# a1q123456/image_stitching

Measured on AMD Instinct MI355X. Metric: 4K frames stitched/sec, higher is better.
Workload: dtype u8

## Files before the change

host/job.cpp:

```cpp
#include "job.hpp"
#include <cstring>

namespace mis {

StitchJob::StitchJob(int device, int width, int height, const std::vector<CameraParams>& cameras, const StitchConfig& cfg)
    : JobCore("mis::StitchJob", "", device, nullptr, width, height, cameras, cfg) {}

StitchJob::~StitchJob() {
    mis_image_free(cctx_, &pano_);
    mis_image_free(cctx_, &mask_);
}

void StitchJob::finalize() {
    if (pano_.data && (pano_.width != key_.pano.width || pano_.height != key_.pano.height)) { mis_image_free(cctx_, &pano_); mis_image_free(cctx_, &mask_); pano_ = MisImage{}; mask_ = MisImage{}; }
    if (!pano_.data) { pano_ = MisImage{}; mask_ = MisImage{}; pano_.mem = mask_.mem = MIS_MEM_DEVICE; }
    check(cctx_, mis_blender_blend(blender_, &pano_, &mask_), "mis_blender_blend");
}

JobOutput StitchJob::run(const std::vector<MisImage>& frames) {
    if ((int)frames.size() != n_) throw std::runtime_error("StitchJob::run: one frame per camera");
    JobOutput out;
    check(cctx_, mis_context_wait(cctx_, ctx_), "mis_context_wait");
    const MisImage* work = work_frames(frames);
    prep_.arm([this] { if (spec_ok_) prepare(everyone_); });
    check(ctx_, mis_orb_on_enqueued(orb_, &Hook::fire, &prep_), "mis_orb_on_enqueued");
    std::vector<MisFeatures> feats(n_);
    std::memset(feats.data(), 0, sizeof(MisFeatures) * n_);
    const int rc_f = mis_orb_detect_batch(orb_, work, n_, feats.data());
    mis_orb_on_enqueued(orb_, nullptr, nullptr);
    check(ctx_, rc_f, "mis_orb_detect_batch");
    prep_.finish();
    for (int i = 0; i < n_; i++) { feats[i].img_idx = i; out.num_features.push_back(feats[i].n); }
    const MisMatchParams mp = reset_matches();
    match_.arm([this, &frames] {
        if (!spec_ok_) return;
        fence_knn();
        compose(frames, everyone_, everyone_);
        finalize();
    });
    check(ctx_, mis_match_on_enqueued(ctx_, &Hook::fire, &match_), "mis_match_on_enqueued");
    const int rc = mis_match_pairs_model(ctx_, feats.data(), n_, &mp, model_, nullptr, cfg_.range_width, 0, 1, pairwise_.data());
    mis_match_on_enqueued(ctx_, nullptr, nullptr);
    for (auto& f : feats) mis_features_free(ctx_, &f);
    check(ctx_, rc, "mis_match_pairs_model");
    match_.finish();
    out.confidence.resize((size_t)n_ * n_);
    for (int k = 0; k < n_ * n_; k++) out.confidence[k] = pairwise_[k].confidence;
    std::vector<int> idx(n_);
    int kept = 0;
    check(ctx_, mis_leave_biggest_component(pairwise_.data(), n_, cfg_.conf_thresh, idx.data(), &kept), "mis_leave_biggest_component");
    idx.resize(kept);
    if (kept < 2) throw std::runtime_error("Need more images");
    out.indices = idx;
    out.speculation_kept = spec_ok_ && kept == n_;
    if (!out.speculation_kept) {
        prepare(idx);
        compose(frames, everyone_, idx);
        finalize();
    }
    check(cctx_, mis_context_synchronize(cctx_), "mis_context_synchronize (compose)");
    out.pano = pano_; out.mask = mask_;
    out.num_bands = key_.bands; out.pano_width = key_.pano.width; out.pano_height = key_.pano.height;
    out.matches = pairwise_;
    return out;
}

}
```

host/job_core.cpp:

```cpp
#include "job_core.hpp"
#include <algorithm>
#include <numeric>

namespace mis {

static float median_focal(const std::vector<CameraParams>& cams, const std::vector<int>& idx) {
    std::vector<double> f;
    for (int i : idx) f.push_back(cams[i].focal);
    std::sort(f.begin(), f.end());
    return f.size() % 2 == 1 ? static_cast<float>(f[f.size() / 2]) : static_cast<float>(f[f.size() / 2 - 1] + f[f.size() / 2]) * 0.5f;
}

void JobCore::Hook::fire(void* self_) {
    Hook* self = static_cast<Hook*>(self_);
    self->ran_ = true;
    try { self->body_(); } catch (const std::exception& e) { self->error_ = e.what(); }
}

void JobCore::Hook::arm(std::function<void()> body) {
    body_ = std::move(body);
    ran_ = false;
    error_.clear();
}

void JobCore::Hook::finish() {
    if (!ran_) fire(this);
    if (!error_.empty()) throw std::runtime_error(error_);
}

void JobCore::check(MisContext* c, int rc, const char* what) const {
    if (rc != MIS_OK) throw std::runtime_error(std::string(what) + " failed" + where_ + ": " + mis_last_error(c));
}

JobCore::JobCore(const char* who, std::string where, int device, void* main_stream, int width, int height, const std::vector<CameraParams>& cameras,
                 const StitchConfig& cfg)
    : w_(width), h_(height), n_((int)cameras.size()), wg_(work_geometry(cfg, width, height)), cams_(cameras), cfg_(cfg), everyone_(n_), mstream_(main_stream),
      where_(std::move(where)) {
    std::iota(everyone_.begin(), everyone_.end(), 0);
    if (wg_.scale != 1.0) {
        for (auto& c : cams_) { c.focal *= wg_.scale; c.ppx *= wg_.scale; c.ppy *= wg_.scale; }
        compose_work_aspect_ = 1.0 / wg_.scale;
    }
    try {
        if (cfg_.features_type != "orb" || cfg_.ba_cost_func != "no" || cfg_.expos_comp_type != "no" || cfg_.seam_find_type != "no")
            throw std::runtime_error(std::string(who) + " runs the hot path (ORB, supplied cameras, no seam-scale step); use mis::Stitcher for the other options");
        kind_ = warp_kind(cfg_.warp_type);
        check_range_width(cfg_.range_width);
        model_ = matcher_model(cfg_.matcher_type, cfg_.range_width);
        if (mis_context_create(device, mstream_, &ctx_) != MIS_OK) throw std::runtime_error("mis_context_create failed: no HIP device (there is no CPU fallback)");
        check(ctx_, mis_stream_create(device, 0, &cstream_), "mis_stream_create");
        if (mis_context_create(device, cstream_, &cctx_) != MIS_OK) throw std::runtime_error("mis_context_create (compose stream) failed");
        MisOrbParams op;
        mis_orb_default_params(&op);
        check(ctx_, mis_orb_create(ctx_, &op, wg_.width, wg_.height, &orb_), "mis_orb_create");
    } catch (...) {
        release();
        throw;
    }
    Ks_.resize((size_t)n_ * 9); Rs_.resize((size_t)n_ * 9);
    for (int i = 0; i < n_; i++) {
        CameraParams cc = cams_[i];
        if (compose_work_aspect_ != 1.0) { cc.focal *= compose_work_aspect_; cc.ppx *= compose_work_aspect_; cc.ppy *= compose_work_aspect_; }
        const Mat3<float> K = cc.K().cast<float>(), R = cams_[i].R.cast<float>();
        std::copy(K.m.begin(), K.m.end(), Ks_.begin() + 9 * i);
        std::copy(R.m.begin(), R.m.end(), Rs_.begin() + 9 * i);
    }
    if (kind_ != MIS_WARP_SPHERICAL) {
        const float scale = warp_scale(everyone_);
        MisRect r;
        if (MIS_WARP_ROI_IS_FULL_SCAN(kind_)) {
            std::vector<MisRect> rr((size_t)n_);
            spec_ok_ = n_ == 0 || mis_warper_roi_batch(cctx_, kind_, scale, w_, h_, n_, Ks_.data(), Rs_.data(), rr.data()) == MIS_OK;
        } else
            for (int i = 0; i < n_ && spec_ok_; i++) spec_ok_ = mis_warper_roi(kind_, scale, w_, h_, &Ks_[9 * i], &Rs_[9 * i], &r) == MIS_OK;
    }
}

JobCore::~JobCore() { release(); }

float JobCore::warp_scale(const std::vector<int>& idx) const {
    const float scale = median_focal(cams_, idx);
    return compose_work_aspect_ != 1.0 ? scale * static_cast<float>(compose_work_aspect_) : scale;
}

const MisImage* JobCore::work_frames(const std::vector<MisImage>& frames) {
    if (wg_.scale == 1.0 || frames.empty()) return frames.data();
    if (work_.size() < frames.size()) work_.resize(frames.size(), MisImage{});
    check(ctx_, mis_resize_linear_exact_batch(ctx_, frames.data(), (int)frames.size(), 0, 0, wg_.scale, wg_.scale, work_.data()), "mis_resize_linear_exact_batch");
    return work_.data();
}

void JobCore::release() {
    if (cctx_) mis_context_synchronize(cctx_);
    if (ctx_) mis_context_synchronize(ctx_);
    if (!pairwise_.empty()) mis_matches_free(pairwise_.data(), (int)pairwise_.size());
    if (ctx_) for (auto& im : work_) mis_image_free(ctx_, &im);
    if (blender_) mis_blender_destroy(blender_);
    if (orb_) mis_orb_destroy(orb_);
    if (cctx_) mis_context_destroy(cctx_);
    if (ctx_) mis_context_destroy(ctx_);
    if (cstream_) mis_stream_destroy(cstream_);
    if (mstream_) mis_stream_destroy(mstream_);
}

void JobCore::synchronize() {
    check(ctx_, mis_context_synchronize(ctx_), "mis_context_synchronize");
    check(cctx_, mis_context_synchronize(cctx_), "mis_context_synchronize (compose)");
}

JobCore::Compose JobCore::prepare(const std::vector<int>& idx) {
    const int m = (int)idx.size();
    const float scale = warp_scale(idx);
    std::vector<float> Ks((size_t)m * 9), Rs((size_t)m * 9);
    for (int k = 0; k < m; k++) {
        std::copy(Ks_.begin() + 9 * idx[k], Ks_.begin() + 9 * idx[k] + 9, Ks.begin() + 9 * k);
        std::copy(Rs_.begin() + 9 * idx[k], Rs_.begin() + 9 * idx[k] + 9, Rs.begin() + 9 * k);
    }
    rois_.assign(m, MisRect{});
    check(cctx_, mis_warper_roi_batch(cctx_, kind_, scale, w_, h_, m, Ks.data(), Rs.data(), rois_.data()), "mis_warper_roi_batch");
    std::vector<MisPoint> corners(m);
    std::vector<MisSize> sizes(m);
    for (int k = 0; k < m; k++) { corners[k] = {rois_[k].x, rois_[k].y}; sizes[k] = {rois_[k].width, rois_[k].height}; }
    Compose c;
    check(cctx_, mis_result_roi(corners.data(), sizes.data(), m, &c.pano), "mis_result_roi");
    check(cctx_, mis_blend_config(cfg_.blend_type, cfg_.blend_strength, c.pano.width, c.pano.height, &c.type, &c.bands, &c.sharp), "mis_blend_config");
    if (!blender_ || c.type != key_.type || c.bands != key_.bands || c.sharp != key_.sharp) {
        if (blender_) { mis_blender_destroy(blender_); blender_ = nullptr; }
        check(cctx_, mis_blender_create(cctx_, c.type, c.bands, c.sharp, &blender_), "mis_blender_create");
    }
    key_ = c;
    check(cctx_, mis_blender_prepare(blender_, corners.data(), sizes.data(), m), "mis_blender_prepare");
    return c;
}

void JobCore::fence_knn() {
    const int rc = mis_match_knn_fence(ctx_, cstream_, mis_match_sequence(ctx_), 0);
    if (rc < 0) check(ctx_, rc, "mis_match_knn_fence");
}

void JobCore::compose(const std::vector<MisImage>& frames, const std::vector<int>& frame_ids, const std::vector<int>& idx) {
    std::vector<MisImage> fr;
    std::vector<float> Ks, Rs;
    std::vector<MisRect> rois;
    for (size_t q = 0; q < frame_ids.size(); q++) {
        const auto it = std::find(idx.begin(), idx.end(), frame_ids[q]);
        if (it == idx.end()) continue;
        fr.push_back(frames[q]);
        Ks.insert(Ks.end(), Ks_.begin() + 9 * frame_ids[q], Ks_.begin() + 9 * frame_ids[q] + 9);
        Rs.insert(Rs.end(), Rs_.begin() + 9 * frame_ids[q], Rs_.begin() + 9 * frame_ids[q] + 9);
        rois.push_back(rois_[it - idx.begin()]);
    }
    if (fr.empty()) return;
    check(cctx_, mis_compose_frames_kind(blender_, kind_, fr.data(), (int)fr.size(), warp_scale(idx), Ks.data(), Rs.data(), rois.data()),
          "mis_compose_frames_kind");
}

MisMatchParams JobCore::reset_matches() {
    if (!pairwise_.empty()) { mis_matches_free(pairwise_.data(), (int)pairwise_.size()); pairwise_.clear(); }
    pairwise_.assign((size_t)n_ * n_, MisMatchesInfo{});
    return match_params(model_, cfg_.match_conf);
}

}
```

host/job_core.hpp:

```cpp
#pragma once
#include <functional>
#include <string>
#include <vector>
#include "stitcher.hpp"

namespace mis {

struct JobOutput {
    std::vector<int> indices;
    std::vector<double> confidence;
    std::vector<int> num_features;
    MisImage pano{}, mask{};
    int num_bands = 0, pano_width = 0, pano_height = 0;
    bool speculation_kept = false;
    std::vector<MisMatchesInfo> matches;
};

class JobCore {
protected:
    struct Compose { int type = 0, bands = 0; float sharp = 0; MisRect pano{}; };

    class Hook {
    public:
        static void fire(void* self);
        void arm(std::function<void()> body);
        void finish();
    private:
        std::function<void()> body_;
        bool ran_ = false;
        std::string error_;
    };

    JobCore(const char* who, std::string where, int device, void* main_stream, int width, int height, const std::vector<CameraParams>& cameras,
            const StitchConfig& cfg);
    ~JobCore();
    JobCore(const JobCore&) = delete;
    JobCore& operator=(const JobCore&) = delete;

    void check(MisContext* c, int rc, const char* what) const;
    void synchronize();
    Compose prepare(const std::vector<int>& idx);
    void fence_knn();
    const MisImage* work_frames(const std::vector<MisImage>& frames);
    float warp_scale(const std::vector<int>& idx) const;
    void compose(const std::vector<MisImage>& frames, const std::vector<int>& frame_ids, const std::vector<int>& idx);
    MisMatchParams reset_matches();

    int w_, h_, n_;
    WorkGeometry wg_;
    double compose_work_aspect_ = 1;
    std::vector<CameraParams> cams_;
    std::vector<MisImage> work_;
    StitchConfig cfg_;
    std::vector<int> everyone_;
    int kind_ = MIS_WARP_SPHERICAL;
    int model_ = MIS_MATCH_HOMOGRAPHY;
    bool spec_ok_ = true;
    void* mstream_ = nullptr;
    void* cstream_ = nullptr;
    MisContext* ctx_ = nullptr;
    MisContext* cctx_ = nullptr;
    MisOrb* orb_ = nullptr;
    MisBlender* blender_ = nullptr;
    Compose key_{};
    std::vector<float> Ks_, Rs_;
    std::vector<MisRect> rois_;
    std::vector<MisMatchesInfo> pairwise_;

private:
    void release();
    std::string where_;
};

}
```

image_stitching_amd/_capi.py:

```python
import ctypes as C
import os
import re

_HERE = os.path.dirname(os.path.abspath(__file__))
LIB_PATH = os.path.join(_HERE, "libmistitch.so")
HEADER_PATH = os.path.join(os.path.dirname(_HERE), "include", "mistitch.h")

MIS_OK = 0
MIS_FENCE_TIMEOUT = 1
MEM_HOST, MEM_DEVICE = 0, 1
U8, S16, F32 = 0, 1, 2
INTER_NEAREST, INTER_LINEAR = 0, 1
BORDER_CONSTANT, BORDER_REFLECT = 0, 2
BLEND_NO, BLEND_FEATHER, BLEND_MULTI_BAND = 0, 1, 2
WARP_SPHERICAL, WARP_CYLINDRICAL, WARP_PLANE, WARP_MERCATOR, WARP_FISHEYE, WARP_STEREOGRAPHIC = 0, 1, 2, 3, 4, 5


def roi_is_full_scan(kind):
    return WARP_MERCATOR <= kind <= WARP_STEREOGRAPHIC


MATH_LOG, MATH_TAN, MATH_SINH, MATH_ASIN, MATH_ATAN, MATH_EXP = 0, 1, 2, 3, 4, 5
MATCH_HOMOGRAPHY, MATCH_AFFINE_PARTIAL = 0, 1
EXPOS_NO, EXPOS_GAIN, EXPOS_GAIN_BLOCKS, EXPOS_CHANNELS, EXPOS_CHANNELS_BLOCKS = 0, 1, 2, 3, 4


class MisPoint(C.Structure):
    _fields_ = [("x", C.c_int), ("y", C.c_int)]


class MisSize(C.Structure):
    _fields_ = [("width", C.c_int), ("height", C.c_int)]


class MisRect(C.Structure):
    _fields_ = [("x", C.c_int), ("y", C.c_int), ("width", C.c_int), ("height", C.c_int)]


class MisLevelRect(C.Structure):
    _fields_ = [("level", C.c_int), ("x0", C.c_int), ("y0", C.c_int), ("x1", C.c_int), ("y1", C.c_int), ("offset", C.c_ulonglong)]


class MisImage(C.Structure):
    _fields_ = [("data", C.c_void_p), ("width", C.c_int), ("height", C.c_int), ("channels", C.c_int),
                ("stride", C.c_size_t), ("dtype", C.c_int), ("mem", C.c_int)]


class MisKeyPoint(C.Structure):
    _fields_ = [("x", C.c_float), ("y", C.c_float), ("size", C.c_float), ("angle", C.c_float),
                ("response", C.c_float), ("octave", C.c_int)]


class MisOrbParams(C.Structure):
    _fields_ = [("nfeatures", C.c_int), ("scale_factor", C.c_float), ("nlevels", C.c_int),
                ("edge_threshold", C.c_int), ("first_level", C.c_int), ("wta_k", C.c_int),
                ("score_type", C.c_int), ("patch_size", C.c_int), ("fast_threshold", C.c_int)]


class MisSiftParams(C.Structure):
    _fields_ = [("nfeatures", C.c_int), ("n_octave_layers", C.c_int), ("contrast_threshold", C.c_double),
                ("edge_threshold", C.c_double), ("sigma", C.c_double)]


class MisCameraParams(C.Structure):
    _fields_ = [("focal", C.c_double), ("aspect", C.c_double), ("ppx", C.c_double), ("ppy", C.c_double), ("R", C.c_double * 9),
                ("t", C.c_double * 3)]


class MisFeatures(C.Structure):
    _fields_ = [("img_idx", C.c_int), ("img_w", C.c_int), ("img_h", C.c_int), ("n", C.c_int),
                ("keypoints", C.c_void_p), ("descriptors", C.c_void_p), ("desc_cols", C.c_int),
                ("desc_dtype", C.c_int), ("owner_", C.c_void_p)]


class MisMatchParams(C.Structure):
    _fields_ = [("match_conf", C.c_float), ("num_matches_thresh1", C.c_int), ("num_matches_thresh2", C.c_int),
                ("ransac_thresh", C.c_double), ("max_iters", C.c_int), ("confidence", C.c_double)]


class MisCompensatorParams(C.Structure):
    _fields_ = [("type", C.c_int), ("nr_feeds", C.c_int), ("block_width", C.c_int), ("block_height", C.c_int),
                ("nr_gain_filtering_iterations", C.c_int)]


class MisDMatch(C.Structure):
    _fields_ = [("query_idx", C.c_int), ("train_idx", C.c_int), ("img_idx", C.c_int), ("distance", C.c_float)]


class MisMatchesInfo(C.Structure):
    _fields_ = [("src_img_idx", C.c_int), ("dst_img_idx", C.c_int), ("n_matches", C.c_int),
                ("matches", C.POINTER(MisDMatch)), ("inliers_mask", C.POINTER(C.c_uint8)), ("num_inliers", C.c_int),
                ("has_H", C.c_int), ("H", C.c_double * 9), ("confidence", C.c_double)]


_vp, _i, _f, _d = C.c_void_p, C.c_int, C.c_float, C.c_double
_P = C.POINTER

PROTOTYPES = {
    "mis_context_create": (_i, [_i, _vp, _P(_vp)]),
    "mis_stream_create": (_i, [_i, _i, _P(_vp)]),
    "mis_stream_destroy": (_i, [_vp]),
    "mis_context_destroy": (_i, [_vp]),
    "mis_context_synchronize": (_i, [_vp]),
    "mis_context_wait": (_i, [_vp, _vp]),
    "mis_last_error": (C.c_char_p, [_vp]),
    "mis_version": (C.c_char_p, []),
    "mis_image_free": (_i, [_vp, _P(MisImage)]),
    "mis_orb_default_params": (None, [_P(MisOrbParams)]),
    "mis_orb_create": (_i, [_vp, _P(MisOrbParams), _i, _i, _P(_vp)]),
    "mis_orb_destroy": (_i, [_vp]),
    "mis_orb_detect": (_i, [_vp, _P(MisImage), _P(MisFeatures)]),
    "mis_orb_detect_batch": (_i, [_vp, _P(MisImage), _i, _P(MisFeatures)]),
    "mis_orb_on_enqueued": (_i, [_vp, _vp, _vp]),
    "mis_features_download": (_i, [_vp, _P(MisFeatures), _vp, _vp]),
    "mis_features_upload": (_i, [_vp, _i, _i, _i, _vp, _vp, _i, _i, _P(MisFeatures)]),
    "mis_features_free": (_i, [_vp, _P(MisFeatures)]),
    "mis_orb_debug_level": (_i, [_vp, _i, _i, _vp, _P(_i), _P(_i)]),
    "mis_sift_default_params": (None, [_P(MisSiftParams)]),
    "mis_sift_create": (_i, [_vp, _P(MisSiftParams), _i, _i, _P(_vp)]),
    "mis_sift_destroy": (_i, [_vp]),
    "mis_sift_detect": (_i, [_vp, _P(MisImage), _P(MisFeatures)]),
    "mis_sift_detect_batch": (_i, [_vp, _P(MisImage), _i, _P(MisFeatures)]),
    "mis_sift_debug_level": (_i, [_vp, _P(MisImage), _i, _i, _i, _vp, _P(_i), _P(_i)]),
    "mis_sift_debug_counts": (_i, [_vp, _P(C.c_uint)]),
    "mis_match_default_params": (None, [_P(MisMatchParams)]),
    "mis_match_all_pairs": (_i, [_vp, _P(MisFeatures), _i, _P(MisMatchParams), _P(MisMatchesInfo)]),
    "mis_match_pairs_sharded": (_i, [_vp, _P(MisFeatures), _i, _P(MisMatchParams), _i, _i, _P(MisMatchesInfo)]),
    "mis_match_pairs_select": (_i, [_vp, _P(MisFeatures), _i, _P(MisMatchParams), _vp, _i, _i, _i, _P(MisMatchesInfo)]),
    "mis_match_affine_default_params": (None, [_P(MisMatchParams)]),
    "mis_match_pairs_model": (_i, [_vp, _P(MisFeatures), _i, _P(MisMatchParams), _i, _vp, _i, _i, _i, _P(MisMatchesInfo)]),
    "mis_estimate_affine_partial": (_i, [_vp, _vp, _vp, _i, _d, _i, _d, _i, _vp, _vp, _P(_i)]),
    "mis_matches_free": (_i, [_P(MisMatchesInfo), _i]),
    "mis_match_sequence": (C.c_longlong, [_vp]),
    "mis_match_knn_fence": (_i, [_vp, _vp, C.c_longlong, _i]),
    "mis_match_on_enqueued": (_i, [_vp, _vp, _vp]),
    "mis_knn2": (_i, [_vp, _P(MisFeatures), _P(MisFeatures), _vp, _vp]),
    "mis_find_homography": (_i, [_vp, _vp, _vp, _i, _d, _i, _d, _vp, _vp, _P(_i)]),
    "mis_leave_biggest_component": (_i, [_P(MisMatchesInfo), _i, _f, _vp, _P(_i)]),
    "mis_leave_biggest_component_conf": (_i, [_vp, _i, _f, _vp, _P(_i)]),
    "mis_bundle_adjust_reproj": (_i, [_vp, _P(MisFeatures), _P(MisMatchesInfo), _i, _f, C.c_char_p, _P(MisCameraParams)]),
    "mis_wave_correct": (_i, [_vp, _i, _i]),
    "mis_warp_roi": (_i, [_f, _i, _i, _vp, _vp, _P(MisRect)]),
    "mis_warp_spherical": (_i, [_vp, _P(MisImage), _f, _vp, _vp, _i, _i, _P(MisImage), _P(MisPoint)]),
    "mis_warp_roi_batch": (_i, [_vp, _f, _i, _i, _i, _vp, _vp, _P(MisRect)]),
    "mis_warp_spherical_fused_roi": (_i, [_vp, _P(MisImage), _f, _vp, _vp, _P(MisRect), _P(MisImage), _P(MisImage), _P(MisPoint)]),
    "mis_warp_spherical_fused_batch": (_i, [_vp, _P(MisImage), _i, C.c_float, _P(C.c_float), _P(C.c_float), _P(MisRect), _P(MisImage), _P(MisImage), _P(MisPoint)]),
    "mis_warp_spherical_fused_batch_timed": (_i, [_vp, _P(MisImage), _i, C.c_float, _P(C.c_float), _P(C.c_float), _P(MisRect), _P(MisImage), _P(MisImage), _P(MisPoint), _i,
                                               _P(C.c_float)]),
    "mis_debug_math_f32": (_i, [_vp, _i, _vp, _vp, _i]),
    "mis_warper_roi": (_i, [_i, _f, _i, _i, _vp, _vp, _P(MisRect)]),
    "mis_warper_roi_batch": (_i, [_vp, _i, _f, _i, _i, _i, _vp, _vp, _P(MisRect)]),
    "mis_warper_warp": (_i, [_vp, _i, _P(MisImage), _f, _vp, _vp, _i, _i, _P(MisImage), _P(MisPoint)]),
    "mis_warper_warp_roi": (_i, [_vp, _i, _P(MisImage), _f, _vp, _vp, _P(MisRect), _i, _i, _P(MisImage), _P(MisPoint)]),
    "mis_warper_warp_fused": (_i, [_vp, _i, _P(MisImage), _f, _vp, _vp, _P(MisImage), _P(MisImage), _P(MisPoint)]),
    "mis_warper_warp_fused_roi": (_i, [_vp, _i, _P(MisImage), _f, _vp, _vp, _P(MisRect), _P(MisImage), _P(MisImage), _P(MisPoint)]),
    "mis_warper_warp_fused_batch": (_i, [_vp, _i, _P(MisImage), _i, C.c_float, _P(C.c_float), _P(C.c_float), _P(MisRect), _P(MisImage), _P(MisImage), _P(MisPoint)]),
    "mis_warp_spherical_fused": (_i, [_vp, _P(MisImage), _f, _vp, _vp, _P(MisImage), _P(MisImage), _P(MisPoint)]),
    "mis_resize_linear_exact": (_i, [_vp, _P(MisImage), _i, _i, C.c_double, C.c_double, _P(MisImage)]),
    "mis_resize_linear_exact_batch": (_i, [_vp, _P(MisImage), _i, _i, _i, C.c_double, C.c_double, _P(MisImage)]),
    "mis_rotate": (_i, [_vp, _P(MisImage), _i, _P(MisImage)]),
    "mis_seam_mask_apply": (_i, [_vp, _P(MisImage), _P(MisImage)]),
    "mis_compensator_create": (_i, [_vp, _i, _i, _i, _P(_vp)]),
    "mis_compensator_default_params": (None, [_P(MisCompensatorParams)]),
    "mis_compensator_create_ex": (_i, [_vp, _P(MisCompensatorParams), _P(_vp)]),
    "mis_compensator_destroy": (_i, [_vp]),
    "mis_compensator_gains": (_i, [_vp, _i, _P(_d)]),
    "mis_compensator_gain_map_channels": (_i, [_vp, _i, _P(C.c_float), _i, _P(_i), _P(_i), _P(_i)]),
    "mis_compensator_debug_stats": (_i, [_vp, _i, _i, _i, _P(_i), _P(_d), _P(_d)]),
    "mis_compensator_feed": (_i, [_vp, _P(MisPoint), _P(MisImage), _P(MisImage), _i]),
    "mis_compensator_gain_map": (_i, [_vp, _i, _P(C.c_float), _i, _P(_i), _P(_i)]),
    "mis_compensator_apply": (_i, [_vp, _i, _P(MisImage)]),
    "mis_seam_voronoi": (_i, [_vp, _P(MisPoint), _P(MisImage), _i]),
    "mis_seam_dp": (_i, [_vp, _P(MisPoint), _P(MisImage), _P(MisImage), _i, _i]),
    "mis_warp_spherical_fused_timed": (_i, [_vp, _P(MisImage), _f, _vp, _vp, _P(MisImage), _P(MisImage), _P(MisPoint), _i, _P(C.c_float)]),
    "mis_blend_config": (_i, [_i, _f, _i, _i, _P(_i), _P(_i), _P(_f)]),
    "mis_result_roi": (_i, [_P(MisPoint), _P(MisSize), _i, _P(MisRect)]),
    "mis_blender_create": (_i, [_vp, _i, _i, _f, _P(_vp)]),
    "mis_blender_destroy": (_i, [_vp]),
    "mis_blender_prepare": (_i, [_vp, _P(MisPoint), _P(MisSize), _i]),
    "mis_blender_num_bands": (_i, [_vp]),
    "mis_blender_feed": (_i, [_vp, _P(MisImage), _P(MisImage), MisPoint]),
    "mis_blender_feed_batch": (_i, [_vp, _P(MisImage), _P(MisImage), _P(MisPoint), _i]),
    "mis_blender_blend": (_i, [_vp, _P(MisImage), _P(MisImage)]),
    "mis_compose_frames": (_i, [_vp, _P(MisImage), _i, _f, _vp, _vp, _P(MisRect)]),
    "mis_compose_frames_kind": (_i, [_vp, _i, _P(MisImage), _i, _f, _vp, _vp, _P(MisRect)]),
    "mis_blender_blend_columns": (_i, [_vp, _i, _i, _P(MisImage), _P(MisImage)]),
    "mis_blender_pack_rects": (_i, [_vp, _P(MisLevelRect), _i, _vp, C.c_size_t]),
    "mis_blender_add_rects": (_i, [_vp, _P(MisLevelRect), _i, _vp, C.c_size_t]),
    "mis_blender_zero_rects": (_i, [_vp, _P(MisLevelRect), _i]),
    "mis_features_pack": (_i, [_vp, _P(MisFeatures), _i, _i, _i, _vp, _vp]),
    "mis_copy_2d": (_i, [_vp, _vp, C.c_size_t, _vp, C.c_size_t, C.c_size_t, C.c_size_t]),
    "mis_blender_feed_rect": (_i, [_vp, _i, _i, MisPoint, _P(MisRect)]),
    "mis_blender_level_info": (_i, [_vp, _i, _P(_i), _P(_i), _P(_vp), _P(_vp)]),
}


def header_functions():
    txt = open(HEADER_PATH).read()
    txt = re.sub(r"/\*.*?\*/", "", txt, flags=re.S)
    return sorted(set(re.findall(r"\b(mis_[a-z0-9_]+)\s*\(", txt)))


_lib = None


def load():
    global _lib
    if _lib is not None:
        return _lib
    if not os.path.exists(LIB_PATH):
        raise ImportError("libmistitch.so is not built (%s missing): run `python -c 'import __graft_entry__ as g; g.build()'` "
                          "or `make -C image_stitching_amd/csrc`; there is no CPU fallback" % LIB_PATH)
    lib = C.CDLL(LIB_PATH)
    for name, (res, args) in PROTOTYPES.items():
        fn = getattr(lib, name)
        fn.restype = res
        fn.argtypes = args
    _lib = lib
    return lib
```

image_stitching_amd/csrc/common.h:

```cpp
#pragma once
#include <hip/hip_runtime.h>
#include <stdint.h>
#include <stdio.h>
#include <string.h>
#include <string>
#include <vector>
#include "../../include/mistitch.h"

struct MisWorkspace {
    virtual ~MisWorkspace() {}
};

struct MisContext {
    int device = 0;
    int num_cu = 256;
    MisWorkspace* match_ws = nullptr;
    MisWorkspace* resize_ws = nullptr;
    std::vector<std::pair<size_t, void*>> pool;
    hipStream_t stream = nullptr;
    bool own_stream = false;
    std::string err;
    void* stage = nullptr;
    size_t stage_bytes = 0;
    hipStream_t aux[2] = {nullptr, nullptr};
    void* roi_pinned = nullptr;
    size_t roi_pinned_bytes = 0;
    void* host_stage = nullptr;
    size_t host_stage_bytes = 0;
};

int mis_set_error(MisContext* ctx, int code, const char* fmt, ...);
int mis_host_stage(MisContext* ctx, size_t bytes, void** out);
int mis_dev_stage(MisContext* ctx, size_t bytes, void** out);
int mis_pool_alloc(MisContext* ctx, size_t bytes, void** out, size_t* got, MisContext* errs = nullptr);
int mis_aux_stream(MisContext* ctx, int k, hipStream_t* out);
void mis_pool_free(MisContext* ctx, void* p, size_t bytes);
int mis_feat_block_alloc(MisContext* ctx, size_t bytes, void** out, MisContext* errs = nullptr);
struct MisFeatLayout { size_t desc_off, count_off, bytes; };
MisFeatLayout mis_feat_layout(int cap, int desc_cols, int desc_dtype);
int mis_feat_alloc(MisContext* ctx, int cap, int desc_cols, int desc_dtype, MisFeatures* f);
int* mis_feat_count(const MisFeatures* f, int cap);

#define MIS_HIP(ctx, call)                                                                             \
    do {                                                                                               \
        hipError_t e_ = (call);                                                                        \
        if (e_ != hipSuccess)                                                                          \
            return mis_set_error((ctx), MIS_E_HIP, "%s failed: %s (%s:%d)", #call, hipGetErrorString(e_), \
                                 __FILE__, __LINE__);                                                  \
    } while (0)

#define MIS_CHECK(ctx, cond, code, ...)                              \
    do {                                                             \
        if (!(cond)) return mis_set_error((ctx), (code), __VA_ARGS__); \
    } while (0)

static inline size_t mis_dtype_size(int dtype) { return dtype == MIS_U8 ? 1 : (dtype == MIS_S16 ? 2 : 4); }
static inline size_t mis_align_up(size_t v, size_t a) { return (v + a - 1) / a * a; }

struct DevView {
    void* data = nullptr;
    size_t stride = 0;
    DevView() = default;
    DevView(const DevView&) = delete;
    DevView& operator=(const DevView&) = delete;
    ~DevView();
    int read(MisContext* ctx, const MisImage* img);
    int write(MisContext* ctx, MisImage* img, int width, int height, int channels, int dtype);
    int read_write(MisContext* ctx, MisImage* img);
    int commit();
private:
    MisContext* ctx_ = nullptr;
    MisImage* out_ = nullptr;
    MisImage entry_{};
    bool staged_ = false, fresh_ = false;
};

struct OwnedEvent {
    hipEvent_t ev = nullptr;
    OwnedEvent() = default; OwnedEvent(const OwnedEvent&) = delete;
    ~OwnedEvent() { if (ev) hipEventDestroy(ev); }
    hipError_t ready(unsigned flags = hipEventDisableTiming) { return ev ? hipSuccess : hipEventCreateWithFlags(&ev, flags); }
};
```

image_stitching_amd/csrc/features.hip:

```cpp
#include "common.h"
#include <algorithm>
#include <mutex>
#include <unordered_map>

namespace {

std::mutex g_feat_mutex;
std::unordered_map<void*, size_t> g_feat_sizes;

}

MisFeatLayout mis_feat_layout(int cap, int desc_cols, int desc_dtype) {
    MisFeatLayout l;
    l.desc_off = mis_align_up(sizeof(MisKeyPoint) * (size_t)cap, 256);
    l.count_off = l.desc_off + mis_align_up((size_t)cap * desc_cols * mis_dtype_size(desc_dtype), 256);
    l.bytes = l.count_off + 256;
    return l;
}

int mis_feat_block_alloc(MisContext* ctx, size_t bytes, void** out, MisContext* errs) {
    size_t got = 0;
    const int rc = mis_pool_alloc(ctx, bytes, out, &got, errs);
    if (rc != MIS_OK) return rc;
    std::lock_guard<std::mutex> lock(g_feat_mutex);
    g_feat_sizes[*out] = got;
    return MIS_OK;
}

int mis_feat_alloc(MisContext* ctx, int cap, int desc_cols, int desc_dtype, MisFeatures* f) {
    const MisFeatLayout l = mis_feat_layout(cap, desc_cols, desc_dtype);
    void* mem = nullptr;
    const int rc = mis_feat_block_alloc(ctx, l.bytes, &mem);
    if (rc != MIS_OK) return rc;
    f->keypoints = (MisKeyPoint*)mem;
    f->descriptors = (uint8_t*)mem + l.desc_off;
    f->desc_cols = desc_cols; f->desc_dtype = desc_dtype;
    f->owner_ = mem;
    f->n = 0;
    return MIS_OK;
}

int* mis_feat_count(const MisFeatures* f, int cap) {
    return (int*)((uint8_t*)f->owner_ + mis_feat_layout(cap, f->desc_cols, f->desc_dtype).count_off);
}

extern "C" int mis_features_download(MisContext* ctx, const MisFeatures* f, MisKeyPoint* kps, void* desc) {
    if (!ctx || !f) return MIS_E_INVALID;
    MIS_HIP(ctx, hipSetDevice(ctx->device));
    if (f->n > 0) {
        if (kps) MIS_HIP(ctx, hipMemcpyAsync(kps, f->keypoints, sizeof(MisKeyPoint) * (size_t)f->n, hipMemcpyDeviceToHost, ctx->stream));
        if (desc) MIS_HIP(ctx, hipMemcpyAsync(desc, f->descriptors, (size_t)f->n * f->desc_cols * mis_dtype_size(f->desc_dtype), hipMemcpyDeviceToHost, ctx->stream));
    }
    MIS_HIP(ctx, hipStreamSynchronize(ctx->stream));
    return MIS_OK;
}

extern "C" int mis_features_upload(MisContext* ctx, int img_w, int img_h, int n, const MisKeyPoint* kps, const void* desc, int desc_cols,
                                   int desc_dtype, MisFeatures* out) {
    if (!ctx || !out) return MIS_E_INVALID;
    MIS_CHECK(ctx, n >= 0 && (n == 0 || (kps && desc)) && desc_cols > 0 && (desc_dtype == MIS_U8 || desc_dtype == MIS_F32), MIS_E_INVALID,
              "bad feature arrays");
    MIS_HIP(ctx, hipSetDevice(ctx->device));
    memset(out, 0, sizeof(*out));
    out->img_w = img_w; out->img_h = img_h;
    int rc = mis_feat_alloc(ctx, std::max(n, 1), desc_cols, desc_dtype, out);
    if (rc != MIS_OK) return rc;
    if (n) {
        MIS_HIP(ctx, hipMemcpyAsync(out->keypoints, kps, sizeof(MisKeyPoint) * (size_t)n, hipMemcpyHostToDevice, ctx->stream));
        MIS_HIP(ctx, hipMemcpyAsync(out->descriptors, desc, (size_t)n * desc_cols * mis_dtype_size(desc_dtype), hipMemcpyHostToDevice, ctx->stream));
        MIS_HIP(ctx, hipStreamSynchronize(ctx->stream));
    }
    out->n = n;
    return MIS_OK;
}

extern "C" int mis_features_free(MisContext* ctx, MisFeatures* f) {
    if (!ctx || !f) return MIS_E_INVALID;
    if (f->owner_) {
        size_t bytes = 0;
        {
            std::lock_guard<std::mutex> lock(g_feat_mutex);
            auto it = g_feat_sizes.find(f->owner_);
            if (it != g_feat_sizes.end()) { bytes = it->second; g_feat_sizes.erase(it); }
        }
        if (bytes) mis_pool_free(ctx, f->owner_, bytes);
        else {
            MIS_HIP(ctx, hipSetDevice(ctx->device));
            MIS_HIP(ctx, hipStreamSynchronize(ctx->stream));
            MIS_HIP(ctx, hipFree(f->owner_));
        }
    }
    f->owner_ = nullptr; f->keypoints = nullptr; f->descriptors = nullptr; f->n = 0;
    return MIS_OK;
}
```

image_stitching_amd/csrc/match.hip:

```cpp
#include "common.h"
#include <thread>
#include <chrono>
#include <atomic>
#include "dev_math.h"
#include "homography.h"
#include <algorithm>
#include <vector>

namespace {

struct FeatDev {
    const uint8_t* desc;
    const MisKeyPoint* kps;
    int n, w, h;
};

struct PairDesc {
    int i, j;
    size_t knn_off12, knn_off21;
    size_t m_off;
    int cap;
};

constexpr int KNN_TILE = 256;
__global__ __launch_bounds__(256) void knn2_hamming_kernel(const FeatDev* feats, const PairDesc* pairs, int* idx2, float* dist2) {
    __shared__ uint4 tr[KNN_TILE * 2];
    const PairDesc pd = pairs[blockIdx.y >> 1];
    const bool fwd = (blockIdx.y & 1) == 0;
    const FeatDev Q = feats[fwd ? pd.i : pd.j], T = feats[fwd ? pd.j : pd.i];
    const size_t off = fwd ? pd.knn_off12 : pd.knn_off21;
    const int q0 = blockIdx.x * 256;
    if (q0 >= Q.n) return;
    const int q = q0 + threadIdx.x;
    const bool active = q < Q.n;
    uint4 a0 = make_uint4(0, 0, 0, 0), a1 = a0;
    if (active) {
        const uint4* p = reinterpret_cast<const uint4*>(Q.desc + (size_t)q * 32);
        a0 = p[0]; a1 = p[1];
    }
    int k0 = 0x7fffffff, k1 = 0x7fffffff;
    for (int t0 = 0; t0 < T.n; t0 += KNN_TILE) {
        const int nt = min(KNN_TILE, T.n - t0);
        __syncthreads();
        const uint4* src = reinterpret_cast<const uint4*>(T.desc + (size_t)t0 * 32);
        for (int k = threadIdx.x; k < nt * 2; k += 256) tr[k] = src[k];
        __syncthreads();
        if (active) {
            auto one = [&](int j) {
                const uint4 b0 = tr[2 * j], b1 = tr[2 * j + 1];
                unsigned d = 0;
                auto acc = [&](unsigned x) { asm("v_bcnt_u32_b32 %0, %1, %0" : "+v"(d) : "v"(x)); };
                acc(a0.x ^ b0.x); acc(a0.y ^ b0.y); acc(a0.z ^ b0.z); acc(a0.w ^ b0.w);
                acc(a1.x ^ b1.x); acc(a1.y ^ b1.y); acc(a1.z ^ b1.z); acc(a1.w ^ b1.w);
                const int key = (int)((d << 22) | (unsigned)(t0 + j));
                asm("v_med3_i32 %0, %1, %2, %3" : "=v"(k1) : "v"(k0), "v"(k1), "v"(key));
                k0 = min(k0, key);
            };
            int j = 0;
            for (; j + 8 <= nt; j += 8) {
#pragma unroll
                for (int u = 0; u < 8; u++) one(j + u);
            }
            for (; j < nt; j++) one(j);
        }
    }
    if (active) {
        const int d0 = k0 == 0x7fffffff ? 1 << 30 : k0 >> 22, d1 = k1 == 0x7fffffff ? 1 << 30 : k1 >> 22;
        idx2[(off + q) * 2] = k0 == 0x7fffffff ? -1 : (k0 & 0x3fffff); idx2[(off + q) * 2 + 1] = k1 == 0x7fffffff ? -1 : (k1 & 0x3fffff);
        dist2[(off + q) * 2] = (float)d0; dist2[(off + q) * 2 + 1] = (float)d1;
    }
}

typedef int v4i __attribute__((ext_vector_type(4)));
typedef int v16i __attribute__((ext_vector_type(16)));
constexpr int HM_ROWPAD = 256;
constexpr int HM_MAX_TRAINS = 8192;
constexpr int HM_NONE = 0x7f000000;

struct HmFrame { size_t train_off, query_off; };

struct HmKeys { int k0[2], k1[2]; };
struct HmJob { int pair, dir, q0, pad; };
constexpr int HM_FBIAS = 0x3F800000;
__device__ __forceinline__ void hm_update(HmKeys& K, int set, int key) {
    asm volatile("v_med3_f32 %0, %1, %2, %3" : "=v"(K.k1[set]) : "v"(K.k0[set]), "v"(K.k1[set]), "v"(key));
    asm volatile("v_min_f32 %0, %1, %2" : "=v"(K.k0[set]) : "v"(K.k0[set]), "v"(key));
}
__device__ __forceinline__ void hm_dma(const int8_t* base, unsigned voff, uint32_t lds_off) {
    asm volatile("s_mov_b32 m0, %2\n\ts_nop 0\n\tglobal_load_lds_dwordx4 %0, %1" ::"v"(voff), "s"(base), "s"(lds_off) : "memory", "m0");
}
__global__ __launch_bounds__(256) void hamming_expand4_kernel(const FeatDev* feats, const HmFrame* fr, int8_t* out) {
    const FeatDev F = feats[blockIdx.y];
    const int npad = (F.n + HM_ROWPAD - 1) / HM_ROWPAD * HM_ROWPAD;
    const int item = blockIdx.x * 256 + threadIdx.x, d = item >> 3, w = item & 7;
    if (d >= npad) return;
    const bool live = d < F.n;
    const unsigned x = live ? reinterpret_cast<const unsigned*>(F.desc)[(size_t)d * 8 + w] : 0u;
    unsigned tq[4], qq[4];
#pragma unroll
    for (int k = 0; k < 4; k++) {
        unsigned t = (x >> (8 * k)) & 255u;
        t = (t | (t << 12)) & 0x000F000Fu;
        t = (t | (t << 6)) & 0x03030303u;
        t = (t | (t << 3)) & 0x11111111u;
        tq[k] = live ? (0xEEEEEEEEu ^ (t << 3)) : 0u;
        qq[k] = live ? (0x66666666u ^ (t << 3)) : 0u;
    }
    *reinterpret_cast<uint4*>(out + fr[blockIdx.y].train_off + (size_t)d * 128 + 16 * w) = make_uint4(tq[0], tq[1], tq[2], tq[3]);
    *reinterpret_cast<uint4*>(out + fr[blockIdx.y].query_off + (size_t)d * 128 + 16 * w) = make_uint4(qq[0], qq[1], qq[2], qq[3]);
}
#define HM4_MFMA_FIRST(D, A, B, C, SA, SB) \
    asm volatile("v_mfma_scale_f32_32x32x64_f8f6f4 %0, %1, %2, %3, %4, %5 op_sel_hi:[0,0,0] cbsz:4 blgp:4" : "=&v"(D) : "v"(A), "v"(B), "v"(C), "v"(SA), "v"(SB))
#define HM4_MFMA_ACC(D, A, B, SA, SB) \
    asm volatile("v_mfma_scale_f32_32x32x64_f8f6f4 %0, %1, %2, %0, %3, %4 op_sel_hi:[0,0,0] cbsz:4 blgp:4" : "+v"(D) : "v"(A), "v"(B), "v"(SA), "v"(SB))
typedef float v16f __attribute__((ext_vector_type(16)));
__device__ __forceinline__ void hm_update_triples(HmKeys& K, int x0, int x1, int x2, int y0, int y1, int y2) {
    int t0, t1, u0, u1;
    asm volatile(
        "v_min3_f32 %4, %8, %9, %10\n\tv_med3_f32 %5, %8, %9, %10\n\tv_min3_f32 %6, %11, %12, %13\n\tv_med3_f32 %7, %11, %12, %13\n\t"
        "v_min_f32 %5, %1, %5\n\tv_min_f32 %7, %3, %7\n\t"
        "v_med3_f32 %1, %0, %4, %5\n\tv_med3_f32 %3, %2, %6, %7\n\t"
        "v_min_f32 %0, %0, %4\n\tv_min_f32 %2, %2, %6"
        : "+v"(K.k0[0]), "+v"(K.k1[0]), "+v"(K.k0[1]), "+v"(K.k1[1]), "=&v"(t0), "=&v"(t1), "=&v"(u0), "=&v"(u1)
        : "v"(x0), "v"(x1), "v"(x2), "v"(y0), "v"(y1), "v"(y2));
}
__device__ __forceinline__ void hm_update_both(HmKeys& K, int a, int b) {
    asm volatile("v_med3_f32 %1, %0, %1, %4\n\tv_min_f32 %0, %0, %4\n\tv_med3_f32 %3, %2, %3, %5\n\tv_min_f32 %2, %2, %5"
                 : "+v"(K.k0[0]), "+v"(K.k1[0]), "+v"(K.k0[1]), "+v"(K.k1[1]) : "v"(a), "v"(b));
}
template <bool UPD>
__device__ __forceinline__ void hm_tile_fp4(v16i& accA, v16i& accB, const v16i& prevA, const v16i& prevB, v16f& cb, v4i* a, const v4i (&bq)[2][4], HmKeys& K,
                                            const int8_t* lds_next, uint32_t lds_store, const int8_t* gnext, unsigned voff, const unsigned (&aoff)[4], int sa, int sb) {
    hm_dma(gnext, voff, lds_store);
#pragma unroll
    for (int s4 = 0; s4 < 4; s4++) {
#pragma unroll
        for (int half = 0; half < 2; half++) {
            const int slot = 2 * s4 + half;
            if (half == 0) { if (s4 == 0) HM4_MFMA_FIRST(accA, a[0], bq[0][0], cb, sa, sb); else HM4_MFMA_ACC(accA, a[s4], bq[0][s4], sa, sb); }
            else {
                if (s4 == 0) HM4_MFMA_FIRST(accB, a[0], bq[1][0], cb, sa, sb); else HM4_MFMA_ACC(accB, a[s4], bq[1][s4], sa, sb);
                a[s4] = *reinterpret_cast<const v4i*>(lds_next + aoff[s4]);
            }
            if (slot >= 2) {
                if (UPD) {
                    const int j = slot - 2;
                    if (j < 5) hm_update_triples(K, prevA[3 * j], prevA[3 * j + 1], prevA[3 * j + 2], prevB[3 * j], prevB[3 * j + 1], prevB[3 * j + 2]);
                    else hm_update_both(K, prevA[15], prevB[15]);
                }
                if (slot >= 4) {
#pragma unroll
                    for (int g = (slot - 4) * 4; g < (slot - 3) * 4; g++) cb[g] += 32.f;
                }
            }
            __builtin_amdgcn_sched_barrier(0);
        }
    }
    asm volatile("s_waitcnt vmcnt(0)" ::: "memory");
    __syncthreads();
}

__global__ __launch_bounds__(256) void knn2_hamming_fp4_kernel(const FeatDev* feats, const PairDesc* pairs, const HmFrame* fr, const int8_t* __restrict__ xp, int* idx2,
                                                               float* dist2, const HmJob* jobs) {
    __shared__ __attribute__((aligned(1024))) int8_t tr[2][32 * 128];
    const HmJob job = jobs[blockIdx.x];
    if (job.pair < 0) return;
    const PairDesc pd = pairs[job.pair];
    const bool fwd = job.dir == 0;
    const int qi = fwd ? pd.i : pd.j, ti = fwd ? pd.j : pd.i;
    const int nq = feats[qi].n, nt = feats[ti].n;
    const size_t off = fwd ? pd.knn_off12 : pd.knn_off21;
    const int q0 = job.q0;
    if (q0 >= nq) return;
    const int lane = threadIdx.x & 63, wave = __builtin_amdgcn_readfirstlane(threadIdx.x >> 6), r = lane & 31, h = lane >> 5;
    const int8_t* qx = xp + fr[qi].query_off;
    const int8_t* tx = xp + fr[ti].train_off;
    HmKeys K;
    K.k0[0] = K.k0[1] = K.k1[0] = K.k1[1] = HM_NONE;
    const int ntiles = (nt + 31) / 32;
    if (ntiles > 0) {
        v4i bq[2][4];
#pragma unroll
        for (int set = 0; set < 2; set++)
#pragma unroll
            for (int s4 = 0; s4 < 4; s4++)
                bq[set][s4] = *reinterpret_cast<const v4i*>(qx + (size_t)(q0 + wave * 64 + set * 32 + r) * 128 + 32 * s4 + 16 * h);
        v16f cb;
#pragma unroll
        for (int g = 0; g < 16; g++) cb[g] = (float)((1 << 20) + (g & 3) + 8 * (g >> 2) + 4 * h);
        const int sa = 127 + 4, sb = 127 + 4;
        const int R = 8 * wave + (lane >> 3);
        const unsigned voff = (unsigned)(R * 128 + 16 * ((lane & 7) ^ ((R >> 1) & 7)));
        unsigned aoff[4];
#pragma unroll
        for (int s4 = 0; s4 < 4; s4++) aoff[s4] = (unsigned)(r * 128 + 16 * ((2 * s4 + h) ^ ((r >> 1) & 7)));
        const uint32_t lds0 = (uint32_t)(uintptr_t)&tr[0][0] + (uint32_t)wave * 1024, lds1 = (uint32_t)(uintptr_t)&tr[1][0] + (uint32_t)wave * 1024;
        auto gtile = [&](int t) { return tx + (size_t)min(t, ntiles - 1) * 32 * 128; };
        hm_dma(gtile(0), voff, lds0);
        hm_dma(gtile(1), voff, lds1);
        asm volatile("s_waitcnt vmcnt(0)" ::: "memory");
        __syncthreads();
        v4i a[4];
#pragma unroll
        for (int s4 = 0; s4 < 4; s4++) a[s4] = *reinterpret_cast<const v4i*>(&tr[0][aoff[s4]]);
        __syncthreads();
        v16i A0, B0, A1, B1;
        hm_tile_fp4<false>(A0, B0, A1, B1, cb, a, bq, K, tr[1], lds0, gtile(2), voff, aoff, sa, sb);
        int t = 1;
        for (; t + 1 < ntiles; t += 2) {
            hm_tile_fp4<true>(A1, B1, A0, B0, cb, a, bq, K, tr[0], lds1, gtile(t + 2), voff, aoff, sa, sb);
            hm_tile_fp4<true>(A0, B0, A1, B1, cb, a, bq, K, tr[1], lds0, gtile(t + 3), voff, aoff, sa, sb);
        }
        const bool odd_last = t < ntiles;
        if (odd_last) hm_tile_fp4<true>(A1, B1, A0, B0, cb, a, bq, K, tr[0], lds1, gtile(t + 2), voff, aoff, sa, sb);
        asm volatile("s_nop 15\n\ts_nop 15\n\ts_nop 15\n\ts_nop 15\n\ts_nop 15" ::: "memory");
#pragma unroll
        for (int g = 0; g < 16; g++) {
            const int ka = odd_last ? A1[g] : A0[g], kb = odd_last ? B1[g] : B0[g];
            hm_update(K, 0, ((int)__int_as_float(ka) & (HM_MAX_TRAINS - 1)) < nt ? ka : HM_NONE);
            hm_update(K, 1, ((int)__int_as_float(kb) & (HM_MAX_TRAINS - 1)) < nt ? kb : HM_NONE);
        }
    }
#pragma unroll
    for (int set = 0; set < 2; set++) {
        const int o0 = __shfl_xor(K.k0[set], 32), o1 = __shfl_xor(K.k1[set], 32);
        const int b0 = min(K.k0[set], o0), b1 = min(max(K.k0[set], o0), min(K.k1[set], o1));
        const int q = q0 + wave * 64 + set * 32 + r;
        if (h == 0 && q < nq) {
            const bool v0 = b0 < HM_NONE, v1 = b1 < HM_NONE;
            const int i0 = v0 ? (int)__int_as_float(b0) : 0, i1 = v1 ? (int)__int_as_float(b1) : 0;
            idx2[(off + q) * 2] = v0 ? (i0 & (HM_MAX_TRAINS - 1)) : -1; idx2[(off + q) * 2 + 1] = v1 ? (i1 & (HM_MAX_TRAINS - 1)) : -1;
            dist2[(off + q) * 2] = (float)(v0 ? i0 >> 13 : 1 << 30); dist2[(off + q) * 2 + 1] = (float)(v1 ? i1 >> 13 : 1 << 30);
        }
    }
}

struct L2Set {
    const _Float16* h;
    const float* nrm;
    int n;
};
__global__ __launch_bounds__(256) void l2_prep_kernel(const float* desc, int n, int dim, _Float16* h, float* nrm, int* bad) {
    const int i = blockIdx.x * 4 + (threadIdx.x >> 6), lane = threadIdx.x & 63;
    if (i >= n) return;
    float s = 0;
    for (int k = lane; k < 128; k += 64) {
        float v = k < dim ? desc[(size_t)i * dim + k] : 0.f;
        if (!(v >= 0.f && v <= 255.f && v == floorf(v))) atomicOr(bad, 1);
        h[(size_t)i * 128 + k] = (_Float16)v;
        s += v * v;
    }
    for (int o = 32; o > 0; o >>= 1) s += __shfl_xor(s, o);
    if (lane == 0) nrm[i] = s;
}

typedef _Float16 half8 __attribute__((ext_vector_type(8)));
typedef float float16v __attribute__((ext_vector_type(16)));

__device__ __forceinline__ void top2_insert(float d, int i, float& d0, int& i0, float& d1, int& i1) {
    if (d < d0 || (d == d0 && i < i0)) { d1 = d0; i1 = i0; d0 = d; i0 = i; }
    else if (d < d1 || (d == d1 && i < i1)) { d1 = d; i1 = i; }
}
// ... 193 lines not shown
    const int* i21 = idx2 + pd.knn_off21 * 2;
    const float* d21 = dist2 + pd.knn_off21 * 2;
    const float hw1 = centre ? (float)F1.w * 0.5f : 0.f, hh1 = centre ? (float)F1.h * 0.5f : 0.f, hw2 = centre ? (float)F2.w * 0.5f : 0.f, hh2 = centre ? (float)F2.h * 0.5f : 0.f;
    int base = 0;
    if (F2.n >= 2)
        for (int q0 = 0; q0 < F1.n; q0 += 1024) {
            int q = q0 + threadIdx.x, ok = 0;
            if (q < F1.n) ok = d12[2 * q] < ratio * d12[2 * q + 1];
            int tot, off = block_scan_flag(ok, &tot);
            if (ok) {
                int t = i12[2 * q];
                MisDMatch mm = {q, t, 0, d12[2 * q]};
                m[base + off] = mm;
                sp[2 * (base + off)] = F1.kps[q].x - hw1; sp[2 * (base + off) + 1] = F1.kps[q].y - hh1;
                dp[2 * (base + off)] = F2.kps[t].x - hw2; dp[2 * (base + off) + 1] = F2.kps[t].y - hh2;
            }
            base += tot;
        }
    if (F1.n >= 2)
        for (int q0 = 0; q0 < F2.n; q0 += 1024) {
            int q = q0 + threadIdx.x, ok = 0, t1 = 0;
            if (q < F2.n) {
                ok = d21[2 * q] < ratio * d21[2 * q + 1];
                if (ok) {
                    t1 = i21[2 * q];
                    bool acc12 = F2.n >= 2 && d12[2 * t1] < ratio * d12[2 * t1 + 1];
                    if (acc12 && i12[2 * t1] == q) ok = 0;
                }
            }
            int tot, off = block_scan_flag(ok, &tot);
            if (ok) {
                MisDMatch mm = {t1, q, -1, d21[2 * q]};
                m[base + off] = mm;
                sp[2 * (base + off)] = F1.kps[t1].x - hw1; sp[2 * (base + off) + 1] = F1.kps[t1].y - hh1;
                dp[2 * (base + off)] = F2.kps[q].x - hw2; dp[2 * (base + off) + 1] = F2.kps[q].y - hh2;
            }
            base += tot;
        }
    if (threadIdx.x == 0) n_matches[blockIdx.x] = base;
}

struct PairOut {
    int ran_ransac;
    int passed;
    int second;
    int pad;
};

__host__ __device__ __forceinline__ double det3(const double* H) {
    return H[0] * (H[4] * H[8] - H[5] * H[7]) - H[1] * (H[3] * H[8] - H[5] * H[6]) + H[2] * (H[3] * H[7] - H[4] * H[6]);
}

__global__ void first_calls_kernel(const PairDesc* pairs, int np, const int* n_matches, const float* src_xy, const float* dst_xy, uint8_t* masks,
                                   int thresh1, HomoCall* calls, PairOut* outs) {
    int k = blockIdx.x * blockDim.x + threadIdx.x;
    if (k >= np) return;
    const PairDesc pd = pairs[k];
    const int nm = n_matches[k];
    HomoCall c;
    c.src = src_xy + 2 * pd.m_off; c.dst = dst_xy + 2 * pd.m_off; c.mask = masks + pd.m_off; c.pt_off = (long long)pd.m_off;
    c.n = nm; c.active = nm >= thresh1;
    calls[k] = c;
    outs[k].ran_ransac = c.active; outs[k].passed = 0; outs[k].second = 0;
}


__global__ __launch_bounds__(256) void pack_lists_kernel(const PairDesc* pairs, int np, const int* nm, const MisDMatch* matches, MisDMatch* host_m, int* host_nm) {
    __shared__ int red[256];
    const int k = blockIdx.x, t = threadIdx.x;
    int part = 0;
    for (int q = t; q < k; q += 256) part += nm[q];
    red[t] = part;
    __syncthreads();
    for (int o = 128; o > 0; o >>= 1) { if (t < o) red[t] += red[t + o]; __syncthreads(); }
    const int off = red[0], cnt = nm[k];
    if (t == 0) host_nm[k] = cnt;
    const uint4* s = reinterpret_cast<const uint4*>(matches + pairs[k].m_off);
    uint4* d = reinterpret_cast<uint4*>(host_m + off);
    static_assert(sizeof(MisDMatch) == 16, "one 16-byte store per match");
    for (int i = t; i < cnt; i += 256) d[i] = s[i];
}

struct CopySegs { const uint8_t* src[8]; uint8_t* dst[8]; unsigned bytes[8]; int n; };
__global__ __launch_bounds__(256) void copy_segments_kernel(CopySegs c) {
    for (int k = 0; k < c.n; k++) {
        const uint8_t* s = c.src[k];
        uint8_t* d = c.dst[k];
        const unsigned nb = c.bytes[k];
        if ((((uintptr_t)s | (uintptr_t)d) & 3) == 0) {
            const unsigned nw = nb >> 2;
            for (unsigned i = blockIdx.x * 256 + threadIdx.x; i < nw; i += gridDim.x * 256) reinterpret_cast<unsigned*>(d)[i] = reinterpret_cast<const unsigned*>(s)[i];
            for (unsigned i = (nw << 2) + blockIdx.x * 256 + threadIdx.x; i < nb; i += gridDim.x * 256) d[i] = s[i];
        } else {
            for (unsigned i = blockIdx.x * 256 + threadIdx.x; i < nb; i += gridDim.x * 256) d[i] = s[i];
        }
    }
}

__global__ void second_calls_kernel(int np, const HomoCall* calls1, const HomoResult* res1, const float* scr1, const int* fin1, int want, int thresh2,
                                    HomoCall* calls2, PairOut* outs) {
    int k = blockIdx.x * blockDim.x + threadIdx.x;
    if (k >= np) return;
    const HomoCall c1 = calls1[k];
    HomoCall c;
    c.src = nullptr; c.dst = nullptr; c.mask = nullptr; c.pt_off = c1.pt_off; c.n = 0; c.active = 0;
    if (fin1[k] == want && c1.active && res1[k].ok) {
        outs[k].passed = 1;
        const int ninl = res1[k].ninl;
        if (ninl >= thresh2) {
            c.src = scr1 + 4 * c1.pt_off; c.dst = c.src + 2 * (size_t)c1.n; c.n = ninl; c.active = 1;
            outs[k].second = 1;
        }
    }
    calls2[k] = c;
}

void invert3(const double* H, double* I) {
    double d = H[0] * (H[4] * H[8] - H[5] * H[7]) - H[1] * (H[3] * H[8] - H[5] * H[6]) + H[2] * (H[3] * H[7] - H[4] * H[6]);
    if (d != 0.) d = 1. / d;
    I[0] = (H[4] * H[8] - H[5] * H[7]) * d; I[1] = (H[2] * H[7] - H[1] * H[8]) * d; I[2] = (H[1] * H[5] - H[2] * H[4]) * d;
    I[3] = (H[5] * H[6] - H[3] * H[8]) * d; I[4] = (H[0] * H[8] - H[2] * H[6]) * d; I[5] = (H[2] * H[3] - H[0] * H[5]) * d;
    I[6] = (H[3] * H[7] - H[4] * H[6]) * d; I[7] = (H[1] * H[6] - H[0] * H[7]) * d; I[8] = (H[0] * H[4] - H[1] * H[3]) * d;
}

struct Arena {
    void* p = nullptr;
    size_t bytes = 0;
    bool host = false;
    hipError_t reserve(size_t need) {
        if (need <= bytes) return hipSuccess;
        if (p) { hipError_t e = host ? hipHostFree(p) : hipFree(p); p = nullptr; bytes = 0; if (e != hipSuccess) return e; }
        need = need + need / 4 + 4096;
        hipError_t e = host ? hipHostMalloc(&p, need, hipHostMallocDefault) : hipMalloc(&p, need);
        if (e == hipSuccess) bytes = need;
        return e;
    }
    void release() { if (p) { if (host) hipHostFree(p); else hipFree(p); } p = nullptr; bytes = 0; }
};

struct MatchWorkspace : MisWorkspace {
    Arena dev, pinned, l2;
    HomoBatch b1, b2, b3;
    hipStream_t side = nullptr, third = nullptr;
    OwnedEvent ev_phase0, ev_side_done, ev_phase1, ev_third_done, ev_matches;
    OwnedEvent ev_knn;
    OwnedEvent ev_draw1;
    OwnedEvent ev_spec_fork, ev_spec_join;
    OwnedEvent tev[9];
    hipEvent_t ev_gate = nullptr;
    std::atomic<long long> seq{0}, knn_seq{0};
    OwnedEvent ev_lists;
    void (*enqueued_cb)(void*) = nullptr;
    void* enqueued_user = nullptr;
    MatchWorkspace() { pinned.host = true; }
    ~MatchWorkspace() override {
        dev.release(); pinned.release(); l2.release();
        homo_batch_release(&b1); homo_batch_release(&b2); homo_batch_release(&b3);
    }
    hipError_t events_ready() {
        for (OwnedEvent* e : {&ev_knn, &ev_matches, &ev_lists, &ev_phase0, &ev_draw1, &ev_side_done, &ev_phase1, &ev_third_done, &ev_spec_fork, &ev_spec_join})
            if (const hipError_t r = e->ready()) return r;
        return hipSuccess;
    }
};

MatchWorkspace* workspace(MisContext* ctx) {
    if (!ctx->match_ws) ctx->match_ws = new MatchWorkspace();
    return static_cast<MatchWorkspace*>(ctx->match_ws);
}

struct Carver {
    uintptr_t base = 0;
    size_t off = 0;
    size_t take(size_t bytes) { size_t o = off; off += mis_align_up(bytes ? bytes : 1, 256); return o; }
    void* at(size_t bytes) { return (void*)(base + take(bytes)); }
};

void init_info(MisMatchesInfo* m) { memset(m, 0, sizeof(*m)); m->src_img_idx = -1; m->dst_img_idx = -1; }

bool match_trace() { static const bool on = getenv("MIS_MATCH_TRACE") != nullptr; return on; }
void trace_mark(MatchWorkspace* ws, int i, hipStream_t s) {
    if (match_trace() && ws->tev[i].ready(hipEventDefault) == hipSuccess) hipEventRecord(ws->tev[i].ev, s);
}

int l2_knn2_pairs(MisContext* ctx, Arena& arena, const MisFeatures* f, int nsets, const PairDesc* pairs, int np, bool both_ways, int* idx2,
                  float* dist2, int* bad_host) {
    hipStream_t st = ctx->stream;
    std::vector<size_t> off(nsets);
    Carver lc;
    int maxq = 0;
    for (int s = 0; s < nsets; s++) {
        off[s] = lc.take((size_t)std::max(f[s].n, 1) * (256 + 4));
        maxq = std::max(maxq, f[s].n);
    }
    const size_t o_bad = lc.take(4), o_part = lc.take((size_t)16 * L2_MAX_SLICES * std::max(maxq, 1));
    MIS_HIP(ctx, arena.reserve(lc.off));
    uint8_t* L = (uint8_t*)arena.p;
    auto set = [&](int s) { return L2Set{(const _Float16*)(L + off[s]), (const float*)(L + off[s] + (size_t)std::max(f[s].n, 1) * 256), std::max(f[s].n, 0)}; };
    MIS_HIP(ctx, hipMemsetAsync(L + o_bad, 0, 4, st));
    for (int s = 0; s < nsets; s++)
        if (f[s].n > 0)
            hipLaunchKernelGGL(l2_prep_kernel, dim3((f[s].n + 3) / 4), dim3(256), 0, st, (const float*)f[s].descriptors, f[s].n, f[s].desc_cols,
                               (_Float16*)set(s).h, (float*)set(s).nrm, (int*)(L + o_bad));
    for (const PairDesc* pd = pairs; pd < pairs + np; pd++) {
        l2_knn2_launch(st, ctx->num_cu, set(pd->i), set(pd->j), L + o_part, idx2 + 2 * pd->knn_off12, dist2 + 2 * pd->knn_off12);
        if (both_ways) l2_knn2_launch(st, ctx->num_cu, set(pd->j), set(pd->i), L + o_part, idx2 + 2 * pd->knn_off21, dist2 + 2 * pd->knn_off21);
    }
    MIS_HIP(ctx, hipMemcpyAsync(bad_host, L + o_bad, 4, hipMemcpyDeviceToHost, st));
    return MIS_OK;
}

enum DescKind { DESC_NONE, DESC_BINARY, DESC_L2 };
struct MatchPlan {
    std::vector<PairDesc> pairs;
    std::vector<FeatDev> fd;
    size_t knn_total = 0, m_total = 0;
    int maxq = 0;
    DescKind kind = DESC_NONE;
    std::vector<HmJob> hm_jobs;
};
int plan_match(MisContext* ctx, const MisFeatures* feats, int n, const uint8_t* mask, int range_width, int rank, int world, MatchPlan* pl) {
    std::vector<PairDesc>& pairs = pl->pairs;
    pl->fd.resize(n);
    bool use_l2 = false, use_bin = false;
    for (int i = 0; i < n; i++) {
        const bool bin_i = feats[i].desc_dtype == MIS_U8 && feats[i].desc_cols == 32;
        const bool l2_i = feats[i].desc_dtype == MIS_F32 && feats[i].desc_cols >= 1 && feats[i].desc_cols <= 128;
        MIS_CHECK(ctx, feats[i].n == 0 || bin_i || l2_i, MIS_E_UNSUPPORTED,
                  "all-pairs matching supports 32-byte binary descriptors (Hamming) or f32 descriptors of <= 128 columns (L2)");
        MIS_CHECK(ctx, feats[i].n < (1 << 22), MIS_E_UNSUPPORTED, "more than 4 M keypoints in one image");
        if (feats[i].n > 0) { if (l2_i) use_l2 = true; else use_bin = true; }
        pl->fd[i] = FeatDev{(const uint8_t*)feats[i].descriptors, feats[i].keypoints, feats[i].n, feats[i].img_w, feats[i].img_h};
    }
    int pair_index = 0;
    for (int i = 0; i < n; i++)
        for (int j = i + 1; j < n; j++) {
            if (feats[i].n <= 0 || feats[j].n <= 0) continue;
            if (mask && !mask[(size_t)i * n + j]) continue;
            if (range_width != -1 && j >= i + range_width) continue;
            if ((pair_index++ % world) != rank) continue;
            const int cap = feats[i].n + feats[j].n;
            pl->maxq = std::max(pl->maxq, std::max(feats[i].n, feats[j].n));
            pairs.push_back(PairDesc{i, j, pl->knn_total, pl->knn_total + feats[i].n, pl->m_total, cap});
            pl->knn_total += cap; pl->m_total += cap;
        }
    MIS_CHECK(ctx, !(use_l2 && use_bin), MIS_E_INVALID, "binary and float descriptors cannot be mixed in one matcher call");
    for (int i = 0, cols = 0; use_l2 && i < n; i++)
        if (feats[i].n > 0) {
            MIS_CHECK(ctx, cols == 0 || feats[i].desc_cols == cols, MIS_E_INVALID, "float descriptors of different widths in one matcher call");
            cols = feats[i].desc_cols;
        }
    pl->kind = use_l2 ? DESC_L2 : (use_bin ? DESC_BINARY : DESC_NONE);
    const int np = (int)pairs.size();
    if (np == 0) return MIS_OK;
    if (pl->kind == DESC_BINARY && pl->maxq <= HM_MAX_TRAINS) {
        std::vector<HmJob> lists[8];
        for (int t = 0; t < n; t++)
            for (int k = 0; k < np; k++) {
                const int dir = pairs[k].j == t ? 0 : (pairs[k].i == t ? 1 : -1);
                if (dir < 0) continue;
                const int nqf = feats[dir == 0 ? pairs[k].i : pairs[k].j].n;
                for (int q0 = 0; q0 < nqf; q0 += 256) lists[t & 7].push_back(HmJob{k, dir, q0, 0});
            }
        size_t longest = 0;
        for (auto& l : lists) longest = std::max(longest, l.size());
        pl->hm_jobs.assign(longest * 8, HmJob{-1, 0, 0, 0});
        for (int c = 0; c < 8; c++)
            for (size_t sl = 0; sl < lists[c].size(); sl++) pl->hm_jobs[sl * 8 + c] = lists[c][sl];
    }
    return MIS_OK;
}

struct MatchDev { FeatDev* feats; PairDesc* pairs; int* idx; float* dist; MisDMatch* matches; float* src; float* dst; int* nm; uint8_t* mask; PairOut* out; };
int carve_dev(MisContext* ctx, Arena& arena, const MatchPlan& pl, MatchDev* d) {
    const size_t n = pl.fd.size(), np = pl.pairs.size(), kt = pl.knn_total, mt = pl.m_total;
    auto lay = [&](Carver c) {
        d->feats = (FeatDev*)c.at(sizeof(FeatDev) * n); d->pairs = (PairDesc*)c.at(sizeof(PairDesc) * np);
        d->idx = (int*)c.at(sizeof(int) * 2 * kt); d->dist = (float*)c.at(sizeof(float) * 2 * kt);
        d->matches = (MisDMatch*)c.at(sizeof(MisDMatch) * mt); d->src = (float*)c.at(sizeof(float) * 2 * mt); d->dst = (float*)c.at(sizeof(float) * 2 * mt);
        d->nm = (int*)c.at(sizeof(int) * np); d->mask = (uint8_t*)c.at(mt); d->out = (PairOut*)c.at(sizeof(PairOut) * np);
        return c.off;
    };
    MIS_HIP(ctx, arena.reserve(lay(Carver{})));
    lay(Carver{(uintptr_t)arena.p});
    return MIS_OK;
}

struct MatchPinned {
    FeatDev* feats; PairDesc* pairs; HmFrame* frames; HmJob* jobs;
    int* nm; PairOut* out; HomoResult *r1, *r2, *r3; int* fin; MisDMatch* m; uint8_t* mask; volatile int* l2_bad;
};
int carve_pinned(MisContext* ctx, Arena& arena, const MatchPlan& pl, MatchPinned* h) {
    const size_t n = pl.fd.size(), np = pl.pairs.size(), mt = pl.m_total;
    auto lay = [&](Carver c) {
        h->feats = (FeatDev*)c.at(sizeof(FeatDev) * n); h->pairs = (PairDesc*)c.at(sizeof(PairDesc) * np); h->frames = (HmFrame*)c.at(sizeof(HmFrame) * n);
        h->jobs = (HmJob*)c.at(sizeof(HmJob) * pl.hm_jobs.size()); h->nm = (int*)c.at(sizeof(int) * np); h->out = (PairOut*)c.at(sizeof(PairOut) * np);
        h->r1 = (HomoResult*)c.at(sizeof(HomoResult) * np); h->r2 = (HomoResult*)c.at(sizeof(HomoResult) * np); h->r3 = (HomoResult*)c.at(sizeof(HomoResult) * np);
        h->fin = (int*)c.at(sizeof(int) * np); h->m = (MisDMatch*)c.at(sizeof(MisDMatch) * mt); h->mask = (uint8_t*)c.at(mt); h->l2_bad = (volatile int*)c.at(sizeof(int));
        return c.off;
    };
    MIS_HIP(ctx, arena.reserve(lay(Carver{})));
    lay(Carver{(uintptr_t)arena.p});
    return MIS_OK;
}

int enqueue_knn(MisContext* ctx, MatchWorkspace* ws, const MatchPlan& pl, const MisFeatures* feats, const MatchDev& d, const MatchPinned& h) {
    hipStream_t st = ctx->stream;
    const int n = (int)pl.fd.size(), np = (int)pl.pairs.size();
    if (pl.kind == DESC_L2) return l2_knn2_pairs(ctx, ws->l2, feats, n, pl.pairs.data(), np, true, d.idx, d.dist, (int*)h.l2_bad);
    if (pl.maxq > HM_MAX_TRAINS) {
        hipLaunchKernelGGL(knn2_hamming_kernel, dim3((pl.maxq + 255) / 256, 2 * np), dim3(256), 0, st, (const FeatDev*)d.feats, (const PairDesc*)d.pairs, d.idx, d.dist);
        return MIS_OK;
    }
    Carver lc;
    const size_t o_fr = lc.take(sizeof(HmFrame) * n), o_jobs = lc.take(sizeof(HmJob) * pl.hm_jobs.size());
    for (int i = 0; i < n; i++) {
        const size_t rows = (size_t)(std::max(feats[i].n, 1) + HM_ROWPAD - 1) / HM_ROWPAD * HM_ROWPAD;
        h.frames[i].train_off = lc.take(rows * 128); h.frames[i].query_off = lc.take(rows * 128);
    }
    MIS_HIP(ctx, ws->l2.reserve(lc.off));
    uint8_t* L = (uint8_t*)ws->l2.p;
    MIS_HIP(ctx, hipMemcpyAsync(L + o_fr, h.frames, sizeof(HmFrame) * n, hipMemcpyHostToDevice, st));
    const int maxpad = (pl.maxq + HM_ROWPAD - 1) / HM_ROWPAD * HM_ROWPAD;
    hipLaunchKernelGGL(hamming_expand4_kernel, dim3(maxpad * 8 / 256, n), dim3(256), 0, st, (const FeatDev*)d.feats, (const HmFrame*)(L + o_fr), (int8_t*)L);
    memcpy(h.jobs, pl.hm_jobs.data(), sizeof(HmJob) * pl.hm_jobs.size());
    MIS_HIP(ctx, hipMemcpyAsync(L + o_jobs, h.jobs, sizeof(HmJob) * pl.hm_jobs.size(), hipMemcpyHostToDevice, st));
    hipLaunchKernelGGL(knn2_hamming_fp4_kernel, dim3((unsigned)pl.hm_jobs.size()), dim3(256), 0, st, (const FeatDev*)d.feats, (const PairDesc*)d.pairs,
                       (const HmFrame*)(L + o_fr), (const int8_t*)L, d.idx, d.dist, (const HmJob*)(L + o_jobs));
    return MIS_OK;
}

int enqueue_chains(MisContext* ctx, MatchWorkspace* ws, int np, const MisMatchParams* p, int model, const MatchDev& d, const MatchPinned& h) {
    hipStream_t st = ctx->stream;
    int rc;
    if (!ws->side && (rc = mis_aux_stream(ctx, 0, &ws->side)) != MIS_OK) return rc;
    trace_mark(ws, 0, st);
    if (!ws->third && (rc = mis_aux_stream(ctx, 1, &ws->third)) != MIS_OK) return rc;
    MIS_HIP(ctx, hipEventRecord(ws->ev_matches.ev, st));
    MIS_HIP(ctx, hipStreamWaitEvent(ws->third, ws->ev_matches.ev, 0));
    hipLaunchKernelGGL(pack_lists_kernel, dim3(np), dim3(256), 0, ws->third, (const PairDesc*)d.pairs, np, (const int*)d.nm, (const MisDMatch*)d.matches, h.m, h.nm);
    MIS_HIP(ctx, hipEventRecord(ws->ev_lists.ev, ws->third));
    if (model == MIS_MATCH_AFFINE_PARTIAL) {
        const HomoParams aprm{p->ransac_thresh, p->max_iters, p->confidence, MODEL_AFFINE_PARTIAL, 10};
        for (RansacPhase ph : {PHASE_FIRST, PHASE_SECOND})
            if ((rc = homo_phase(ctx, &ws->b1, aprm, ph, st)) != MIS_OK || (rc = homo_tails(ctx, &ws->b1, aprm, ph, TAIL_MASK, st)) != MIS_OK ||
                (rc = homo_tails(ctx, &ws->b1, aprm, ph, TAIL_REFINE, st)) != MIS_OK) return rc;
        MIS_HIP(ctx, hipStreamWaitEvent(st, ws->ev_lists.ev, 0));
        return MIS_OK;
    }
    const HomoParams prm{p->ransac_thresh, p->max_iters, p->confidence};
    HomoHooks chain;
    chain.spec_stream = ws->side; chain.spec_fork = ws->ev_spec_fork.ev; chain.spec_join = ws->ev_spec_join.ev;
    if (match_trace() && ws->tev[8].ready(hipEventDefault) == hipSuccess) chain.spec_mark = ws->tev[8].ev;
    if (match_trace() && ws->tev[7].ready(hipEventDefault) == hipSuccess) chain.after_second_draw = ws->tev[7].ev;
    if ((rc = homo_phase(ctx, &ws->b1, prm, PHASE_FIRST, st, &chain)) != MIS_OK || (rc = homo_tails(ctx, &ws->b1, prm, PHASE_FIRST, TAIL_MASK, st)) != MIS_OK) return rc;
    MIS_HIP(ctx, hipEventRecord(ws->ev_phase0.ev, st));
    trace_mark(ws, 1, st);
    MIS_HIP(ctx, hipStreamWaitEvent(ws->side, ws->ev_phase0.ev, 0));
    hipLaunchKernelGGL(second_calls_kernel, dim3((np + 127) / 128), dim3(128), 0, ws->side, np, (const HomoCall*)ws->b1.calls, (const HomoResult*)ws->b1.results,
                       (const float*)ws->b1.scr, (const int*)ws->b1.fin, PHASE_FIRST, p->num_matches_thresh2, ws->b2.calls, d.out);
    HomoHooks gate;
    gate.after_first_draw = ws->ev_gate = ws->ev_draw1.ev;
    if ((rc = homo_solve(ctx, &ws->b2, prm, ws->side, &gate)) != MIS_OK) return rc;
    MIS_HIP(ctx, hipEventRecord(ws->ev_side_done.ev, ws->side));
    trace_mark(ws, 4, ws->side);
    MIS_HIP(ctx, hipStreamWaitEvent(ws->third, ws->ev_phase0.ev, 0));
    if ((rc = homo_tails(ctx, &ws->b1, prm, PHASE_FIRST, TAIL_REFINE, ws->third)) != MIS_OK) return rc;
    trace_mark(ws, 6, ws->third);
    if ((rc = homo_phase(ctx, &ws->b1, prm, PHASE_SECOND, st, &chain)) != MIS_OK || (rc = homo_tails(ctx, &ws->b1, prm, PHASE_SECOND, TAIL_MASK, st)) != MIS_OK) return rc;
    MIS_HIP(ctx, hipEventRecord(ws->ev_phase1.ev, st));
    trace_mark(ws, 2, st);
    if ((rc = homo_tails(ctx, &ws->b1, prm, PHASE_SECOND, TAIL_REFINE, st)) != MIS_OK) return rc;
    trace_mark(ws, 3, st);
    MIS_HIP(ctx, hipStreamWaitEvent(ws->third, ws->ev_phase1.ev, 0));
    hipLaunchKernelGGL(second_calls_kernel, dim3((np + 127) / 128), dim3(128), 0, ws->third, np, (const HomoCall*)ws->b1.calls, (const HomoResult*)ws->b1.results,
                       (const float*)ws->b1.scr, (const int*)ws->b1.fin, PHASE_SECOND, p->num_matches_thresh2, ws->b3.calls, d.out);
    if ((rc = homo_solve(ctx, &ws->b3, prm, ws->third)) != MIS_OK) return rc;
    MIS_HIP(ctx, hipEventRecord(ws->ev_third_done.ev, ws->third));
    trace_mark(ws, 5, ws->third);
    MIS_HIP(ctx, hipStreamWaitEvent(st, ws->ev_third_done.ev, 0));
    MIS_HIP(ctx, hipStreamWaitEvent(st, ws->ev_side_done.ev, 0));
    return MIS_OK;
}

void enqueue_results(MatchWorkspace* ws, int np, size_t m_total, const MatchDev& d, const MatchPinned& h, hipStream_t st, int model) {
    CopySegs cs{};
    const void* srcs[6] = {d.out, ws->b1.results, ws->b2.results, ws->b3.results, ws->b1.fin, d.mask};
    void* dsts[6] = {h.out, h.r1, h.r2, h.r3, h.fin, h.mask};
    const size_t sizes[6] = {sizeof(PairOut) * np, sizeof(HomoResult) * np, sizeof(HomoResult) * np, sizeof(HomoResult) * np, sizeof(int) * np, m_total};
    cs.n = 6;
    for (int k = 0; k < 6; k++) { cs.src[k] = (const uint8_t*)srcs[k]; cs.dst[k] = (uint8_t*)dsts[k]; cs.bytes[k] = model == MIS_MATCH_AFFINE_PARTIAL && (k == 2 || k == 3) ? 0u : (unsigned)sizes[k]; }
    hipLaunchKernelGGL(copy_segments_kernel, dim3(64), dim3(256), 0, st, cs);
}

int assemble_matches(MisContext* ctx, MatchWorkspace* ws, const MatchPlan& pl, const MatchPinned& h, int n, int model, MisMatchesInfo* out,
                     std::chrono::steady_clock::time_point* ts) {
    const int np = (int)pl.pairs.size();
    auto drop_lists = [&]() {
        for (const PairDesc& pd : pl.pairs)
            for (MisMatchesInfo* m : {&out[pd.i * n + pd.j], &out[pd.j * n + pd.i]}) { free(m->matches); free(m->inliers_mask); init_info(m); }
    };
    MIS_HIP(ctx, hipEventSynchronize(ws->ev_lists.ev));
    size_t packed_off = 0;
    for (int k = 0; k < np; k++) {
        const PairDesc& pd = pl.pairs[k];
        MisMatchesInfo *a = &out[pd.i * n + pd.j], *b = &out[pd.j * n + pd.i];
        const int nm = h.nm[k];
        a->src_img_idx = pd.i; a->dst_img_idx = pd.j;
        a->n_matches = nm;
        a->matches = (MisDMatch*)malloc(sizeof(MisDMatch) * (size_t)(nm + 1));
        memcpy(a->matches, h.m + packed_off, sizeof(MisDMatch) * (size_t)nm);
        packed_off += (size_t)nm;
        b->matches = (MisDMatch*)malloc(sizeof(MisDMatch) * (size_t)(nm + 1));
        for (int q = 0; q < nm; q++) { b->matches[q] = a->matches[q]; std::swap(b->matches[q].query_idx, b->matches[q].train_idx); }
    }
    const hipError_t e = hipStreamSynchronize(ctx->stream);
    *ts = std::chrono::steady_clock::now();
    if (e != hipSuccess || *h.l2_bad) {
        drop_lists();
        if (e != hipSuccess) return mis_set_error(ctx, MIS_E_HIP, "hipStreamSynchronize failed: %s (%s:%d)", hipGetErrorString(e), __FILE__, __LINE__);
        return mis_set_error(ctx, MIS_E_UNSUPPORTED, "L2 matching needs integer-valued descriptors in 0..255 (SIFT style)");
    }
    for (int k = 0; k < np; k++) {
        const PairDesc& pd = pl.pairs[k];
        const PairOut& po = h.out[k];
        const int nm = h.nm[k];
        MisMatchesInfo *a = &out[pd.i * n + pd.j], *b = &out[pd.j * n + pd.i];
        MisDMatch* bm = b->matches;
        if (po.ran_ransac) {
            a->inliers_mask = (uint8_t*)malloc((size_t)nm + 1);
            memcpy(a->inliers_mask, h.mask + pd.m_off, (size_t)nm);
        }
        if (model == MIS_MATCH_AFFINE_PARTIAL) {
            const HomoResult& ar = h.r1[k];
            a->has_H = po.ran_ransac ? ar.ok : 0;
            if (a->has_H) {
                memcpy(a->H, ar.H, sizeof(a->H));
                a->num_inliers = ar.ninl;
                a->confidence = a->num_inliers / (8 + 0.3 * nm);
            }
            *b = *a;
            b->src_img_idx = pd.j; b->dst_img_idx = pd.i;
            b->matches = bm;
            if (a->inliers_mask) {
                b->inliers_mask = (uint8_t*)malloc((size_t)nm + 1);
                memcpy(b->inliers_mask, a->inliers_mask, (size_t)nm);
            }
            if (a->has_H) invert3(a->H, b->H);
            continue;
        }
        const bool det_ok = !(fabs(det3(h.r1[k].H)) < DBL_EPSILON);
        const bool passed = po.passed && det_ok, second = po.second && det_ok;
        const HomoResult& hr = second ? (h.fin[k] == 0 ? h.r2[k] : h.r3[k]) : h.r1[k];
        a->has_H = po.ran_ransac ? hr.ok : 0;
        if (a->has_H) memcpy(a->H, hr.H, sizeof(a->H));
        a->num_inliers = passed ? h.r1[k].ninl : 0;
        if (passed) {
            double c = a->num_inliers / (8 + 0.3 * nm);
            a->confidence = c > 3. ? 0. : c;
        }
        *b = *a;
        b->src_img_idx = pd.j; b->dst_img_idx = pd.i;
        b->matches = bm;
        if (a->inliers_mask) {
            b->inliers_mask = (uint8_t*)malloc((size_t)nm + 1);
            memcpy(b->inliers_mask, a->inliers_mask, (size_t)nm);
        }
        if (a->has_H) invert3(a->H, b->H);
    }
    return MIS_OK;
}

void trace_report(MatchWorkspace* ws, std::chrono::steady_clock::time_point t_begin, std::chrono::steady_clock::time_point tq,
                  std::chrono::steady_clock::time_point ts) {
    const auto te = std::chrono::steady_clock::now();
    auto us = [](auto a, auto b) { return (double)std::chrono::duration_cast<std::chrono::microseconds>(b - a).count(); };
    fprintf(stderr, "match: enqueue %.0f us, device wait %.0f us, host assembly %.0f us\n", us(t_begin, tq), us(tq, ts), us(ts, te));
    const OwnedEvent* t = ws->tev;
    auto ms = [&](int i) { float e = 0; if (t[i].ev) hipEventElapsedTime(&e, t[0].ev, t[i].ev); return e; };
    if (!(t[0].ev && t[1].ev && t[3].ev && t[4].ev && t[5].ev && t[6].ev)) return;
    if (t[7].ev) fprintf(stderr, "match chains: main chain's second draw done %.2f\n", ms(7));
    if (t[8].ev) fprintf(stderr, "match chains: speculative draw done %.2f\n", ms(8));
    fprintf(stderr, "match chains, ms after the 2-NN pass was enqueued-behind (device events): first phase done %.2f | tails of its finishers done %.2f | main chain: second RANSAC phase done %.2f, done %.2f | side chain done %.2f | third chain done %.2f\n",
            ms(1), ms(6), ms(2), ms(3), ms(4), ms(5));
}

int match_impl(MisContext* ctx, const MisFeatures* feats, int n, const MisMatchParams* p, int model, const uint8_t* mask, int range_width, int rank, int world,
               MisMatchesInfo* out) {
    MIS_CHECK(ctx, feats && p && out && n >= 1, MIS_E_INVALID, "null argument");
    MIS_CHECK(ctx, model == MIS_MATCH_HOMOGRAPHY || model == MIS_MATCH_AFFINE_PARTIAL, MIS_E_UNSUPPORTED, "unknown matcher model %d (MIS_MATCH_HOMOGRAPHY, MIS_MATCH_AFFINE_PARTIAL)", model);
    MIS_CHECK(ctx, world >= 1 && rank >= 0 && rank < world, MIS_E_INVALID, "bad rank / world size");
    MIS_CHECK(ctx, range_width == -1 || range_width >= 1, MIS_E_INVALID, "range_width must be -1 (all pairs) or >= 1");
    MIS_HIP(ctx, hipSetDevice(ctx->device));
    const auto t_begin = std::chrono::steady_clock::now();
    struct SeqGuard {
        MatchWorkspace* ws; long long seq;
        ~SeqGuard() { if (ws->knn_seq.load() < seq) ws->knn_seq.store(seq); }
    } seq_guard{workspace(ctx), 0};
    seq_guard.seq = ++seq_guard.ws->seq;
    for (int i = 0; i < n * n; i++) init_info(&out[i]);
    MatchPlan pl;
    int rc;
    if ((rc = plan_match(ctx, feats, n, mask, range_width, rank, world, &pl)) != MIS_OK) return rc;
    const int np = (int)pl.pairs.size();
    if (np == 0) return MIS_OK;
    MatchWorkspace* ws = workspace(ctx);
    hipStream_t st = ctx->stream;
    MIS_HIP(ctx, hipStreamSynchronize(st));
    MatchDev d; MatchPinned h;
    if ((rc = carve_dev(ctx, ws->dev, pl, &d)) != MIS_OK) return rc;
    for (HomoBatch* b : {&ws->b1, &ws->b2, &ws->b3})
        if ((rc = homo_batch_reserve(ctx, b, np, (long long)pl.m_total, p->max_iters)) != MIS_OK) return rc;
    if ((rc = carve_pinned(ctx, ws->pinned, pl, &h)) != MIS_OK) return rc;
    memcpy(h.feats, pl.fd.data(), sizeof(FeatDev) * n);
    memcpy(h.pairs, pl.pairs.data(), sizeof(PairDesc) * np);
    MIS_HIP(ctx, hipMemcpyAsync(d.feats, h.feats, sizeof(FeatDev) * n, hipMemcpyHostToDevice, st));
    MIS_HIP(ctx, hipMemcpyAsync(d.pairs, h.pairs, sizeof(PairDesc) * np, hipMemcpyHostToDevice, st));
    *h.l2_bad = 0;
    if ((rc = enqueue_knn(ctx, ws, pl, feats, d, h)) != MIS_OK) return rc;
    MIS_HIP(ctx, ws->events_ready());
    MIS_HIP(ctx, hipEventRecord(ws->ev_knn.ev, st));
    ws->ev_gate = ws->ev_knn.ev;
    hipLaunchKernelGGL(ratio_union_kernel, dim3(np), dim3(1024), 0, st, (const FeatDev*)d.feats, (const PairDesc*)d.pairs, (const int*)d.idx,
                       (const float*)d.dist, 1.f - p->match_conf, d.matches, d.src, d.dst, d.nm, model == MIS_MATCH_HOMOGRAPHY ? 1 : 0);
    hipLaunchKernelGGL(first_calls_kernel, dim3((np + 127) / 128), dim3(128), 0, st, (const PairDesc*)d.pairs, np, (const int*)d.nm, (const float*)d.src,
                       (const float*)d.dst, d.mask, p->num_matches_thresh1, ws->b1.calls, d.out);
    if ((rc = enqueue_chains(ctx, ws, np, p, model, d, h)) != MIS_OK) {
        if (ws->side) hipStreamSynchronize(ws->side);
        if (ws->third) hipStreamSynchronize(ws->third);
        hipStreamSynchronize(st);
        return rc;
    }
    MIS_HIP(ctx, hipGetLastError());
    enqueue_results(ws, np, pl.m_total, d, h, st, model);
    ws->knn_seq.store(seq_guard.seq);
    if (ws->enqueued_cb) {
        void (*cb)(void*) = ws->enqueued_cb;
        void* user = ws->enqueued_user;
        ws->enqueued_cb = nullptr; ws->enqueued_user = nullptr;
        cb(user);
        MIS_HIP(ctx, hipSetDevice(ctx->device));
    }
    const auto tq = std::chrono::steady_clock::now();
    std::chrono::steady_clock::time_point ts;
    if ((rc = assemble_matches(ctx, ws, pl, h, n, model, out, &ts)) != MIS_OK) return rc;
    if (match_trace() && model == MIS_MATCH_HOMOGRAPHY) trace_report(ws, t_begin, tq, ts);
    return MIS_OK;
}

}

extern "C" int mis_match_on_enqueued(MisContext* ctx, void (*fn)(void*), void* user) {
    if (!ctx) return MIS_E_INVALID;
    MatchWorkspace* ws = workspace(ctx);
    ws->enqueued_cb = fn; ws->enqueued_user = user;
    return MIS_OK;
}

extern "C" long long mis_match_sequence(MisContext* ctx) {
    if (!ctx) return -1;
    return workspace(ctx)->seq.load();
}

extern "C" int mis_match_knn_fence(MisContext* ctx, void* stream, long long target_seq, int timeout_ms) {
    if (!ctx) return MIS_E_INVALID;
    MatchWorkspace* ws = (MatchWorkspace*)ctx->match_ws;
    MIS_CHECK(ctx, ws, MIS_E_STATE, "mis_match_sequence must have been called on this context first");
    const auto t0 = std::chrono::steady_clock::now();
    while (ws->knn_seq.load() < target_seq) {
        if (std::chrono::duration_cast<std::chrono::milliseconds>(std::chrono::steady_clock::now() - t0).count() >= timeout_ms) return MIS_FENCE_TIMEOUT;
        std::this_thread::yield();
    }
    if (stream && ws->ev_gate && hipStreamWaitEvent((hipStream_t)stream, ws->ev_gate, 0) != hipSuccess) return mis_set_error(ctx, MIS_E_HIP, "hipStreamWaitEvent failed");
    return MIS_OK;
}

extern "C" int mis_debug_ransac_states(MisContext* ctx, int which, int* out, int cap) {
    if (!ctx || !ctx->match_ws || !out) return -1;
    MatchWorkspace* ws = (MatchWorkspace*)ctx->match_ws;
    return homo_batch_debug_states(ctx, which ? &ws->b2 : &ws->b1, out, cap);
}

extern "C" void mis_match_default_params(MisMatchParams* p) {
    if (p) *p = MisMatchParams{0.32f, 6, 6, 3.0, 2000, 0.995};
}

extern "C" int mis_match_all_pairs(MisContext* ctx, const MisFeatures* feats, int n, const MisMatchParams* p, MisMatchesInfo* out) {
    if (!ctx) return MIS_E_INVALID;
    return match_impl(ctx, feats, n, p, MIS_MATCH_HOMOGRAPHY, nullptr, -1, 0, 1, out);
}

extern "C" int mis_match_pairs_sharded(MisContext* ctx, const MisFeatures* feats, int n, const MisMatchParams* p, int rank, int world,
                                       MisMatchesInfo* out) {
    if (!ctx) return MIS_E_INVALID;
    return match_impl(ctx, feats, n, p, MIS_MATCH_HOMOGRAPHY, nullptr, -1, rank, world, out);
}

extern "C" int mis_match_pairs_select(MisContext* ctx, const MisFeatures* feats, int n, const MisMatchParams* p, const uint8_t* mask, int range_width,
                                      int rank, int world, MisMatchesInfo* out) {
    if (!ctx) return MIS_E_INVALID;
    return match_impl(ctx, feats, n, p, MIS_MATCH_HOMOGRAPHY, mask, range_width, rank, world, out);
}

extern "C" void mis_match_affine_default_params(MisMatchParams* p) {
    if (p) *p = MisMatchParams{0.32f, 6, 6, 3.0, 2000, 0.99};
}

extern "C" int mis_match_pairs_model(MisContext* ctx, const MisFeatures* feats, int n, const MisMatchParams* p, int model, const uint8_t* mask, int range_width,
                                     int rank, int world, MisMatchesInfo* out) {
    if (!ctx) return MIS_E_INVALID;
    return match_impl(ctx, feats, n, p, model, mask, range_width, rank, world, out);
}

extern "C" int mis_matches_free(MisMatchesInfo* m, int count) {
    if (!m) return MIS_E_INVALID;
    for (int i = 0; i < count; i++) {
        free(m[i].matches); free(m[i].inliers_mask);
        m[i].matches = nullptr; m[i].inliers_mask = nullptr;
    }
    return MIS_OK;
}

extern "C" int mis_knn2(MisContext* ctx, const MisFeatures* q, const MisFeatures* t, int* idx2, float* dist2) {
    if (!ctx) return MIS_E_INVALID;
    MIS_CHECK(ctx, q && t && idx2 && dist2, MIS_E_INVALID, "null argument");
    const bool binary = q->desc_dtype == MIS_U8 && q->desc_cols == 32 && t->desc_dtype == MIS_U8 && t->desc_cols == 32;
    const bool l2 = q->desc_dtype == MIS_F32 && t->desc_dtype == MIS_F32 && q->desc_cols == t->desc_cols && q->desc_cols >= 1 && q->desc_cols <= 128;
    MIS_CHECK(ctx, binary || l2, MIS_E_UNSUPPORTED, "mis_knn2 supports 32-byte binary descriptors (Hamming) and f32 descriptors of <= 128 columns (L2)");
    if (q->n <= 0) return MIS_OK;
    MIS_HIP(ctx, hipSetDevice(ctx->device));
    MatchWorkspace* ws = workspace(ctx);
    hipStream_t st = ctx->stream;
    MIS_HIP(ctx, hipStreamSynchronize(st));
    const size_t nq = (size_t)q->n;
    Carver dc;
    const size_t o_feats = dc.take(2 * sizeof(FeatDev)), o_pairs = dc.take(sizeof(PairDesc)), o_idx = dc.take(sizeof(int) * 2 * nq), o_dist = dc.take(sizeof(float) * 2 * nq);
    MIS_HIP(ctx, ws->dev.reserve(dc.off));
    uint8_t* D = (uint8_t*)ws->dev.p;
    const PairDesc pd{0, 1, 0, nq, 0, q->n + t->n};
    int bad = 0;
    if (binary) {
        FeatDev fd[2] = {{(const uint8_t*)q->descriptors, q->keypoints, q->n, q->img_w, q->img_h},
                         {(const uint8_t*)t->descriptors, t->keypoints, t->n, t->img_w, t->img_h}};
        MIS_HIP(ctx, hipMemcpyAsync(D + o_feats, fd, sizeof(fd), hipMemcpyHostToDevice, st));
        MIS_HIP(ctx, hipMemcpyAsync(D + o_pairs, &pd, sizeof(pd), hipMemcpyHostToDevice, st));
        MIS_HIP(ctx, hipStreamSynchronize(st));
        hipLaunchKernelGGL(knn2_hamming_kernel, dim3((q->n + 255) / 256, 1), dim3(256), 0, st, (const FeatDev*)(D + o_feats), (const PairDesc*)(D + o_pairs),
                           (int*)(D + o_idx), (float*)(D + o_dist));
    } else {
        const MisFeatures qt[2] = {*q, *t};
        if (int rc = l2_knn2_pairs(ctx, ws->l2, qt, 2, &pd, 1, false, (int*)(D + o_idx), (float*)(D + o_dist), &bad); rc != MIS_OK) return rc;
    }
    MIS_HIP(ctx, hipGetLastError());
    MIS_HIP(ctx, hipMemcpyAsync(idx2, D + o_idx, sizeof(int) * 2 * nq, hipMemcpyDeviceToHost, st));
    MIS_HIP(ctx, hipMemcpyAsync(dist2, D + o_dist, sizeof(float) * 2 * nq, hipMemcpyDeviceToHost, st));
    MIS_HIP(ctx, hipStreamSynchronize(st));
    MIS_CHECK(ctx, !bad, MIS_E_UNSUPPORTED, "L2 matching needs integer-valued descriptors in 0..255 (SIFT style): exactness of the fp16 MFMA path");
    return MIS_OK;
}

static int solve_single(MisContext* ctx, const float* src, const float* dst, int n, const HomoParams& prm, double* out, int n_out, uint8_t* mask, int* ok) {
    MIS_HIP(ctx, hipSetDevice(ctx->device));
    MatchWorkspace* ws = workspace(ctx);
    hipStream_t st = ctx->stream;
    MIS_HIP(ctx, hipStreamSynchronize(st));
    const size_t nn = (size_t)std::max(n, 1);
    Carver dc;
    const size_t o_src = dc.take(sizeof(float) * 2 * nn), o_dst = dc.take(sizeof(float) * 2 * nn), o_mask = dc.take(nn);
    MIS_HIP(ctx, ws->dev.reserve(dc.off));
    uint8_t* D = (uint8_t*)ws->dev.p;
    int rc;
    if ((rc = homo_batch_reserve(ctx, &ws->b1, 1, (long long)nn, prm.max_iters)) != MIS_OK) return rc;
    if (n) {
        MIS_HIP(ctx, hipMemcpyAsync(D + o_src, src, sizeof(float) * 2 * n, hipMemcpyHostToDevice, st));
        MIS_HIP(ctx, hipMemcpyAsync(D + o_dst, dst, sizeof(float) * 2 * n, hipMemcpyHostToDevice, st));
    }
    HomoCall c;
    c.src = (const float*)(D + o_src); c.dst = (const float*)(D + o_dst); c.mask = D + o_mask; c.pt_off = 0; c.n = n; c.active = 1;
    MIS_HIP(ctx, hipMemcpyAsync(ws->b1.calls, &c, sizeof(c), hipMemcpyHostToDevice, st));
    MIS_HIP(ctx, hipStreamSynchronize(st));
    if ((rc = homo_solve(ctx, &ws->b1, prm)) != MIS_OK) return rc;
    HomoResult r;
    MIS_HIP(ctx, hipMemcpyAsync(&r, ws->b1.results, sizeof(r), hipMemcpyDeviceToHost, st));
    if (mask && n) MIS_HIP(ctx, hipMemcpyAsync(mask, D + o_mask, n, hipMemcpyDeviceToHost, st));
    MIS_HIP(ctx, hipStreamSynchronize(st));
    *ok = r.ok;
    if (r.ok) memcpy(out, r.H, sizeof(double) * n_out); else memset(out, 0, sizeof(double) * n_out);
    return MIS_OK;
}

extern "C" int mis_find_homography(MisContext* ctx, const float* src, const float* dst, int n, double thresh, int max_iters, double confidence,
                                   double H[9], uint8_t* mask, int* ok) {
    if (!ctx) return MIS_E_INVALID;
    MIS_CHECK(ctx, src && dst && H && ok && n >= 0, MIS_E_INVALID, "null argument");
    return solve_single(ctx, src, dst, n, HomoParams{thresh, max_iters, confidence}, H, 9, mask, ok);
}

extern "C" int mis_estimate_affine_partial(MisContext* ctx, const float* src, const float* dst, int n, double thresh, int max_iters, double confidence,
                                           int refine_iters, double M[6], uint8_t* mask, int* ok) {
    if (!ctx) return MIS_E_INVALID;
    MIS_CHECK(ctx, src && dst && M && ok && n >= 0, MIS_E_INVALID, "null argument");
    return solve_single(ctx, src, dst, n, HomoParams{thresh, max_iters, confidence, MODEL_AFFINE_PARTIAL, refine_iters}, M, 6, mask, ok);
// ... 39 lines not shown
```

image_stitching_amd/csrc/orb.hip:

```cpp
#include "common.h"
#include "dev_math.h"
#include <algorithm>
#include <chrono>
#include <cmath>

#define ORB_MAX_LEVELS 16
#define ORB_BORDER 32

namespace {

struct LevelDesc {
    int w, h;
    int pp;
    int sp;
    size_t pad_off;
    size_t map_off;
    float scale;
    int nfeat;
    int n2;
    int tiles_x, tiles_y, tile_off;
    int cap1, cand_off;
    int cap2, fin_off;
    int tab_off;
};
// ... 655 lines not shown
    }
    __syncthreads();
    const int kq[7] = {18, 34, 48, 56, 48, 34, 18};
    for (int i = t; i < (TR + 6) * 16; i += 256) {
        const int r = i >> 4, cg = i & 15;
        const unsigned* p = reinterpret_cast<const unsigned*>(tile + r * TP + 4 * cg);
        const unsigned w0 = p[0], w1 = p[1], w2 = p[2];
        int b[12];
#pragma unroll
        for (int k = 0; k < 4; k++) { b[k] = (w0 >> (8 * k)) & 255; b[4 + k] = (w1 >> (8 * k)) & 255; b[8 + k] = (w2 >> (8 * k)) & 255; }
        unsigned short o[4];
#pragma unroll
        for (int k = 0; k < 4; k++) {
            int acc = 0;
#pragma unroll
            for (int j = 0; j < 7; j++) acc += kq[j] * b[k + 1 + j];
            o[k] = (unsigned short)acc;
        }
        *reinterpret_cast<uint2*>(hbuf + r * 64 + 4 * cg) = make_uint2(o[0] | ((unsigned)o[1] << 16), o[2] | ((unsigned)o[3] << 16));
    }
    __syncthreads();
    const int c = t & 63, px = tx0 + c;
    if (px >= pw) return;
    const int r0 = (t >> 6) * (TR / 4);
    int hv[TR / 4 + 6];
#pragma unroll
    for (int j = 0; j < TR / 4 + 6; j++) hv[j] = hbuf[(r0 + j) * 64 + c];
#pragma unroll
    for (int k = 0; k < TR / 4; k++) {
        const int r = r0 + k, py = ty0 + r;
        if (py >= ph) break;
        const int x = px - ORB_BORDER, y = py - ORB_BORDER;
        uint8_t o;
        if ((unsigned)x < (unsigned)d.w && (unsigned)y < (unsigned)d.h) {
            int acc = 0;
#pragma unroll
            for (int j = 0; j < 7; j++) acc += kq[j] * hv[k + j];
            o = (uint8_t)((acc + (1 << 15)) >> 16);
        } else o = tile[(r + 3) * TP + c + 4];
        dst[(size_t)py * d.pp + px] = o;
    }
}

constexpr int DD_R = 28, DD_P = DD_R + 3, DD_N = 2 * DD_P + 1, DD_ROW_DW = (DD_N + 3 + 3) / 4, DD_PITCH = 4 * DD_ROW_DW + 4;
constexpr int ORB_MAX_PATCH = 40;
static_assert(8 * (ORB_MAX_PATCH / 2) * (ORB_MAX_PATCH / 2) < (2 * DD_R + 1) * (2 * DD_R + 1), "round(sqrt(2) h) <= DD_R: every sample lies in the staged patch");
static_assert(3 + ORB_BORDER >= DD_P, "the staged patch lies inside the padded level");
struct UMax16 { int v[16]; };
__global__ __launch_bounds__(256) void describe_direct_kernel(Levels L, const uint8_t* pad, OrbIO io, const int8_t* pattern, const int* umax, UMax16 um16, size_t ws) {
    __shared__ __attribute__((aligned(16))) uint8_t patch[4][DD_N * DD_PITCH];
    const int wave = threadIdx.x >> 6, lane = threadIdx.x & 63;
    const int i = blockIdx.x * 4 + wave, fr = blockIdx.y;
    WS_OFF(pad, fr, ws);
    MisKeyPoint* kps = io.kps[fr];
    const int* n_ptr = io.n_dev[fr];
    uint8_t* desc = io.desc[fr];
    if (i >= *n_ptr) return;
    const MisKeyPoint kp = kps[i];
    const LevelDesc& d = L.d[kp.octave];
    const float inv = 1.f / d.scale;
    const int cx = mis_round_f(kp.x * inv), cy = mis_round_f(kp.y * inv);
    const int pp = d.pp;
    const uint8_t* org = pad + d.pad_off + (size_t)(cy + ORB_BORDER - DD_P) * pp + (cx + ORB_BORDER - DD_P);
    const int shift = (int)((uintptr_t)org & 3);
    const uint8_t* abase = org - shift;
    uint8_t* P = patch[wave];
    for (int k = lane; k < DD_N * DD_ROW_DW; k += 64) {
        const int r = k / DD_ROW_DW, c = k - r * DD_ROW_DW;
        reinterpret_cast<unsigned*>(P + r * DD_PITCH)[c] = *reinterpret_cast<const unsigned*>(abase + (size_t)r * pp + 4 * c);
    }
    __builtin_amdgcn_fence(__ATOMIC_ACQ_REL, "wavefront");
    __builtin_amdgcn_wave_barrier();
    const int c0 = DD_P * DD_PITCH + DD_P + shift;
    float kp_angle;
    {
        const int hp = L.half_patch;
        const uint8_t* ctr = P + c0;
        int m01 = 0, m10 = 0;
        const int u = lane - hp;
        if (lane <= 2 * hp) {
            m10 = u * ctr[u];
            if (hp <= 15) {
#pragma unroll 3
                for (int v = 1; v <= hp; ++v) {
                    const int vp = ctr[u + v * DD_PITCH], vm = ctr[u - v * DD_PITCH];
                    const bool in = abs(u) <= um16.v[v];
                    m10 += in ? u * (vp + vm) : 0;
                    m01 += in ? v * (vp - vm) : 0;
                }
            } else {
                for (int v = 1; v <= hp; ++v) {
                    if (abs(u) <= umax[v]) {
                        const int vp = ctr[u + v * DD_PITCH], vm = ctr[u - v * DD_PITCH];
                        m10 += u * (vp + vm);
                        m01 += v * (vp - vm);
                    }
                }
            }
        }
#pragma unroll
        for (int o = 32; o > 0; o >>= 1) { m01 += __shfl_xor(m01, o); m10 += __shfl_xor(m10, o); }
        kp_angle = mis_fast_atan2((float)m01, (float)m10);
        if (lane == 0) kps[i].angle = kp_angle;
    }
    float ang = kp_angle * (float)(3.14159265358979323846 / 180.f);
    float sa, ca;
    mis_sincosf(ang, &sa, &ca);
    const int b = lane & 31, h = lane >> 5;
    const int8_t* pat = pattern + b * 32 + h * 16;
    const unsigned* P32 = reinterpret_cast<const unsigned*>(P);
    auto blurred = [&](int ix, int iy) {
        const int a = c0 + (iy - 3) * DD_PITCH + (ix - 3);
        const bool inside = (unsigned)(cx + ix) < (unsigned)d.w && (unsigned)(cy + iy) < (unsigned)d.h;
        const unsigned* q = P32 + (a >> 2);
        const unsigned sh = (unsigned)(a & 3) << 3;
        const int kq[7] = {18, 34, 48, 56, 48, 34, 18};
        unsigned acc = 0, centre = 0;
#pragma unroll
        for (int j = 0; j < 7; j++) {
            const unsigned d0 = q[j * (DD_PITCH / 4)], d1 = q[j * (DD_PITCH / 4) + 1], d2 = q[j * (DD_PITCH / 4) + 2];
            const unsigned lo = __builtin_amdgcn_alignbit(d1, d0, sh), hi = __builtin_amdgcn_alignbit(d2, d1, sh);
            const unsigned hs = __builtin_amdgcn_udot4(lo, 0x38302212u, __builtin_amdgcn_udot4(hi, 0x00122230u, 0u, false), false);
            acc += (unsigned)kq[j] * hs;
            if (j == 3) centre = lo >> 24;
        }
        return inside ? (int)((acc + (1u << 15)) >> 16) : (int)centre;
    };
    int val = 0;
#pragma unroll 1
    for (int bit = 0; bit < 4; bit++) {
        float x0 = (float)pat[4 * bit], y0 = (float)pat[4 * bit + 1], x1 = (float)pat[4 * bit + 2], y1 = (float)pat[4 * bit + 3];
        int ix0 = mis_round_f(x0 * ca - y0 * sa), iy0 = mis_round_f(x0 * sa + y0 * ca);
        int ix1 = mis_round_f(x1 * ca - y1 * sa), iy1 = mis_round_f(x1 * sa + y1 * ca);
        const int t0 = blurred(ix0, iy0), t1 = blurred(ix1, iy1);
        val |= (t0 < t1) << (bit + 4 * h);
    }
    val |= __shfl_xor(val, 32);
    if (h == 0) desc[(size_t)i * 32 + b] = (uint8_t)val;
}

constexpr int ORB_GATHER_MAX = 96;
struct GatherPtrs { const int* p[ORB_GATHER_MAX]; };
__global__ void gather_ints_kernel(GatherPtrs g, int n, int* __restrict__ out) {
    const int i = blockIdx.x * blockDim.x + threadIdx.x;
    if (i < n) out[i] = *g.p[i];
}

}

struct MisOrb {
    MisContext* ctx = nullptr;
    void (*enqueued_cb)(void*) = nullptr;
    void* enqueued_user = nullptr;
    MisOrbParams p;
    int max_w = 0, max_h = 0;
    int cur_w = 0, cur_h = 0;
    Levels L;
    Work w;
    size_t ws_stride = 0;
    int ws_frames = 0;
    int umax_host[64] = {0};
    int8_t pattern_host[1024] = {0};
    void* mem = nullptr;
    size_t pad_bytes = 0, map_bytes = 0;
    int cand_total = 0, fin_total = 0, tab_total = 0, surv_total = 0, out_cap = 0;
    std::vector<int> tab_host;
    int* host_counts = nullptr;
};

namespace {

void linear_exact_coeffs(int dlen, int slen, int* ofs, int* m1) {
    double inv = (double)dlen / (double)slen, scale = 1.0 / inv;
    for (int i = 0; i < dlen; i++) {
        double v = ((double)i + 0.5) * scale - 0.5;
        int iv = (int)floor(v);
        if (iv < 0) { ofs[i] = 0; m1[i] = 0; }
        else if (iv >= slen - 1) { ofs[i] = slen - 1; m1[i] = 0; }
        else { ofs[i] = iv; m1[i] = (int)lrint((v - (double)iv) * 256.0); }
    }
}

constexpr int ORB_MAX_LEVEL_FEATURES = 2048 - 128;

inline float level_scale(const MisOrbParams& p, int l) { return (float)pow((double)p.scale_factor, (double)l); }
inline int level_dim(int len, float sc) { return (int)lrint((double)((float)len / sc)); }

void level_budgets(const MisOrbParams& p, int* nfeat) {
    float factor = (float)(1.0 / (double)p.scale_factor);
    float nd = (float)p.nfeatures * (1 - factor) / (1 - (float)pow((double)factor, (double)p.nlevels));
    int sum = 0;
    for (int l = 0; l < p.nlevels - 1; l++) { nfeat[l] = (int)lrintf(nd); sum += nfeat[l]; nd *= factor; }
    nfeat[p.nlevels - 1] = std::max(p.nfeatures - sum, 0);
}

int check_level_sizes(MisContext* ctx, const MisOrbParams& p, int w, int h) {
    for (int l = 0; l < p.nlevels; l++) {
        const float sc = level_scale(p, l);
        MIS_CHECK(ctx, level_dim(w, sc) >= 1 && level_dim(h, sc) >= 1, MIS_E_UNSUPPORTED,
                  "ORB level %d of a %dx%d frame is empty (scale_factor %g, nlevels %d)", l, w, h, (double)p.scale_factor, p.nlevels);
    }
    return MIS_OK;
}

void plan_levels(MisOrb* o, int w, int h) {
    Levels& L = o->L;
    const MisOrbParams& p = o->p;
    L.n = p.nlevels; L.fast_t = p.fast_threshold; L.patch = p.patch_size; L.half_patch = p.patch_size / 2; L.edge = p.edge_threshold;
    size_t pad_off = 0, map_off = 0;
    int cand_off = 0, fin_off = 0, tab_off = 0, surv_off = 0;
    int nfeat[ORB_MAX_LEVELS];
    level_budgets(p, nfeat);
    for (int l = 0; l < L.n; l++) {
        LevelDesc& d = L.d[l];
        float sc = level_scale(p, l);
        d.scale = sc;
        d.w = level_dim(w, sc);
        d.h = level_dim(h, sc);
        d.pp = (int)mis_align_up((size_t)d.w + 2 * ORB_BORDER, 64);
        d.sp = (int)mis_align_up((size_t)d.w, 64);
        d.pad_off = pad_off; pad_off += (size_t)d.pp * (d.h + 2 * ORB_BORDER);
        d.map_off = map_off; map_off += (size_t)d.sp * d.h;
        d.nfeat = nfeat[l];
        d.n2 = p.score_type == 0 ? 2 * d.nfeat : d.nfeat;
        d.tiles_x = (d.w + FT_COLS - 1) / FT_COLS; d.tiles_y = (d.h + FT_ROWS - 1) / FT_ROWS;
        d.tile_off = surv_off; surv_off += d.tiles_x * d.tiles_y;
        d.cap1 = 4 * d.n2 + 4096;
        d.cap2 = std::min(d.nfeat + 128, 2048);
        d.cand_off = cand_off; cand_off += d.cap1;
        d.fin_off = fin_off; fin_off += d.cap2;
        d.tab_off = tab_off; tab_off += (2 * ((d.w + 3) & ~3) + 2 * d.h + 3) & ~3;
    }
    o->pad_bytes = pad_off; o->map_bytes = map_off; o->cand_total = cand_off; o->fin_total = fin_off; o->tab_total = tab_off; o->surv_total = surv_off;
    o->tab_host.assign(tab_off, 0);
    for (int l = 1; l < L.n; l++) {
        int* t = o->tab_host.data() + L.d[l].tab_off;
        const int dw4 = (L.d[l].w + 3) & ~3;
        linear_exact_coeffs(L.d[l].w, L.d[l - 1].w, t, t + dw4);
        linear_exact_coeffs(L.d[l].h, L.d[l - 1].h, t + 2 * dw4, t + 2 * dw4 + L.d[l].h);
    }
}

int upload_tables(MisOrb* o) {
    MisContext* ctx = o->ctx;
    if (o->tab_total)
        MIS_HIP(ctx, hipMemcpyAsync(o->w.tab, o->tab_host.data(), sizeof(int) * o->tab_total, hipMemcpyHostToDevice, ctx->stream));
    MIS_HIP(ctx, hipStreamSynchronize(ctx->stream));
    return MIS_OK;
}

int enqueue_detect_group(MisOrb* o, const DevView* img, int w, int h, MisFeatures* out, int ng) {
    MisContext* ctx = o->ctx;
    const Levels& L = o->L;
    const Work& W = o->w;
    hipStream_t st = ctx->stream;
    const LevelDesc& d0 = L.d[0];
    const size_t ws = o->ws_stride;
    const unsigned nf = (unsigned)ng;
    OrbIO io;
    for (int k = 0; k < ORB_BATCH; k++) {
        const int q = k < ng ? k : 0;
        io.src[k] = (const uint8_t*)img[q].data; io.sstride[k] = img[q].stride;
        io.aligned[k] = (img[q].stride % 4 == 0) && ((uintptr_t)img[q].data % 4 == 0);
        io.kps[k] = out[q].keypoints; io.n_dev[k] = mis_feat_count(&out[q], o->out_cap);
        io.desc[k] = (uint8_t*)out[q].descriptors;
    }
    MIS_HIP(ctx, hipMemset2DAsync(W.hist, ws ? ws : sizeof(int) * (256 * HIST_COPIES * ORB_MAX_LEVELS + 4 * ORB_MAX_LEVELS), 0,
                                  sizeof(int) * (256 * HIST_COPIES * ORB_MAX_LEVELS + 4 * ORB_MAX_LEVELS), nf, st));
    hipLaunchKernelGGL(gray_kernel, dim3((w + 1023) / 1024, (h + GRAY_ROWS - 1) / GRAY_ROWS, nf), dim3(256), 0, st, io, w, h, W.pad + d0.pad_off, d0.pp, ws);
    for (int l = 1; l < L.n; l++) {
        const LevelDesc &s = L.d[l - 1], &d = L.d[l];
        hipLaunchKernelGGL(resize_kernel, dim3((d.w + 255) / 256, (d.h + 4 * RS_ROWS - 1) / (4 * RS_ROWS), nf), dim3(256), 0, st, W.pad + s.pad_off, s.w, s.h, s.pp, W.pad + d.pad_off, d.w,
                           d.h, d.pp, W.tab + d.tab_off, ws);
    }
    const int pw0 = d0.w + 2 * ORB_BORDER;
    hipLaunchKernelGGL((border_kernel<true>), dim3((d0.h * 16 + 255) / 256, 1, L.n * nf), dim3(256), 0, st, L, W.pad, ws);
    hipLaunchKernelGGL((border_kernel<false>), dim3((pw0 + 1023) / 1024, 2 * ORB_BORDER / 4, L.n * nf), dim3(256), 0, st, L, W.pad, ws);
    dim3 gmap((d0.w + FT_COLS - 1) / FT_COLS, (d0.h + FT_ROWS - 1) / FT_ROWS, L.n * nf);
    hipLaunchKernelGGL(fast_nms_kernel, gmap, dim3(256), 0, st, L, W.pad, W.hist, W.tile_cnt, W.surv_xy, W.surv_sc, ws);
    hipLaunchKernelGGL(fast_cut_kernel, dim3(L.n, nf), dim3(256), 0, st, L, W.hist, W.thr, W.flags, ws);
    hipLaunchKernelGGL(compact_kernel, dim3((d0.tiles_x * d0.tiles_y + CT_TILES - 1) / CT_TILES, L.n, nf), dim3(256), 0, st, L, W.tile_cnt, W.surv_xy, W.surv_sc, W.thr, W.cnt1,
                       W.cand_xy, W.cand_resp, ws);
    const int use_harris = o->p.score_type == 0;
    if (use_harris)
        hipLaunchKernelGGL(harris_kernel, dim3((L.d[0].cap1 + 255) / 256, L.n, nf), dim3(256), 0, st, L, W.pad, W.cnt1, W.cand_xy, W.cand_resp, ws);
    hipLaunchKernelGGL(select_rank_kernel, dim3(L.n, nf), dim3(1024), 0, st, L, W.cnt1, W.cand_xy, W.cand_resp, W.cnt2, W.fin_xy, W.fin_resp, W.flags,
                       use_harris, ws);
    hipLaunchKernelGGL(assemble_kernel, dim3((o->out_cap + 3) / 4, nf), dim3(256), 0, st, L, W.cnt2, W.fin_xy, W.fin_resp, io, o->out_cap, ws);
    UMax16 um16;
    for (int v = 0; v < 16; v++) um16.v[v] = o->umax_host[v];
    hipLaunchKernelGGL(describe_direct_kernel, dim3((o->out_cap + 3) / 4, nf), dim3(256), 0, st, L, W.pad, io, W.pattern, W.umax, um16, ws);
    MIS_HIP(ctx, hipGetLastError());
    return MIS_OK;
}

int check_image(MisOrb* o, const MisImage* bgr) {
    MisContext* ctx = o->ctx;
    MIS_CHECK(ctx, bgr && bgr->data, MIS_E_INVALID, "null image");
    MIS_CHECK(ctx, bgr->dtype == MIS_U8 && bgr->channels == 3, MIS_E_UNSUPPORTED, "ORB input must be 8UC3 (BGR)");
    MIS_CHECK(ctx, bgr->width <= o->max_w && bgr->height <= o->max_h && bgr->width >= 64 && bgr->height >= 64, MIS_E_INVALID,
              "image %dx%d outside the finder's range (64x64 .. %dx%d)", bgr->width, bgr->height, o->max_w, o->max_h);
    return MIS_OK;
}

int replan_if_needed(MisOrb* o, int w, int h) {
    if (w == o->cur_w && h == o->cur_h) return MIS_OK;
    const int rc = check_level_sizes(o->ctx, o->p, w, h);
    if (rc != MIS_OK) return rc;
    MIS_HIP(o->ctx, hipStreamSynchronize(o->ctx->stream));
    plan_levels(o, w, h);
    o->cur_w = w; o->cur_h = h;
    return upload_tables(o);
}

int orb_alloc_workspace(MisOrb* o, int frames) {
    MisContext* ctx = o->ctx;
    size_t off = 0;
    auto carve = [&](size_t bytes) { size_t o_ = off; off += mis_align_up(bytes, 256); return o_; };
    size_t o_pad = carve(o->pad_bytes);
    size_t o_hist = carve(sizeof(int) * (256 * HIST_COPIES * ORB_MAX_LEVELS + 4 * ORB_MAX_LEVELS)), o_flags = carve(256);
    size_t o_sxy = carve(sizeof(uint32_t) * FT_SLOTS * (size_t)o->surv_total), o_ssc = carve(FT_SLOTS * (size_t)o->surv_total), o_tc = carve(sizeof(int) * (size_t)o->surv_total);
    size_t o_cxy = carve(sizeof(uint32_t) * o->cand_total), o_cr = carve(sizeof(float) * o->cand_total);
    size_t o_fxy = carve(sizeof(uint32_t) * o->fin_total), o_fr = carve(sizeof(float) * o->fin_total);
    size_t o_tab = carve(sizeof(int) * (o->tab_total + 4)), o_umax = carve(sizeof(int) * 64), o_pat = carve(1024);
    const size_t tail = mis_align_up(o->map_bytes, 256) + mis_align_up(o->pad_bytes, 256);
    void* mem = nullptr;
    if (hipMalloc(&mem, off * (size_t)frames + tail) != hipSuccess) return mis_set_error(ctx, MIS_E_NOMEM, "hipMalloc of %zu bytes failed", off * (size_t)frames + tail);
    o->mem = mem; o->ws_stride = off; o->ws_frames = frames;
    uint8_t* m = (uint8_t*)o->mem;
    uint8_t* shared = m + off * (size_t)frames;
    Work& W = o->w;
    W.pad = m + o_pad; W.nms = shared; W.blur = shared + mis_align_up(o->map_bytes, 256);
    W.hist = (int*)(m + o_hist); W.thr = W.hist + 256 * HIST_COPIES * ORB_MAX_LEVELS; W.cnt1 = W.thr + ORB_MAX_LEVELS; W.cnt2 = W.cnt1 + ORB_MAX_LEVELS;
    W.surv_xy = (uint32_t*)(m + o_sxy); W.surv_sc = m + o_ssc; W.tile_cnt = (int*)(m + o_tc);
    W.flags = (int*)(m + o_flags);
    W.cand_xy = (uint32_t*)(m + o_cxy); W.cand_resp = (float*)(m + o_cr); W.fin_xy = (uint32_t*)(m + o_fxy); W.fin_resp = (float*)(m + o_fr);
    W.tab = (int*)(m + o_tab); W.umax = (int*)(m + o_umax); W.pattern = (int8_t*)(m + o_pat);
    return MIS_OK;
}

int orb_init_workspace(MisOrb* o) {
    MisContext* ctx = o->ctx;
    const Work& W = o->w;
    MIS_HIP(ctx, hipMemcpyAsync(W.umax, o->umax_host, sizeof(o->umax_host), hipMemcpyHostToDevice, ctx->stream));
    MIS_HIP(ctx, hipMemcpyAsync(W.pattern, o->pattern_host, sizeof(o->pattern_host), hipMemcpyHostToDevice, ctx->stream));
    MIS_HIP(ctx, hipMemset2DAsync(W.flags, o->ws_stride, 0, 256, (size_t)o->ws_frames, ctx->stream));
    MIS_HIP(ctx, hipStreamSynchronize(ctx->stream));
    return upload_tables(o);
}

int orb_ensure_frames(MisOrb* o, int frames) {
    frames = std::min(frames, ORB_BATCH);
    if (o->ws_frames >= frames) return MIS_OK;
    MisContext* ctx = o->ctx;
    MIS_HIP(ctx, hipStreamSynchronize(ctx->stream));
    void* old = o->mem;
    const Work oldw = o->w;
    const size_t olds = o->ws_stride;
    const int oldf = o->ws_frames;
    int rc = MIS_E_NOMEM;
    for (int f = frames; f > oldf; f = std::max(oldf, f / 2)) {
        if ((rc = orb_alloc_workspace(o, f)) == MIS_OK) break;
    }
    if (rc != MIS_OK) {
        o->mem = old; o->w = oldw; o->ws_stride = olds; o->ws_frames = oldf;
        return oldf >= 1 ? MIS_OK : rc;
    }
    if (old) MIS_HIP(ctx, hipFree(old));
    return orb_init_workspace(o);
}

int gather_counts_and_flags(MisOrb* o, MisFeatures* out, int n, int* flags) {
    MisContext* ctx = o->ctx;
    const int total = n + o->ws_frames;
    std::vector<int> vals(total);
    if (!o->host_counts) MIS_HIP(ctx, hipHostMalloc((void**)&o->host_counts, sizeof(int) * ORB_GATHER_MAX, hipHostMallocMapped));
    int* dev_view = nullptr;
    MIS_HIP(ctx, hipHostGetDevicePointer((void**)&dev_view, o->host_counts, 0));
    for (int i0 = 0; i0 < total; i0 += ORB_GATHER_MAX) {
        const int m = std::min(ORB_GATHER_MAX, total - i0);
        GatherPtrs gp;
        for (int k = 0; k < m; k++)
            gp.p[k] = i0 + k < n ? mis_feat_count(&out[i0 + k], o->out_cap) : (const int*)((const char*)o->w.flags + (size_t)(i0 + k - n) * o->ws_stride);
        hipLaunchKernelGGL(gather_ints_kernel, dim3(1), dim3(ORB_GATHER_MAX), 0, ctx->stream, gp, m, dev_view);
        MIS_HIP(ctx, hipStreamSynchronize(ctx->stream));
        std::copy(o->host_counts, o->host_counts + m, vals.begin() + i0);
    }
    for (int i = 0; i < n; i++) out[i].n = vals[i];
    *flags = 0;
    for (int k = n; k < total; k++) *flags |= vals[k];
    return MIS_OK;
}

}

extern "C" void mis_orb_default_params(MisOrbParams* p) {
    if (p) *p = MisOrbParams{4000, 1.2f, 8, 1, 0, 2, 0, 40, 20};
}

extern "C" int mis_orb_create(MisContext* ctx, const MisOrbParams* p, int max_w, int max_h, MisOrb** out) {
    if (!ctx || !out) return MIS_E_INVALID;
    MIS_CHECK(ctx, p, MIS_E_INVALID, "null params");
    MIS_CHECK(ctx, p->nlevels >= 1 && p->nlevels <= ORB_MAX_LEVELS && p->first_level == 0 && p->wta_k == 2 && p->patch_size >= 2 &&
                       p->patch_size <= ORB_MAX_PATCH && p->nfeatures >= 1 && p->scale_factor > 1.f && (p->score_type == 0 || p->score_type == 1) &&
                       p->edge_threshold >= 0 && p->fast_threshold >= 1 && p->fast_threshold < 255,
              MIS_E_UNSUPPORTED, "unsupported ORB parameters (need first_level 0, wta_k 2, patch <= 40, nlevels <= 16)");
    MIS_CHECK(ctx, p->patch_size != 31, MIS_E_UNSUPPORTED, "ORB patch_size 31 (OpenCV's fixed bit_pattern_31_) is not supported");
    {
        int nfeat[ORB_MAX_LEVELS];
        level_budgets(*p, nfeat);
        for (int l = 0; l < p->nlevels; l++)
            MIS_CHECK(ctx, nfeat[l] <= ORB_MAX_LEVEL_FEATURES, MIS_E_UNSUPPORTED,
                      "ORB nfeatures %d gives level %d a budget of %d keypoints (at most %d per level)", p->nfeatures, l, nfeat[l], ORB_MAX_LEVEL_FEATURES);
    }
    MIS_CHECK(ctx, max_w >= 64 && max_h >= 64 && max_w <= 32767 && max_h <= 32767, MIS_E_INVALID, "bad maximum size");
    if (int rc = check_level_sizes(ctx, *p, max_w, max_h)) return rc;
    MIS_HIP(ctx, hipSetDevice(ctx->device));
    MisOrb* o = new MisOrb();
    o->ctx = ctx; o->p = *p; o->max_w = max_w; o->max_h = max_h;
    plan_levels(o, max_w, max_h);
    o->out_cap = o->fin_total;
    int umax[64] = {0};
    {
        int hp = p->patch_size / 2, v, v0;
        int vmax = (int)floor((double)((float)hp * sqrtf(2.f) / 2 + 1));
        int vmin = (int)ceil((double)((float)hp * sqrtf(2.f) / 2));
        for (v = 0; v <= vmax; ++v) umax[v] = (int)lrint(sqrt((double)hp * hp - (double)v * v));
        for (v = hp, v0 = 0; v >= vmin; --v) {
            while (umax[v0] == umax[v0 + 1]) ++v0;
            umax[v] = v0;
            ++v0;
        }
    }
    int8_t pat[1024];
    {
        uint64_t state = 0x34985739u;
        auto next = [&]() { state = (uint64_t)(uint32_t)state * 4164903690u + (uint32_t)(state >> 32); return (uint32_t)state; };
        int hp = p->patch_size / 2;
        for (int i = 0; i < 1024; i++) pat[i] = (int8_t)(int)(next() % (uint32_t)(2 * hp + 1) + (uint32_t)(-hp));
    }
    int rc0 = orb_alloc_workspace(o, 1);
    if (rc0 != MIS_OK) { delete o; return rc0; }
    memcpy(o->umax_host, umax, sizeof(umax));
    memcpy(o->pattern_host, pat, sizeof(pat));
    o->cur_w = max_w; o->cur_h = max_h;
    int rc = orb_init_workspace(o);
    if (rc != MIS_OK) { hipFree(o->mem); delete o; return rc; }
    *out = o;
    return MIS_OK;
}

extern "C" int mis_orb_destroy(MisOrb* o) {
    if (!o) return MIS_OK;
    hipSetDevice(o->ctx->device);
    hipStreamSynchronize(o->ctx->stream);
    if (o->mem) hipFree(o->mem);
    if (o->host_counts) hipHostFree(o->host_counts);
    delete o;
    return MIS_OK;
}


extern "C" int mis_orb_detect_batch(MisOrb* o, const MisImage* imgs, int n, MisFeatures* out) {
    if (!o) return MIS_E_INVALID;
    MisContext* ctx = o->ctx;
    MIS_CHECK(ctx, imgs && out && n >= 1, MIS_E_INVALID, "null argument");
    MIS_HIP(ctx, hipSetDevice(ctx->device));
    int rc;
    for (int i = 0; i < n; i++) {
        if ((rc = check_image(o, &imgs[i])) != MIS_OK) return rc;
        MIS_CHECK(ctx, imgs[i].width == imgs[0].width && imgs[i].height == imgs[0].height, MIS_E_INVALID, "batch frames must share one size");
    }
    if ((rc = replan_if_needed(o, imgs[0].width, imgs[0].height)) != MIS_OK) return rc;
    if ((rc = orb_ensure_frames(o, n)) != MIS_OK) return rc;
    std::vector<DevView> dimg(n);
    for (int i = 0; i < n; i++) memset(&out[i], 0, sizeof(MisFeatures));
    auto fail = [&](int code) {
        hipStreamSynchronize(ctx->stream);
        for (int i = 0; i < n; i++)
            if (out[i].keypoints || out[i].descriptors) mis_features_free(ctx, &out[i]);
        return code;
    };
    for (int i = 0; i < n; i++) {
        out[i].img_idx = i; out[i].img_w = imgs[i].width; out[i].img_h = imgs[i].height;
        if ((rc = mis_feat_alloc(ctx, o->out_cap, 32, MIS_U8, &out[i])) != MIS_OK) return fail(rc);
        if ((rc = dimg[i].read(ctx, &imgs[i])) != MIS_OK) return fail(rc);
    }
    const bool trace = getenv("MIS_ORB_TRACE") != nullptr;
    const auto t_enq0 = std::chrono::steady_clock::now();
    for (int g0 = 0; g0 < n; g0 += o->ws_frames) {
        const int ng = std::min(o->ws_frames, n - g0);
        if ((rc = enqueue_detect_group(o, &dimg[g0], imgs[0].width, imgs[0].height, &out[g0], ng)) != MIS_OK) return fail(rc);
    }
    if (trace) fprintf(stderr, "orb batch: %d frames enqueued in %.0f us\n", n, (double)std::chrono::duration_cast<std::chrono::microseconds>(std::chrono::steady_clock::now() - t_enq0).count());
    if (o->enqueued_cb) {
        void (*cb)(void*) = o->enqueued_cb;
        void* user = o->enqueued_user;
        o->enqueued_cb = nullptr; o->enqueued_user = nullptr;
        cb(user);
        MIS_HIP(ctx, hipSetDevice(ctx->device));
    }
    int flags = 0;
    if ((rc = gather_counts_and_flags(o, out, n, &flags)) != MIS_OK) return rc;
    if (flags) {
        hipMemset2DAsync(o->w.flags, o->ws_stride, 0, sizeof(int), (size_t)o->ws_frames, ctx->stream);
        return mis_set_error(ctx, MIS_E_OVERFLOW, "ORB candidate buffers overflowed (flags %d): too many tied scores", flags);
    }
    return MIS_OK;
}

extern "C" int mis_orb_detect(MisOrb* o, const MisImage* bgr, MisFeatures* out) { return mis_orb_detect_batch(o, bgr, 1, out); }

extern "C" int mis_orb_on_enqueued(MisOrb* o, void (*fn)(void*), void* user) {
    if (!o) return MIS_E_INVALID;
    o->enqueued_cb = fn; o->enqueued_user = user;
    return MIS_OK;
}

extern "C" int mis_orb_debug_level(MisOrb* o, int level, int which, uint8_t* host_out, int* width, int* height) {
    if (!o) return MIS_E_INVALID;
    MisContext* ctx = o->ctx;
    MIS_CHECK(ctx, level >= 0 && level < o->L.n && which >= 0 && which <= 2, MIS_E_INVALID, "bad level / selector");
    const LevelDesc& d = o->L.d[level];
    int w = which == 2 ? d.w + 2 * ORB_BORDER : d.w, h = which == 2 ? d.h + 2 * ORB_BORDER : d.h;
    if (width) *width = w;
    if (height) *height = h;
    if (!host_out) return MIS_OK;
    MIS_HIP(ctx, hipSetDevice(ctx->device));
    const uint8_t* src;
    size_t pitch;
    if (which == 0) { src = o->w.pad + d.pad_off + (size_t)ORB_BORDER * d.pp + ORB_BORDER; pitch = d.pp; }
    else if (which == 1) {
        MIS_HIP(ctx, hipMemsetAsync(o->w.nms + d.map_off, 0, (size_t)d.sp * d.h, ctx->stream));
        hipLaunchKernelGGL(nms_raster_kernel, dim3(256), dim3(64), 0, ctx->stream, d, o->w.tile_cnt, o->w.surv_xy, o->w.surv_sc, o->w.nms);
        src = o->w.nms + d.map_off; pitch = d.sp;
    }
    else {
        const int pw0 = o->L.d[0].w + 2 * ORB_BORDER, ph0 = o->L.d[0].h + 2 * ORB_BORDER;
        hipLaunchKernelGGL(blur_kernel, dim3((pw0 + 63) / 64, (ph0 + 31) / 32, o->L.n), dim3(256), 0, ctx->stream, o->L, o->w.pad, o->w.blur);
        src = o->w.blur + d.pad_off; pitch = d.pp;
    }
    MIS_HIP(ctx, hipMemcpy2DAsync(host_out, w, src, pitch, w, h, hipMemcpyDeviceToHost, ctx->stream));
    MIS_HIP(ctx, hipStreamSynchronize(ctx->stream));
    return MIS_OK;
}

#ifdef MIS_ORB_STATS
extern "C" int mis_debug_orb_stats(unsigned long long* out, int reset) {
    hipDeviceSynchronize();
    hipMemcpyFromSymbol(out, HIP_SYMBOL(g_orb_stats), sizeof(unsigned long long) * 8);
    if (reset) { unsigned long long z[8] = {0}; hipMemcpyToSymbol(HIP_SYMBOL(g_orb_stats), z, sizeof(z)); }
    return 0;
}
#endif
```

image_stitching_amd/distributed.py:

```python
import ctypes as C
import os
import time

import numpy as np
import torch

from . import _capi as capi
from . import stitching as st


def frame_block(n, rank, world):
    base, rem = divmod(n, world)
    lo = rank * base + min(rank, rem)
    return list(range(lo, lo + base + (1 if rank < rem else 0)))


class Comm:

    def __init__(self, rank=0, world=1, group=None, always_collective=False):
        self.rank, self.world, self.group = rank, world, group
        self._stage = False
        self._solo = world == 1 and not always_collective
        if not self._solo:
            import torch.distributed as dist
# ... 230 lines not shown
                            capi.BLEND_FEATHER: lambda: st.FeatherBlender(self.cctx, sharp), capi.BLEND_NO: lambda: st.Blender(self.cctx)}[btype]()
        self.blender.prepare(corners, sizes)
        self.warper = st.RotationWarper(self.cctx, scale, self.kind)
        self.pano_size = (pw, ph)
        return btype, bands

    def warp_feed(self, frame, cam, roi):
        tl, img_s, mask = self.warper.warp_fused(frame, cam["K"], cam["R"], roi)
        self.blender.feed(img_s, mask, tl)

    def match_fence_target(self):
        return int(self.ctx.lib.mis_match_sequence(self.ctx.h)) + 1

    def on_match_enqueued(self, fn):
        if fn is None:
            self._enqueued_fn = None
            self.ctx.lib.mis_match_on_enqueued(self.ctx.h, None, None)
            return
        self._enqueued_fn = fn
        if getattr(self, "_enqueued_cb", None) is None:
            self._enqueued_cb = C.CFUNCTYPE(None, C.c_void_p)(self._run_enqueued)
        self.ctx.check(self.ctx.lib.mis_match_on_enqueued(self.ctx.h, C.cast(self._enqueued_cb, C.c_void_p), None))

    def _run_enqueued(self, _user):
        fn, self._enqueued_fn = getattr(self, "_enqueued_fn", None), None
        if fn is not None:
            fn()

    def compose_after_knn(self, target_seq):
        rc = self.ctx.lib.mis_match_knn_fence(self.ctx.h, self._compose_stream_handle, target_seq, 50)
        if rc == 1:
            self.fence_timeouts = getattr(self, "fence_timeouts", 0) + 1
        elif rc != 0:
            self.ctx.check(rc)

    def warp_feed_many(self, frames, cams, rois):
        self.blender.compose_frames(frames, self.warper.scale, cams, rois, self.kind)

    def accumulators(self):
        out = []
        dev = self.ctx.device
        nb = self.ctx.lib.mis_blender_num_bands(self.blender.h)
        for l in range(nb + 1):
            w, h, lp, wp = C.c_int(), C.c_int(), C.c_void_p(), C.c_void_p()
            self.cctx.check(self.cctx.lib.mis_blender_level_info(self.blender.h, l, C.byref(w), C.byref(h), C.byref(lp), C.byref(wp)))
            out.append((dev_tensor(lp.value, (h.value, w.value * 3), "<i2", dev), dev_tensor(wp.value, (h.value, w.value), "<f4", dev)))
        return out

    def finalize(self):
        return self.blender.blend()

    def num_bands(self):
        return self.ctx.lib.mis_blender_num_bands(self.blender.h)

    def level_sizes(self):
        out = []
        for l in range(self.num_bands() + 1):
            w, h = C.c_int(), C.c_int()
            self.cctx.check(self.cctx.lib.mis_blender_level_info(self.blender.h, l, C.byref(w), C.byref(h), None, None))
            out.append((w.value, h.value))
        return out

    @staticmethod
    def _rect_array(rects):
        return (capi.MisLevelRect * max(len(rects), 1))(*[capi.MisLevelRect(*r) for r in rects])

    def pack_rects(self, rects, nbytes):
        buf = torch.empty(max(int(nbytes), 16), dtype=torch.uint8, device=self.ctx.device)
        if rects:
            self.cctx.check(self.cctx.lib.mis_blender_pack_rects(self.blender.h, self._rect_array(rects), len(rects), C.c_void_p(buf.data_ptr()), buf.numel()))
        return buf[:int(nbytes)]

    def add_rects(self, rects, buf):
        if rects:
            self.cctx.check(self.cctx.lib.mis_blender_add_rects(self.blender.h, self._rect_array(rects), len(rects), C.c_void_p(buf.data_ptr()), buf.numel()))

    def zero_rects(self, rects):
        if rects:
            self.cctx.check(self.cctx.lib.mis_blender_zero_rects(self.blender.h, self._rect_array(rects), len(rects)))

    def finalize_columns(self, x0, x1):
        w, h = self.blender._size
        x1 = min(x1, w)
        dst = st._empty_image(self.cctx, h, x1 - x0, 3, torch.int16)
        msk = st._empty_image(self.cctx, h, x1 - x0, 1, torch.uint8)
        d, m = st.as_image(dst), st.as_image(msk)
        self.cctx.check(self.cctx.lib.mis_blender_blend_columns(self.blender.h, int(x0), int(x1), C.byref(d), C.byref(m)))
        return dst, msk

    def strip_to_bytes(self, img, msk, cap_w):
        h, w = msk.shape
        out = torch.zeros(h * cap_w * 7, dtype=torch.uint8, device=self.ctx.device)
        lib, cx = self.cctx.lib, self.cctx
        cx.check(lib.mis_copy_2d(cx.h, C.c_void_p(out.data_ptr()), cap_w * 6, C.c_void_p(img.data_ptr()), img.stride(0) * 2, w * 6, h))
        cx.check(lib.mis_copy_2d(cx.h, C.c_void_p(out.data_ptr() + h * cap_w * 6), cap_w, C.c_void_p(msk.data_ptr()), msk.stride(0), w, h))
        return out

    def assemble(self, strips, bounds, cap_w, size):
        w, h = size
        pano = st._empty_image(self.cctx, h, w, 3, torch.int16)
        mask = st._empty_image(self.cctx, h, w, 1, torch.uint8)
        lib, cx = self.cctx.lib, self.cctx
        for k, (x0, x1) in enumerate(bounds):
            x1 = min(x1, w)
            if x1 <= x0:
                continue
            base = strips[k].data_ptr()
            cx.check(lib.mis_copy_2d(cx.h, C.c_void_p(pano.data_ptr() + x0 * 6), pano.stride(0) * 2, C.c_void_p(base), cap_w * 6, (x1 - x0) * 6, h))
            cx.check(lib.mis_copy_2d(cx.h, C.c_void_p(mask.data_ptr() + x0), mask.stride(0), C.c_void_p(base + h * cap_w * 6), cap_w, x1 - x0, h))
        return pano, mask

    def sync(self):
        torch.cuda.synchronize(self.ctx.device)


class StitchJob:

    def __init__(self, ctx, frame_size, cameras, rank=0, world_size=1, group=None, engine=None, config=None, force_collectives=False, always_collective=False):
        self.cfg = config or st.StitchConfig.hot_path()
        st.check_seam_config(self.cfg)
        self.kind = st.check_warp_config(self.cfg)
        st.check_range_config(self.cfg)
        st.check_matcher_config(self.cfg)
        self.engine = engine or HipEngine(ctx, frame_size, self.cfg)
        engine_warp = getattr(self.engine, "warp_type", "spherical")
        if engine_warp != self.cfg.warp_type:
            raise NotImplementedError("warp_type %r: the engine %s warps %r only" % (self.cfg.warp_type, type(self.engine).__name__, engine_warp))
        engine_range = getattr(self.engine, "range_width", -1)
        if engine_range != self.cfg.range_width:
            raise NotImplementedError("range_width %r: the engine %s matches with range_width %r only" % (self.cfg.range_width, type(self.engine).__name__, engine_range))
        engine_matcher = getattr(self.engine, "matcher_type", "homography")
        if engine_matcher != self.cfg.matcher_type:
            raise NotImplementedError("matcher_type %r: the engine %s matches with matcher_type %r only" % (self.cfg.matcher_type, type(self.engine).__name__, engine_matcher))
        self.work_scale, self.work_size = st.work_geometry(self.cfg, frame_size)
        if self.work_scale != 1.0 and getattr(self.engine, "work_scale", 1.0) != self.work_scale:
            raise NotImplementedError("work_megapix %r (work scale %.6f): the engine %s does not resize frames to work scale"
                                      % (self.cfg.work_megapix, self.work_scale, type(self.engine).__name__))
        self.cams0 = cameras
        self.work_cams0 = cameras if self.work_scale == 1.0 else [st.scaled_camera(c, self.work_scale) for c in cameras]
        self.cams = self.work_cams0
        self.n = len(cameras)
        self.rank, self.world = rank, world_size
        self.comm = Comm(rank, world_size, group, always_collective)
        self.my_frames = frame_block(self.n, rank, world_size)
        self.frame_size = frame_size
        self.scale = st.Stitcher.warped_image_scale(self.cams)
        self.force_collectives = force_collectives
        self.seam_needed = self.cfg.expos_comp_type != "no" or self.cfg.seam_find_type != "no"
        counts = {len(frame_block(self.n, r, world_size)) for r in range(world_size)}
        if len(counts) != 1:
            raise ValueError("the frame count must divide evenly over the ranks")

    def stage_features(self, frames):
        return self.engine.detect([frames[i] for i in self.my_frames])

    def stage_gather(self, local_feats):
        if self.world == 1 and not self.force_collectives:
            return local_feats
        counts_all = self.comm.all_gather(self.engine.feature_counts(local_feats)).flatten(0, 1)
        cap = max(int(counts_all.max()), 1)
        kps, desc = self.engine.pack_features(local_feats, cap)
        kps_all = self.comm.all_gather(kps).flatten(0, 1)
        desc_all = self.comm.all_gather(desc).flatten(0, 1)
        return self.engine.unpack_features(kps_all, desc_all, counts_all)

    def stage_match(self, feats):
        pm = self.engine.match(feats, self.rank, self.world)
        if self.world == 1 and not self.force_collectives and isinstance(self.engine, HipEngine):
            return pm, self.engine.confidence_tensor(pm, self.n, on_device=False)
        conf = self.engine.confidence_tensor(pm, self.n)
        conf = self.comm.all_reduce_sum(conf)
        return pm, conf

    def stage_prune(self, conf):
        return [int(i) for i in st.leaveBiggestComponentConf(conf.cpu().numpy().reshape(self.n, self.n), self.cfg.conf_thresh)]

    def stage_compose_prepare(self, indices):
        eng = self.engine
        self.scale = st.Stitcher.warped_image_scale([self.cams[i] for i in indices])
        g = st.compose_geometry(self.cfg, self.frame_size, self.scale, self.work_scale)
        self._geom = g
        ccams = {i: st.scaled_camera(self.cams[i], g.aspect) for i in indices} if g.aspect != 1.0 else {i: self.cams[i] for i in indices}
        if g.size != tuple(self.frame_size) and not hasattr(eng, "resize_frame"):
            raise NotImplementedError("this engine does not resize frames (compose_megapix > 0 needs resize_frame)")
        if hasattr(eng, "warp_rois"):
            rois = dict(zip(indices, eng.warp_rois(g.warp_scale, [ccams[i] for i in indices], g.size)))
        else:
            rois = {i: eng.warp_roi(g.warp_scale, ccams[i], g.size) for i in indices}
        corners = [(rois[i][0], rois[i][1]) for i in indices]
        sizes = [(rois[i][2], rois[i][3]) for i in indices]
        btype, bands = eng.begin_compose(g.warp_scale, corners, sizes)
        self._compose_indices, self._compose_rois, self._compose_cams = indices, rois, ccams
        return btype, bands

    def stage_compose(self, frames, indices, prepared=None):
        eng = self.engine
        btype, bands = prepared if prepared is not None else self.stage_compose_prepare(indices)
        rois, ccams, g = self._compose_rois, self._compose_cams, self._geom
        mine = [i for i in self.my_frames if i in rois]
        cframes = {i: eng.resize_frame(frames[i], g.compose_scale) for i in mine} if g.size != tuple(self.frame_size) else frames
        if self.seam_needed:
            marks = getattr(self, "marks", None)
            if marks is not None:
                marks.append(("compose: sized", time.perf_counter()))
            self.stage_seam(frames, indices)
            if marks is not None:
                marks.append(("compose: seams solved", time.perf_counter()))
            if hasattr(eng, "warp_feed_seam_many"):
                eng.warp_feed_seam_many([cframes[i] for i in mine], [ccams[i] for i in mine], [rois[i] for i in mine], [indices.index(i) for i in mine])
            else:
                for i in mine:
                    eng.warp_feed_seam(cframes[i], ccams[i], rois[i], indices.index(i))
            return btype, bands
        if hasattr(eng, "warp_feed_many"):
            eng.warp_feed_many([cframes[i] for i in mine], [ccams[i] for i in mine], [rois[i] for i in mine])
        else:
            for i in mine:
                eng.warp_feed(cframes[i], ccams[i], rois[i])
        return btype, bands

    def stage_seam(self, frames, indices):
        eng = self.engine
        mine = [i for i in self.my_frames if i in indices]
        local = eng.seam_local([frames[i] for i in mine], [self.cams[i] for i in mine], self.scale)
        if getattr(self, "marks", None) is not None:
            self.marks.append(("compose: seam-scale warps enqueued", time.perf_counter()))
        if self.world == 1 and not self.force_collectives:
            items = local
        else:
            per = len(self.my_frames)
            meta = torch.zeros((per, 5), dtype=torch.int32)
            for k, (i, it) in enumerate(zip(mine, local)):
                meta[k] = torch.tensor([i, it[0][0], it[0][1], it[2].shape[1], it[2].shape[0]], dtype=torch.int32)
            meta[len(mine):, 0] = -1
            dev = torch.device(getattr(eng, "exchange_device", None) or (local[0][1].device if local else "cpu"))
            meta_all = self.comm.all_gather(meta.to(dev)).flatten(0, 1).cpu()
            cap = max(int((meta_all[:, 3] * meta_all[:, 4]).max()), 1)
            bufs = [eng.seam_pack(it, cap) for it in local] + [torch.zeros(cap * 4, dtype=torch.uint8, device=dev) for _ in range(per - len(mine))]
            all_bufs = self.comm.all_gather(torch.stack(bufs)).flatten(0, 1)
            by_index = {}
            for row, buf in zip(meta_all.tolist(), all_bufs):
                if row[0] >= 0:
                    iw, mw = eng.seam_unpack(buf, row[3], row[4], cap)
                    by_index[row[0]] = ((row[1], row[2]), iw, mw)
            items = [by_index[i] for i in indices]
        eng.seam_global([it[0] for it in items], [it[1] for it in items], [it[2] for it in items])

    def rank_region(self, r, indices, rois, bands, w0, h0):
        mine = [i for i in frame_block(self.n, r, self.world) if i in rois]
        if not mine:
            return None
        px = min(rois[i][0] for i in indices)
        py = min(rois[i][1] for i in indices)
        gap, a = 3 << bands, (1 << bands) - 1
        x0 = max(0, min(rois[i][0] for i in mine) - px - gap) & ~a
        y0 = max(0, min(rois[i][1] for i in mine) - py - gap) & ~a
        x1 = min(w0, (max(rois[i][0] + rois[i][2] for i in mine) - px + gap + a) & ~a)
        y1 = min(h0, (max(rois[i][1] + rois[i][3] for i in mine) - py + gap + a) & ~a)
        return x0, y0, x1, y1

    @staticmethod
    def strip_bounds(w0, bands, world):
        q = 1 << bands
        nq = w0 // q
        c = [(k * nq // world) * q for k in range(world)] + [w0]
        return [(c[k], c[k + 1]) for k in range(world)]

    @staticmethod
    def need_ranges(strip, level_sizes):
        lo, hi = strip
        out = [(lo, hi)]
        for l in range(1, len(level_sizes)):
            lo, hi = max(0, (lo >> 1) - 1), min(level_sizes[l][0], ((hi - 1) >> 1) + 2)
            out.append((lo, hi))
        return out

    @staticmethod
    def exchange_rects(region, need, level_sizes):
        rects, off = [], 0
        if region is None:
            return rects, 0
        rx0, ry0, rx1, ry1 = region
        for l, ((lw, lh), (nlo, nhi)) in enumerate(zip(level_sizes, need)):
            x0, x1 = max(min(rx0 >> l, lw), nlo), min(min(-((-rx1) >> l), lw), nhi)
            y0, y1 = min(ry0 >> l, lh), min(-((-ry1) >> l), lh)
            if x1 <= x0 or y1 <= y0:
                continue
            m = (x1 - x0) * (y1 - y0)
            rects.append((l, x0, y0, x1, y1, off))
            off += (m * 6 + 15) // 16 * 16 + (m * 4 + 15) // 16 * 16
        return rects, off

    def stage_reduce_finalize(self):
        eng = self.engine
        sizes = eng.level_sizes()
        bands = len(sizes) - 1
        w0, h0 = sizes[0]
        indices, rois = self._compose_indices, self._compose_rois
        world = self.world
        bounds = self.strip_bounds(w0, bands, world)
        needs = [self.need_ranges(bnd, sizes) for bnd in bounds]
        regions = [self.rank_region(r, indices, rois, bands, w0, h0) for r in range(world)]
        plan = [[self.exchange_rects(regions[r], needs[k], sizes) for k in range(world)] for r in range(world)]
        me = self.rank
        send = [eng.pack_rects(*plan[me][k]) for k in range(world)]
        recv = self.comm.all_to_all_bytes(send, [plan[r][me][1] for r in range(world)])
        full_h = [(l, lo, 0, hi, sizes[l][1], 0) for l, (lo, hi) in enumerate(needs[me]) if hi > lo]
# ... 191 lines not shown
```

image_stitching_amd/stitching.py:

```python
import ctypes as C
import math
from dataclasses import dataclass, field

import numpy as np

from . import _capi as capi

try:
    import torch
except Exception:
    torch = None


class MisError(RuntimeError):
    def __init__(self, code, text):
        super().__init__("libmistitch error %d: %s" % (code, text))
        self.code = code


KP_DTYPE = np.dtype([("x", "f4"), ("y", "f4"), ("size", "f4"), ("angle", "f4"), ("response", "f4"), ("octave", "i4")])
DMATCH_DTYPE = np.dtype([("query_idx", "i4"), ("train_idx", "i4"), ("img_idx", "i4"), ("distance", "f4")])

_TORCH_DT = {}
if torch is not None:
# ... 487 lines not shown
    def feed_batch(self, imgs, masks, tls):
        n = len(imgs)
        im = (capi.MisImage * n)(*[as_image(i) for i in imgs])
        mk = (capi.MisImage * n)(*[as_image(m) for m in masks])
        ts = (capi.MisPoint * n)(*[capi.MisPoint(int(t[0]), int(t[1])) for t in tls])
        self.ctx.check(self.ctx.lib.mis_blender_feed_batch(self.h, im, mk, ts, n))

    def blend(self):
        if self._size is None:
            raise MisError(-5, "blend before prepare")
        w, h = self._size
        dst = _empty_image(self.ctx, h, w, 3, torch.int16)
        msk = _empty_image(self.ctx, h, w, 1, torch.uint8)
        d, m = as_image(dst), as_image(msk)
        self.ctx.check(self.ctx.lib.mis_blender_blend(self.h, C.byref(d), C.byref(m)))
        return dst, msk

    def level(self, i):
        w, h, lp, wp = C.c_int(), C.c_int(), C.c_void_p(), C.c_void_p()
        self.ctx.check(self.ctx.lib.mis_blender_level_info(self.h, i, C.byref(w), C.byref(h), C.byref(lp), C.byref(wp)))
        self.ctx.synchronize()
        n = w.value * h.value
        lap = np.empty((h.value, w.value, 3), np.int16)
        wgt = np.empty((h.value, w.value), np.float32)
        _memcpy_dtoh(lap, lp.value, n * 6)
        _memcpy_dtoh(wgt, wp.value, n * 4)
        return lap, wgt

    def close(self):
        if getattr(self, "h", None) and self.ctx.h:
            self.ctx.lib.mis_blender_destroy(self.h)
        self.h = None

    def __del__(self):
        try:
            self.close()
        except Exception:
            pass


class MultiBandBlender(Blender):

    def __init__(self, ctx, num_bands=5):
        super().__init__(ctx, capi.BLEND_MULTI_BAND, num_bands, 0.0)

    def numBands(self):
        return self.ctx.lib.mis_blender_num_bands(self.h)


class FeatherBlender(Blender):

    def __init__(self, ctx, sharpness=0.02):
        super().__init__(ctx, capi.BLEND_FEATHER, 0, sharpness)


_hip = None


def _memcpy_dtoh(dst_np, dev_ptr, nbytes):
    global _hip
    if _hip is None:
        _hip = C.CDLL("libamdhip64.so")
        _hip.hipMemcpy.argtypes = [C.c_void_p, C.c_void_p, C.c_size_t, C.c_int]
    rc = _hip.hipMemcpy(dst_np.ctypes.data_as(C.c_void_p), C.c_void_p(dev_ptr), nbytes, 2)
    if rc:
        raise RuntimeError("hipMemcpy D2H failed: %d" % rc)


class ImageFeatures:

    def __init__(self, ctx, raw):
        self.ctx, self.raw = ctx, raw

    @property
    def img_idx(self):
        return self.raw.img_idx

    @img_idx.setter
    def img_idx(self, v):
        self.raw.img_idx = int(v)

    @property
    def img_size(self):
        return self.raw.img_w, self.raw.img_h

    def __len__(self):
        return self.raw.n

    def download(self):
        n = self.raw.n
        kps = np.zeros(n, KP_DTYPE)
        dt = np.uint8 if self.raw.desc_dtype == capi.U8 else np.float32
        desc = np.zeros((n, self.raw.desc_cols), dt)
        if n:
            self.ctx.check(self.ctx.lib.mis_features_download(self.ctx.h, C.byref(self.raw), kps.ctypes.data_as(C.c_void_p),
                                                              desc.ctypes.data_as(C.c_void_p)))
        return kps, desc

    @staticmethod
    def upload(ctx, img_size, kps, desc, img_idx=0):
        kps = np.ascontiguousarray(kps, KP_DTYPE)
        desc = np.ascontiguousarray(desc)
        raw = capi.MisFeatures()
        ctx.check(ctx.lib.mis_features_upload(ctx.h, int(img_size[0]), int(img_size[1]), len(kps),
                                              kps.ctypes.data_as(C.c_void_p), desc.ctypes.data_as(C.c_void_p), desc.shape[1],
                                              _NP_DT[desc.dtype], C.byref(raw)))
        raw.img_idx = img_idx
        return ImageFeatures(ctx, raw)

    def close(self):
        if self.raw is not None and self.ctx.h:
            self.ctx.lib.mis_features_free(self.ctx.h, C.byref(self.raw))
        self.raw = None

    def __del__(self):
        try:
            self.close()
        except Exception:
            pass


def orb_params(**kw):
    p = capi.MisOrbParams()
    capi.load().mis_orb_default_params(C.byref(p))
    for k, v in kw.items():
        setattr(p, k, v)
    return p


class OrbFeatureFinder:

    def __init__(self, ctx, max_size, params=None):
        self.ctx = ctx
        self.params = params or orb_params()
        h = C.c_void_p()
        ctx.check(ctx.lib.mis_orb_create(ctx.h, C.byref(self.params), int(max_size[0]), int(max_size[1]), C.byref(h)))
        self.h = h

    def detect(self, img):
        raw = capi.MisFeatures()
        i = as_image(img)
        self.ctx.check(self.ctx.lib.mis_orb_detect(self.h, C.byref(i), C.byref(raw)))
        return ImageFeatures(self.ctx, raw)

    def on_enqueued(self, fn):
        if fn is None:
            self._enqueued_fn = None
            self.ctx.lib.mis_orb_on_enqueued(self.h, None, None)
            return
        self._enqueued_fn = fn
        if getattr(self, "_enqueued_cb", None) is None:
            self._enqueued_cb = C.CFUNCTYPE(None, C.c_void_p)(self._run_enqueued)
        self.ctx.check(self.ctx.lib.mis_orb_on_enqueued(self.h, C.cast(self._enqueued_cb, C.c_void_p), None))

    def _run_enqueued(self, _user):
        fn, self._enqueued_fn = getattr(self, "_enqueued_fn", None), None
        if fn is not None:
            fn()

    def detect_batch(self, imgs):
        n = len(imgs)
        arr = (capi.MisImage * n)(*[as_image(i) for i in imgs])
        raws = (capi.MisFeatures * n)()
        self.ctx.check(self.ctx.lib.mis_orb_detect_batch(self.h, arr, n, raws))
        out = []
        for k in range(n):
            r = capi.MisFeatures()
            C.memmove(C.byref(r), C.byref(raws[k]), C.sizeof(capi.MisFeatures))
            r.img_idx = k
            out.append(ImageFeatures(self.ctx, r))
        return out

    def debug_level(self, level, which):
        w, h = C.c_int(), C.c_int()
        self.ctx.check(self.ctx.lib.mis_orb_debug_level(self.h, level, which, None, C.byref(w), C.byref(h)))
        out = np.zeros((h.value, w.value), np.uint8)
        self.ctx.check(self.ctx.lib.mis_orb_debug_level(self.h, level, which, out.ctypes.data_as(C.c_void_p), C.byref(w), C.byref(h)))
        return out

    def close(self):
        if getattr(self, "h", None) and self.ctx.h:
            self.ctx.lib.mis_orb_destroy(self.h)
        self.h = None

    def __del__(self):
        try:
            self.close()
        except Exception:
            pass


class SiftFeatureFinder:

    def __init__(self, ctx, max_size, params=None):
        self.ctx = ctx
        p = capi.MisSiftParams()
        ctx.lib.mis_sift_default_params(C.byref(p))
        for k, v in (params or {}).items():
            setattr(p, k, v)
        self.params = p
        h = C.c_void_p()
        ctx.check(ctx.lib.mis_sift_create(ctx.h, C.byref(p), int(max_size[0]), int(max_size[1]), C.byref(h)))
        self.h = h

    def detect(self, img):
        raw = capi.MisFeatures()
        i = as_image(img)
        self.ctx.check(self.ctx.lib.mis_sift_detect(self.h, C.byref(i), C.byref(raw)))
        return ImageFeatures(self.ctx, raw)

    def detect_batch(self, imgs):
        n = len(imgs)
        if n == 0:
            return []
        arr = (capi.MisImage * n)(*[as_image(im) for im in imgs])
        raws = (capi.MisFeatures * n)()
        self.ctx.check(self.ctx.lib.mis_sift_detect_batch(self.h, arr, n, raws))
        out = []
        for k in range(n):
            raw = capi.MisFeatures()
            C.memmove(C.byref(raw), C.byref(raws[k]), C.sizeof(capi.MisFeatures))
            out.append(ImageFeatures(self.ctx, raw))
        return out

    def debug_level(self, img, octave, layer, dog=False):
        i = as_image(img)
        w, h = C.c_int(), C.c_int()
        self.ctx.check(self.ctx.lib.mis_sift_debug_level(self.h, C.byref(i), octave, layer, int(dog), None, C.byref(w), C.byref(h)))
        out = np.zeros((h.value, w.value), np.float32)
        self.ctx.check(self.ctx.lib.mis_sift_debug_level(self.h, C.byref(i), octave, layer, int(dog), out.ctypes.data_as(C.c_void_p), C.byref(w), C.byref(h)))
        return out

    def debug_counts(self):
        c = (C.c_uint * 4)()
        self.ctx.check(self.ctx.lib.mis_sift_debug_counts(self.h, c))
        return dict(candidates=int(c[0]), raw=int(c[1]), keypoints=int(c[2]), refined=int(c[3]))

    def close(self):
        if getattr(self, "h", None) and self.ctx.h:
            self.ctx.lib.mis_sift_destroy(self.h)
        self.h = None

    def __del__(self):
        try:
            self.close()
        except Exception:
            pass


def computeImageFeatures(finder, img, img_idx=0):
    f = finder.detect(img)
    f.img_idx = img_idx
    return f


@dataclass
class MatchesInfo:
    src_img_idx: int = -1
    dst_img_idx: int = -1
    matches: np.ndarray = field(default_factory=lambda: np.zeros(0, DMATCH_DTYPE))
    inliers_mask: np.ndarray = field(default_factory=lambda: np.zeros(0, np.uint8))
    num_inliers: int = 0
    H: np.ndarray = None
    confidence: float = 0.0


def _unpack_mi(mi):
    n = mi.n_matches
    out = MatchesInfo(mi.src_img_idx, mi.dst_img_idx)
    if n and mi.matches:
        out.matches = np.frombuffer((C.c_char * (n * 16)).from_address(C.addressof(mi.matches.contents)), DMATCH_DTYPE).copy()
    if n and mi.inliers_mask:
        out.inliers_mask = np.frombuffer((C.c_char * n).from_address(C.addressof(mi.inliers_mask.contents)), np.uint8).copy()
    out.num_inliers = mi.num_inliers
    out.H = np.array(list(mi.H), np.float64).reshape(3, 3) if mi.has_H else None
    out.confidence = mi.confidence
    return out


class PairwiseMatches:

    def __init__(self, ctx, mis, n):
        self._ctx, self._mis, self.n = ctx, mis, n
        self._cache = {}

    @classmethod
    def from_entries(cls, ctx, n, entries):
        mis = (capi.MisMatchesInfo * (n * n))()
        keep = []
        for k in range(n * n):
            mis[k].src_img_idx = mis[k].dst_img_idx = -1
        for i, j, matches, mask, num_inliers, has_H, H, conf in entries:
            mm = np.ascontiguousarray(matches, DMATCH_DTYPE)
            mk = np.ascontiguousarray(mask, np.uint8)
            sw = mm.copy()
            sw["query_idx"], sw["train_idx"] = mm["train_idx"], mm["query_idx"]
            Hd = np.asarray(H, np.float64).reshape(3, 3) if has_H else None
            for (a, b, arr, Hm) in ((i, j, mm, Hd), (j, i, sw, np.linalg.inv(Hd) if has_H else None)):
                e = mis[a * n + b]
                e.src_img_idx, e.dst_img_idx, e.n_matches = a, b, len(arr)
                e.matches = C.cast(arr.ctypes.data, C.POINTER(capi.MisDMatch)) if len(arr) else None
                e.inliers_mask = C.cast(mk.ctypes.data, C.POINTER(C.c_uint8)) if len(mk) else None
                e.num_inliers, e.has_H, e.confidence = int(num_inliers), 1 if has_H else 0, float(conf)
                if has_H:
                    for q, v in enumerate(Hm.reshape(9)):
                        e.H[q] = v
# ... 453 lines not shown
```

include/mistitch.h:

```cpp
#ifndef MISTITCH_H
#define MISTITCH_H

#include <stddef.h>
#include <stdint.h>

#ifdef __cplusplus
extern "C" {
#endif

#define MIS_OK 0
#define MIS_E_INVALID (-1)
#define MIS_E_HIP (-2)
#define MIS_E_NOMEM (-3)
#define MIS_E_OVERFLOW (-4)
#define MIS_E_STATE (-5)
#define MIS_E_UNSUPPORTED (-6)
#define MIS_FENCE_TIMEOUT 1

enum { MIS_MEM_HOST = 0, MIS_MEM_DEVICE = 1 };
enum { MIS_U8 = 0, MIS_S16 = 1, MIS_F32 = 2 };
enum { MIS_INTER_NEAREST = 0, MIS_INTER_LINEAR = 1 };
enum { MIS_BORDER_CONSTANT = 0, MIS_BORDER_REFLECT = 2 };
enum { MIS_WARP_SPHERICAL = 0, MIS_WARP_CYLINDRICAL = 1, MIS_WARP_PLANE = 2, MIS_WARP_MERCATOR = 3, MIS_WARP_FISHEYE = 4, MIS_WARP_STEREOGRAPHIC = 5 };
#define MIS_WARP_KIND_IS_KNOWN(kind) ((kind) >= MIS_WARP_SPHERICAL && (kind) <= MIS_WARP_STEREOGRAPHIC)
#define MIS_WARP_ROI_IS_FULL_SCAN(kind) ((kind) >= MIS_WARP_MERCATOR && (kind) <= MIS_WARP_STEREOGRAPHIC)
enum { MIS_BLEND_NO = 0, MIS_BLEND_FEATHER = 1, MIS_BLEND_MULTI_BAND = 2 };

typedef struct MisContext MisContext;
typedef struct MisOrb MisOrb;
typedef struct MisBlender MisBlender;

typedef struct { int x, y; } MisPoint;
typedef struct { int width, height; } MisSize;
typedef struct { int x, y, width, height; } MisRect;

typedef struct {
    void* data;
    int width, height, channels;
    size_t stride;
    int dtype;
    int mem;
} MisImage;

int mis_context_create(int device, void* stream, MisContext** out);
int mis_stream_create(int device, int priority, void** stream);
int mis_stream_destroy(void* stream);
int mis_context_destroy(MisContext* ctx);
int mis_context_synchronize(MisContext* ctx);
int mis_context_wait(MisContext* ctx, MisContext* other);
const char* mis_last_error(const MisContext* ctx);
const char* mis_version(void);
int mis_image_free(MisContext* ctx, MisImage* img);

typedef struct {
    float x, y, size, angle, response;
    int octave;
} MisKeyPoint;

typedef struct {
    int nfeatures;
    float scale_factor;
    int nlevels, edge_threshold, first_level, wta_k, score_type, patch_size, fast_threshold;
} MisOrbParams;

typedef struct {
    int img_idx;
    int img_w, img_h;
    int n;
    MisKeyPoint* keypoints;
    void* descriptors;
    int desc_cols, desc_dtype;
    void* owner_;
} MisFeatures;

void mis_orb_default_params(MisOrbParams* p);
int mis_orb_create(MisContext* ctx, const MisOrbParams* p, int max_width, int max_height, MisOrb** out);
int mis_orb_destroy(MisOrb* orb);
int mis_orb_detect(MisOrb* orb, const MisImage* bgr, MisFeatures* out);
int mis_orb_detect_batch(MisOrb* orb, const MisImage* bgr, int n_images, MisFeatures* out);
int mis_orb_on_enqueued(MisOrb* orb, void (*fn)(void*), void* user);
int mis_features_download(MisContext* ctx, const MisFeatures* f, MisKeyPoint* kps_host, void* desc_host);
int mis_features_upload(MisContext* ctx, int img_w, int img_h, int n, const MisKeyPoint* kps_host,
                        const void* desc_host, int desc_cols, int desc_dtype, MisFeatures* out);
int mis_features_free(MisContext* ctx, MisFeatures* f);
int mis_features_pack(MisContext* ctx, const MisFeatures* feats, int m, int cap, int row_bytes, void* kps_dst, void* desc_dst);
int mis_copy_2d(MisContext* ctx, void* dst, size_t dst_pitch, const void* src, size_t src_pitch, size_t width_bytes, size_t height);
int mis_orb_debug_level(MisOrb* orb, int level, int which, uint8_t* host_out, int* width, int* height);

typedef struct {
    float match_conf;
    int num_matches_thresh1, num_matches_thresh2;
    double ransac_thresh;
    int max_iters;
    double confidence;
} MisMatchParams;

typedef struct { int query_idx, train_idx, img_idx; float distance; } MisDMatch;

typedef struct {
    int src_img_idx, dst_img_idx;
    int n_matches;
    MisDMatch* matches;
    uint8_t* inliers_mask;
    int num_inliers;
    int has_H;
    double H[9];
    double confidence;
} MisMatchesInfo;

void mis_match_default_params(MisMatchParams* p);
int mis_match_all_pairs(MisContext* ctx, const MisFeatures* feats, int n, const MisMatchParams* p, MisMatchesInfo* out);
int mis_match_pairs_sharded(MisContext* ctx, const MisFeatures* feats, int n, const MisMatchParams* p, int rank,
                            int world_size, MisMatchesInfo* out);
int mis_match_pairs_select(MisContext* ctx, const MisFeatures* feats, int n, const MisMatchParams* p, const uint8_t* mask,
                           int range_width, int rank, int world_size, MisMatchesInfo* out);
enum { MIS_MATCH_HOMOGRAPHY = 0, MIS_MATCH_AFFINE_PARTIAL = 1 };
void mis_match_affine_default_params(MisMatchParams* p);
int mis_match_pairs_model(MisContext* ctx, const MisFeatures* feats, int n, const MisMatchParams* p, int model, const uint8_t* mask,
                          int range_width, int rank, int world_size, MisMatchesInfo* out);
int mis_matches_free(MisMatchesInfo* m, int count);
long long mis_match_sequence(MisContext* ctx);
int mis_match_knn_fence(MisContext* ctx, void* stream, long long target_seq, int timeout_ms);
int mis_match_on_enqueued(MisContext* ctx, void (*fn)(void*), void* user);
int mis_knn2(MisContext* ctx, const MisFeatures* query, const MisFeatures* train, int* idx2_host, float* dist2_host);
int mis_find_homography(MisContext* ctx, const float* src_xy, const float* dst_xy, int n, double thresh, int max_iters,
                        double confidence, double H[9], uint8_t* mask, int* ok);
int mis_estimate_affine_partial(MisContext* ctx, const float* src_xy, const float* dst_xy, int n, double thresh, int max_iters,
                                double confidence, int refine_iters, double M[6], uint8_t* mask, int* ok);
int mis_leave_biggest_component(const MisMatchesInfo* pairwise, int n, float conf_threshold, int* indices, int* n_indices);
int mis_leave_biggest_component_conf(const double* confidence, int n, float conf_threshold, int* indices, int* n_indices);

typedef struct {
    double focal, aspect, ppx, ppy;
    double R[9];
    double t[3];
} MisCameraParams;
int mis_bundle_adjust_reproj(MisContext* ctx, const MisFeatures* features, const MisMatchesInfo* pairwise, int n, float conf_thresh,
                             const char* refine_mask, MisCameraParams* cameras);
int mis_wave_correct(double* rmats, int n, int kind);

int mis_warp_roi(float scale, int src_width, int src_height, const float K[9], const float R[9], MisRect* roi);
int mis_warp_roi_batch(MisContext* ctx, float scale, int src_width, int src_height, int n, const float* Ks, const float* Rs, MisRect* rois);
int mis_warp_spherical(MisContext* ctx, const MisImage* src, float scale, const float K[9], const float R[9], int interp,
                       int border, MisImage* dst, MisPoint* tl);
int mis_warp_spherical_fused(MisContext* ctx, const MisImage* src_bgr, float scale, const float K[9], const float R[9],
                             MisImage* dst_s16x3, MisImage* dst_mask, MisPoint* tl);
int mis_warp_spherical_fused_roi(MisContext* ctx, const MisImage* src_bgr, float scale, const float K[9], const float R[9],
                                 const MisRect* roi, MisImage* dst_s16x3, MisImage* dst_mask, MisPoint* tl);
int mis_warp_spherical_fused_batch(MisContext* ctx, const MisImage* srcs_u8x3, int n, float scale, const float* Ks, const float* Rs, const MisRect* rois,
                                   MisImage* dsts_s16x3, MisImage* dmasks_u8, MisPoint* tls);
int mis_warp_spherical_fused_batch_timed(MisContext* ctx, const MisImage* srcs_u8x3, int n, float scale, const float* Ks, const float* Rs,
                                         const MisRect* rois, MisImage* dsts_s16x3, MisImage* dmasks_u8, MisPoint* tls, int repeats, float* avg_us);
int mis_warp_spherical_fused_timed(MisContext* ctx, const MisImage* src_bgr, float scale, const float K[9], const float R[9],
                                   MisImage* dst_s16x3, MisImage* dst_mask, MisPoint* tl, int repeats, float* avg_us);
int mis_warper_roi(int kind, float scale, int src_width, int src_height, const float K[9], const float R[9], MisRect* roi);
int mis_warper_roi_batch(MisContext* ctx, int kind, float scale, int src_width, int src_height, int n, const float* Ks, const float* Rs,
                         MisRect* rois);
int mis_warper_warp(MisContext* ctx, int kind, const MisImage* src, float scale, const float K[9], const float R[9], int interp,
                    int border, MisImage* dst, MisPoint* tl);
int mis_warper_warp_roi(MisContext* ctx, int kind, const MisImage* src, float scale, const float K[9], const float R[9], const MisRect* roi,
                        int interp, int border, MisImage* dst, MisPoint* tl);
int mis_warper_warp_fused(MisContext* ctx, int kind, const MisImage* src_bgr, float scale, const float K[9], const float R[9],
                          MisImage* dst_s16x3, MisImage* dst_mask, MisPoint* tl);
int mis_warper_warp_fused_roi(MisContext* ctx, int kind, const MisImage* src_bgr, float scale, const float K[9], const float R[9],
                              const MisRect* roi, MisImage* dst_s16x3, MisImage* dst_mask, MisPoint* tl);
int mis_warper_warp_fused_batch(MisContext* ctx, int kind, const MisImage* srcs_u8x3, int n, float scale, const float* Ks, const float* Rs,
                                const MisRect* rois, MisImage* dsts_s16x3, MisImage* dmasks_u8, MisPoint* tls);
enum { MIS_MATH_LOG = 0, MIS_MATH_TAN = 1, MIS_MATH_SINH = 2, MIS_MATH_ASIN = 3, MIS_MATH_ATAN = 4, MIS_MATH_EXP = 5 };
int mis_debug_math_f32(MisContext* ctx_or_null, int fn, const float* in, float* out, int n);

typedef struct {
    int nfeatures, n_octave_layers;
    double contrast_threshold, edge_threshold, sigma;
} MisSiftParams;
typedef struct MisSift MisSift;
void mis_sift_default_params(MisSiftParams* p);
int mis_sift_create(MisContext* ctx, const MisSiftParams* params , int max_width, int max_height, MisSift** out);
int mis_sift_destroy(MisSift* sift);
int mis_sift_detect(MisSift* sift, const MisImage* bgr, MisFeatures* out);
int mis_sift_detect_batch(MisSift* sift, const MisImage* bgr, int n_images, MisFeatures* out);
int mis_sift_debug_level(MisSift* sift, const MisImage* bgr, int octave, int layer, int dog, float* host_out, int* width, int* height);
int mis_sift_debug_counts(MisSift* sift, unsigned* counts4);

int mis_resize_linear_exact(MisContext* ctx, const MisImage* src, int dst_w, int dst_h, double fx, double fy, MisImage* dst);
int mis_resize_linear_exact_batch(MisContext* ctx, const MisImage* srcs, int n, int dst_w, int dst_h, double fx, double fy, MisImage* dsts);
int mis_rotate(MisContext* ctx, const MisImage* src, int rotate_code, MisImage* dst);
int mis_seam_mask_apply(MisContext* ctx, const MisImage* seam_mask_warped, MisImage* mask_warped);

#define MIS_EXPOS_NO 0
#define MIS_EXPOS_GAIN 1
#define MIS_EXPOS_GAIN_BLOCKS 2
#define MIS_EXPOS_CHANNELS 3
#define MIS_EXPOS_CHANNELS_BLOCKS 4
typedef struct {
    int type;
    int nr_feeds;
    int block_width, block_height;
    int nr_gain_filtering_iterations;
} MisCompensatorParams;
typedef struct MisCompensator MisCompensator;
void mis_compensator_default_params(MisCompensatorParams* params);
int mis_compensator_create_ex(MisContext* ctx, const MisCompensatorParams* params, MisCompensator** out);
int mis_compensator_create(MisContext* ctx, int block_width, int block_height, int nr_gain_filtering_iterations, MisCompensator** out);
int mis_compensator_destroy(MisCompensator* c);
int mis_compensator_feed(MisCompensator* c, const MisPoint* corners, const MisImage* images, const MisImage* masks, int n);
int mis_compensator_gains(const MisCompensator* c, int index, double gains[3]);
int mis_compensator_gain_map(const MisCompensator* c, int index, float* map_host, int capacity, int* blocks_x, int* blocks_y);
int mis_compensator_gain_map_channels(const MisCompensator* c, int index, float* map_host, int capacity, int* blocks_x, int* blocks_y, int* channels);
int mis_compensator_apply(MisCompensator* c, int index, MisImage* image);
int mis_compensator_debug_stats(const MisCompensator* c, int i, int j, int channel, int* N, double* I_ij, double* I_ji);
int mis_seam_voronoi(MisContext* ctx, const MisPoint* corners, MisImage* masks, int n);
#define MIS_SEAM_DP_COLOR 0
int mis_seam_dp(MisContext* ctx, const MisPoint* corners, const MisImage* images, MisImage* masks, int n, int cost_func);

int mis_blend_config(int blend_type, float blend_strength, int pano_width, int pano_height, int* type_out, int* num_bands,
                     float* sharpness);
int mis_result_roi(const MisPoint* corners, const MisSize* sizes, int n, MisRect* roi);
int mis_blender_create(MisContext* ctx, int type, int num_bands, float sharpness, MisBlender** out);
int mis_blender_destroy(MisBlender* b);
int mis_blender_prepare(MisBlender* b, const MisPoint* corners, const MisSize* sizes, int n);
int mis_blender_num_bands(const MisBlender* b);
int mis_blender_feed(MisBlender* b, const MisImage* img_s16x3, const MisImage* mask_u8, MisPoint tl);
int mis_blender_feed_batch(MisBlender* b, const MisImage* imgs_s16x3, const MisImage* masks_u8, const MisPoint* tls, int n);
int mis_blender_blend(MisBlender* b, MisImage* dst_s16x3, MisImage* dst_mask);
int mis_blender_blend_columns(MisBlender* b, int x0, int x1, MisImage* dst_s16x3, MisImage* dst_mask);
typedef struct { int level, x0, y0, x1, y1; unsigned long long offset; } MisLevelRect;
int mis_blender_pack_rects(MisBlender* b, const MisLevelRect* rects, int n, void* dev_buf, size_t bytes);
int mis_blender_add_rects(MisBlender* b, const MisLevelRect* rects, int n, const void* dev_buf, size_t bytes);
int mis_blender_zero_rects(MisBlender* b, const MisLevelRect* rects, int n);
int mis_compose_frames(MisBlender* b, const MisImage* frames, int n, float scale, const float* Ks, const float* Rs, const MisRect* rois);
int mis_compose_frames_kind(MisBlender* b, int kind, const MisImage* frames, int n, float scale, const float* Ks, const float* Rs,
                            const MisRect* rois);
int mis_blender_feed_rect(const MisBlender* b, int width, int height, MisPoint tl, MisRect* tile);
int mis_blender_level_info(const MisBlender* b, int level, int* width, int* height, void** lap_dev, void** weight_dev);

#ifdef __cplusplus
}
#endif
#endif
```

Measured before the change: 3466.

## Enqueue the 2-NN descriptor pass right after ORB detection, ahead of matching

The brute-force Hamming 2-NN kernel is now enqueued on the device stream immediately after ORB detection. It sizes its buffers from per-frame capacity and reads device-side keypoint counts, so it no longer waits for the host to read counts and build the match plan. The matcher adopts these precomputed results when the features, selection and pair order match, and otherwise falls back to the normal path. The count readback becomes an event-based mapped-memory gather, and a redundant stream synchronize is skipped when the stream is already drained. This adds state and validation logic, and the kernel may do extra work on capacity-padded buffers.

```diff
diff --git a/host/job.cpp b/host/job.cpp
--- a/host/job.cpp
+++ b/host/job.cpp
@@ -24,6 +24,7 @@
     const MisImage* work = work_frames(frames);
     prep_.arm([this] { if (spec_ok_) prepare(everyone_); });
     check(ctx_, mis_orb_on_enqueued(orb_, &Hook::fire, &prep_), "mis_orb_on_enqueued");
+    arm_knn_ahead();
     std::vector<MisFeatures> feats(n_);
     std::memset(feats.data(), 0, sizeof(MisFeatures) * n_);
     const int rc_f = mis_orb_detect_batch(orb_, work, n_, feats.data());
diff --git a/host/job_core.cpp b/host/job_core.cpp
--- a/host/job_core.cpp
+++ b/host/job_core.cpp
@@ -138,6 +138,10 @@
     if (rc < 0) check(ctx_, rc, "mis_match_knn_fence");
 }
 
+void JobCore::arm_knn_ahead() {
+    check(ctx_, mis_orb_arm_knn_ahead(orb_, n_, nullptr, cfg_.range_width, 0, 1), "mis_orb_arm_knn_ahead");
+}
+
 void JobCore::compose(const std::vector<MisImage>& frames, const std::vector<int>& frame_ids, const std::vector<int>& idx) {
     std::vector<MisImage> fr;
     std::vector<float> Ks, Rs;
diff --git a/host/job_core.hpp b/host/job_core.hpp
--- a/host/job_core.hpp
+++ b/host/job_core.hpp
@@ -41,6 +41,7 @@
     void synchronize();
     Compose prepare(const std::vector<int>& idx);
     void fence_knn();
+    void arm_knn_ahead();
     const MisImage* work_frames(const std::vector<MisImage>& frames);
     float warp_scale(const std::vector<int>& idx) const;
     void compose(const std::vector<MisImage>& frames, const std::vector<int>& frame_ids, const std::vector<int>& idx);
diff --git a/image_stitching_amd/_capi.py b/image_stitching_amd/_capi.py
--- a/image_stitching_amd/_capi.py
+++ b/image_stitching_amd/_capi.py
@@ -112,6 +112,8 @@
     "mis_orb_detect": (_i, [_vp, _P(MisImage), _P(MisFeatures)]),
     "mis_orb_detect_batch": (_i, [_vp, _P(MisImage), _i, _P(MisFeatures)]),
     "mis_orb_on_enqueued": (_i, [_vp, _vp, _vp]),
+    "mis_orb_arm_knn_ahead": (_i, [_vp, _i, _vp, _i, _i, _i]),
+    "mis_debug_knn_ahead_adopted": (C.c_longlong, [_vp]),
     "mis_features_download": (_i, [_vp, _P(MisFeatures), _vp, _vp]),
     "mis_features_upload": (_i, [_vp, _i, _i, _i, _vp, _vp, _i, _i, _P(MisFeatures)]),
     "mis_features_free": (_i, [_vp, _P(MisFeatures)]),
diff --git a/image_stitching_amd/csrc/common.h b/image_stitching_amd/csrc/common.h
--- a/image_stitching_amd/csrc/common.h
+++ b/image_stitching_amd/csrc/common.h
@@ -40,6 +40,10 @@
 MisFeatLayout mis_feat_layout(int cap, int desc_cols, int desc_dtype);
 int mis_feat_alloc(MisContext* ctx, int cap, int desc_cols, int desc_dtype, MisFeatures* f);
 int* mis_feat_count(const MisFeatures* f, int cap);
+int mis_knn_ahead_enqueue(MisContext* ctx, const MisFeatures* feats, int n, const int* caps, int* const* counts, const uint8_t* mask, int range_width,
+                          int rank, int world);
+void mis_knn_ahead_confirm(MisContext* ctx, const MisFeatures* feats, int n);
+void mis_knn_ahead_drop(MisContext* ctx, const void* owner);
 
 #define MIS_HIP(ctx, call)                                                                             \
     do {                                                                                               \
diff --git a/image_stitching_amd/csrc/features.hip b/image_stitching_amd/csrc/features.hip
--- a/image_stitching_amd/csrc/features.hip
+++ b/image_stitching_amd/csrc/features.hip
@@ -77,6 +77,7 @@
 extern "C" int mis_features_free(MisContext* ctx, MisFeatures* f) {
     if (!ctx || !f) return MIS_E_INVALID;
     if (f->owner_) {
+        mis_knn_ahead_drop(ctx, f->owner_);
         size_t bytes = 0;
         {
             std::lock_guard<std::mutex> lock(g_feat_mutex);
diff --git a/image_stitching_amd/csrc/knn_plan.h b/image_stitching_amd/csrc/knn_plan.h
--- /dev/null
+++ b/image_stitching_amd/csrc/knn_plan.h
@@ -0,0 +1,65 @@
+
+struct PairDesc {
+    int i, j;
+    size_t knn_off12, knn_off21;
+    size_t m_off;
+    int cap;
+};
+
+constexpr int HM_ROWPAD = 256;
+constexpr int HM_MAX_TRAINS = 8192;
+
+struct HmFrame { size_t train_off, query_off; };
+
+struct HmJob { int pair, dir, q0, pad; };
+
+inline bool knn_pair_selected(int i, int j, int n, const uint8_t* mask, int range_width) {
+    if (mask && !mask[(size_t)i * n + j]) return false;
+    return range_width == -1 || j < i + range_width;
+}
+
+inline void hm_job_table(const std::vector<PairDesc>& pairs, int n, const int* nq, std::vector<HmJob>* jobs) {
+    const int np = (int)pairs.size();
+    std::vector<HmJob> lists[8];
+    for (int t = 0; t < n; t++)
+        for (int k = 0; k < np; k++) {
+            const int dir = pairs[k].j == t ? 0 : (pairs[k].i == t ? 1 : -1);
+            if (dir < 0) continue;
+            const int nqf = nq[dir == 0 ? pairs[k].i : pairs[k].j];
+            for (int q0 = 0; q0 < nqf; q0 += 256) lists[t & 7].push_back(HmJob{k, dir, q0, 0});
+        }
+    size_t longest = 0;
+    for (auto& l : lists) longest = std::max(longest, l.size());
+    jobs->assign(longest * 8, HmJob{-1, 0, 0, 0});
+    for (int c = 0; c < 8; c++)
+        for (size_t sl = 0; sl < lists[c].size(); sl++) (*jobs)[sl * 8 + c] = lists[c][sl];
+}
+
+struct KnnCapPlan {
+    std::vector<PairDesc> pairs;
+    std::vector<HmFrame> frames;
+    std::vector<HmJob> jobs;
+    size_t knn_total = 0, xp_bytes = 0;
+};
+inline size_t knn_rows_padded(int n) { return (size_t)(std::max(n, 1) + HM_ROWPAD - 1) / HM_ROWPAD * HM_ROWPAD; }
+inline void plan_knn_capacity(int n, const int* caps, const uint8_t* mask, int range_width, int rank, int world, KnnCapPlan* pl) {
+    pl->pairs.clear(); pl->knn_total = 0;
+    int pair_index = 0;
+    for (int i = 0; i < n; i++)
+        for (int j = i + 1; j < n; j++) {
+            if (!knn_pair_selected(i, j, n, mask, range_width)) continue;
+            if ((pair_index++ % world) != rank) continue;
+            const size_t qi = knn_rows_padded(caps[i]), qj = knn_rows_padded(caps[j]);
+            pl->pairs.push_back(PairDesc{i, j, pl->knn_total, pl->knn_total + qi, 0, 0});
+            pl->knn_total += qi + qj;
+        }
+    pl->frames.resize(n);
+    size_t off = 0;
+    for (int i = 0; i < n; i++) {
+        const size_t bytes = knn_rows_padded(caps[i]) * 128;
+        pl->frames[i].train_off = off; off += bytes;
+        pl->frames[i].query_off = off; off += bytes;
+    }
+    pl->xp_bytes = off;
+    hm_job_table(pl->pairs, n, caps, &pl->jobs);
+}
diff --git a/image_stitching_amd/csrc/match.hip b/image_stitching_amd/csrc/match.hip
--- a/image_stitching_amd/csrc/match.hip
+++ b/image_stitching_amd/csrc/match.hip
@@ -15,12 +15,7 @@
     int n, w, h;
 };
 
-struct PairDesc {
-    int i, j;
-    size_t knn_off12, knn_off21;
-    size_t m_off;
-    int cap;
-};
+#include "knn_plan.h"
 
 constexpr int KNN_TILE = 256;
 __global__ __launch_bounds__(256) void knn2_hamming_kernel(const FeatDev* feats, const PairDesc* pairs, int* idx2, float* dist2) {
@@ -73,14 +68,9 @@
 
 typedef int v4i __attribute__((ext_vector_type(4)));
 typedef int v16i __attribute__((ext_vector_type(16)));
-constexpr int HM_ROWPAD = 256;
-constexpr int HM_MAX_TRAINS = 8192;
 constexpr int HM_NONE = 0x7f000000;
 
-struct HmFrame { size_t train_off, query_off; };
-
 struct HmKeys { int k0[2], k1[2]; };
-struct HmJob { int pair, dir, q0, pad; };
 constexpr int HM_FBIAS = 0x3F800000;
 __device__ __forceinline__ void hm_update(HmKeys& K, int set, int key) {
     asm volatile("v_med3_f32 %0, %1, %2, %3" : "=v"(K.k1[set]) : "v"(K.k0[set]), "v"(K.k1[set]), "v"(key));
@@ -108,6 +98,17 @@
     }
     *reinterpret_cast<uint4*>(out + fr[blockIdx.y].train_off + (size_t)d * 128 + 16 * w) = make_uint4(tq[0], tq[1], tq[2], tq[3]);
     *reinterpret_cast<uint4*>(out + fr[blockIdx.y].query_off + (size_t)d * 128 + 16 * w) = make_uint4(qq[0], qq[1], qq[2], qq[3]);
+}
+constexpr int AHEAD_MAX_FRAMES = 64;
+struct AheadFrames {
+    const uint8_t* desc[AHEAD_MAX_FRAMES];
+    const MisKeyPoint* kps[AHEAD_MAX_FRAMES];
+    const int* count[AHEAD_MAX_FRAMES];
+    int cap[AHEAD_MAX_FRAMES], w[AHEAD_MAX_FRAMES], h[AHEAD_MAX_FRAMES];
+};
+__global__ void feat_counts_kernel(FeatDev* feats, AheadFrames f, int n) {
+    const int i = threadIdx.x;
+    if (i < n) feats[i] = FeatDev{f.desc[i], f.kps[i], min(max(*f.count[i], 0), f.cap[i]), f.w[i], f.h[i]};
 }
 #define HM4_MFMA_FIRST(D, A, B, C, SA, SB) \
     asm volatile("v_mfma_scale_f32_32x32x64_f8f6f4 %0, %1, %2, %3, %4, %5 op_sel_hi:[0,0,0] cbsz:4 blgp:4" : "=&v"(D) : "v"(A), "v"(B), "v"(C), "v"(SA), "v"(SB))
@@ -607,9 +608,30 @@
     OwnedEvent ev_lists;
     void (*enqueued_cb)(void*) = nullptr;
     void* enqueued_user = nullptr;
+    bool drained = true;
+    struct Ahead {
+        bool enqueued = false, valid = false;
+        std::vector<const void*> desc, owner;
+        std::vector<int> caps, counts;
+        std::vector<uint8_t> mask;
+        bool has_mask = false;
+        int range_width = -1;
+        KnnCapPlan plan;
+        bool tables_ready = false;
+        Arena dev, pinned;
+        OwnedEvent ev_tables;
+        PairDesc* d_pairs = nullptr;
+        HmFrame* d_frames = nullptr;
+        HmJob* d_jobs = nullptr;
+        FeatDev* d_feats = nullptr;
+        int* idx = nullptr;
+        float* dist = nullptr;
+        Ahead() { pinned.host = true; }
+    } ahead;
+    long long ahead_adopted = 0;
     MatchWorkspace() { pinned.host = true; }
     ~MatchWorkspace() override {
-        dev.release(); pinned.release(); l2.release();
+        dev.release(); pinned.release(); l2.release(); ahead.dev.release(); ahead.pinned.release();
         homo_batch_release(&b1); homo_batch_release(&b2); homo_batch_release(&b3);
     }
     hipError_t events_ready() {
@@ -691,8 +713,7 @@
     for (int i = 0; i < n; i++)
         for (int j = i + 1; j < n; j++) {
             if (feats[i].n <= 0 || feats[j].n <= 0) continue;
-            if (mask && !mask[(size_t)i * n + j]) continue;
-            if (range_width != -1 && j >= i + range_width) continue;
+            if (!knn_pair_selected(i, j, n, mask, range_width)) continue;
             if ((pair_index++ % world) != rank) continue;
             const int cap = feats[i].n + feats[j].n;
             pl->maxq = std::max(pl->maxq, std::max(feats[i].n, feats[j].n));
@@ -709,19 +730,9 @@
     const int np = (int)pairs.size();
     if (np == 0) return MIS_OK;
     if (pl->kind == DESC_BINARY && pl->maxq <= HM_MAX_TRAINS) {
-        std::vector<HmJob> lists[8];
-        for (int t = 0; t < n; t++)
-            for (int k = 0; k < np; k++) {
-                const int dir = pairs[k].j == t ? 0 : (pairs[k].i == t ? 1 : -1);
-                if (dir < 0) continue;
-                const int nqf = feats[dir == 0 ? pairs[k].i : pairs[k].j].n;
-                for (int q0 = 0; q0 < nqf; q0 += 256) lists[t & 7].push_back(HmJob{k, dir, q0, 0});
-            }
-        size_t longest = 0;
-        for (auto& l : lists) longest = std::max(longest, l.size());
-        pl->hm_jobs.assign(longest * 8, HmJob{-1, 0, 0, 0});
-        for (int c = 0; c < 8; c++)
-            for (size_t sl = 0; sl < lists[c].size(); sl++) pl->hm_jobs[sl * 8 + c] = lists[c][sl];
+        std::vector<int> nq(n);
+        for (int i = 0; i < n; i++) nq[i] = feats[i].n;
+        hm_job_table(pairs, n, nq.data(), &pl->hm_jobs);
     }
     return MIS_OK;
 }
@@ -870,6 +881,7 @@
         for (int q = 0; q < nm; q++) { b->matches[q] = a->matches[q]; std::swap(b->matches[q].query_idx, b->matches[q].train_idx); }
     }
     const hipError_t e = hipStreamSynchronize(ctx->stream);
+    ws->drained = e == hipSuccess;
     *ts = std::chrono::steady_clock::now();
     if (e != hipSuccess || *h.l2_bad) {
         drop_lists();
@@ -940,8 +952,24 @@
             ms(1), ms(6), ms(2), ms(3), ms(4), ms(5));
 }
 
+bool ahead_is_for(const MatchWorkspace::Ahead& A, const MisFeatures* feats, int n, const uint8_t* mask, int range_width, int rank, int world) {
+    if (world != 1 || rank != 0 || n != (int)A.desc.size() || range_width != A.range_width || (mask != nullptr) != A.has_mask) return false;
+    for (int i = 0; i < n; i++) {
+        const MisFeatures& f = feats[i];
+        if (f.descriptors != A.desc[i] || f.owner_ != A.owner[i] || f.desc_dtype != MIS_U8 || f.desc_cols != 32) return false;
+        if (f.n != A.counts[i] || f.n <= 0 || f.n > HM_MAX_TRAINS || f.n > A.caps[i]) return false;
+    }
+    for (int i = 0; mask && i < n; i++)
+        for (int j = i + 1; j < n; j++)
+            if ((mask[(size_t)i * n + j] != 0) != (A.mask[(size_t)i * n + j] != 0)) return false;
+    return true;
+}
+
 int match_impl(MisContext* ctx, const MisFeatures* feats, int n, const MisMatchParams* p, int model, const uint8_t* mask, int range_width, int rank, int world,
                MisMatchesInfo* out) {
+    MatchWorkspace::Ahead& ahead = workspace(ctx)->ahead;
+    const bool ahead_pending = ahead.valid;
+    ahead.valid = ahead.enqueued = false;
     MIS_CHECK(ctx, feats && p && out && n >= 1, MIS_E_INVALID, "null argument");
     MIS_CHECK(ctx, model == MIS_MATCH_HOMOGRAPHY || model == MIS_MATCH_AFFINE_PARTIAL, MIS_E_UNSUPPORTED, "unknown matcher model %d (MIS_MATCH_HOMOGRAPHY, MIS_MATCH_AFFINE_PARTIAL)", model);
     MIS_CHECK(ctx, world >= 1 && rank >= 0 && rank < world, MIS_E_INVALID, "bad rank / world size");
@@ -959,20 +987,28 @@
     if ((rc = plan_match(ctx, feats, n, mask, range_width, rank, world, &pl)) != MIS_OK) return rc;
     const int np = (int)pl.pairs.size();
     if (np == 0) return MIS_OK;
+    bool adopt = ahead_pending && ahead_is_for(ahead, feats, n, mask, range_width, rank, world) && pl.kind == DESC_BINARY && ahead.plan.pairs.size() == pl.pairs.size();
+    for (int k = 0; adopt && k < np; k++) adopt = pl.pairs[k].i == ahead.plan.pairs[k].i && pl.pairs[k].j == ahead.plan.pairs[k].j;
     MatchWorkspace* ws = workspace(ctx);
     hipStream_t st = ctx->stream;
-    MIS_HIP(ctx, hipStreamSynchronize(st));
+    if (!ws->drained) MIS_HIP(ctx, hipStreamSynchronize(st));
+    ws->drained = false;
     MatchDev d; MatchPinned h;
     if ((rc = carve_dev(ctx, ws->dev, pl, &d)) != MIS_OK) return rc;
     for (HomoBatch* b : {&ws->b1, &ws->b2, &ws->b3})
         if ((rc = homo_batch_reserve(ctx, b, np, (long long)pl.m_total, p->max_iters)) != MIS_OK) return rc;
     if ((rc = carve_pinned(ctx, ws->pinned, pl, &h)) != MIS_OK) return rc;
+    if (adopt) {
+        for (int k = 0; k < np; k++) { pl.pairs[k].knn_off12 = ahead.plan.pairs[k].knn_off12; pl.pairs[k].knn_off21 = ahead.plan.pairs[k].knn_off21; }
+        d.idx = ahead.idx; d.dist = ahead.dist;
+        ws->ahead_adopted++;
+    }
     memcpy(h.feats, pl.fd.data(), sizeof(FeatDev) * n);
     memcpy(h.pairs, pl.pairs.data(), sizeof(PairDesc) * np);
-    MIS_HIP(ctx, hipMemcpyAsync(d.feats, h.feats, sizeof(FeatDev) * n, hipMemcpyHostToDevice, st));
-    MIS_HIP(ctx, hipMemcpyAsync(d.pairs, h.pairs, sizeof(PairDesc) * np, hipMemcpyHostToDevice, st));
+    MIS_CHECK(ctx, (uint8_t*)h.pairs - (uint8_t*)h.feats == (uint8_t*)d.pairs - (uint8_t*)d.feats, MIS_E_STATE, "matcher arenas: the input regions differ");
+    MIS_HIP(ctx, hipMemcpyAsync(d.feats, h.feats, (size_t)((uint8_t*)(h.pairs + np) - (uint8_t*)h.feats), hipMemcpyHostToDevice, st));
     *h.l2_bad = 0;
-    if ((rc = enqueue_knn(ctx, ws, pl, feats, d, h)) != MIS_OK) return rc;
+    if (!adopt && (rc = enqueue_knn(ctx, ws, pl, feats, d, h)) != MIS_OK) return rc;
     MIS_HIP(ctx, ws->events_ready());
     MIS_HIP(ctx, hipEventRecord(ws->ev_knn.ev, st));
     ws->ev_gate = ws->ev_knn.ev;
@@ -983,7 +1019,7 @@
     if ((rc = enqueue_chains(ctx, ws, np, p, model, d, h)) != MIS_OK) {
         if (ws->side) hipStreamSynchronize(ws->side);
         if (ws->third) hipStreamSynchronize(ws->third);
-        hipStreamSynchronize(st);
+        ws->drained = hipStreamSynchronize(st) == hipSuccess;
         return rc;
     }
     MIS_HIP(ctx, hipGetLastError());
@@ -1003,6 +1039,95 @@
     return MIS_OK;
 }
 
+}
+
+int mis_knn_ahead_enqueue(MisContext* ctx, const MisFeatures* feats, int n, const int* caps, int* const* counts, const uint8_t* mask, int range_width,
+                          int rank, int world) {
+    MatchWorkspace* ws = workspace(ctx);
+    MatchWorkspace::Ahead& A = ws->ahead;
+    A.valid = A.enqueued = false;
+    if (!feats || !caps || !counts || n < 2 || n > AHEAD_MAX_FRAMES || world != 1 || rank != 0 || !(range_width == -1 || range_width >= 1)) return MIS_OK;
+    int maxcap = 0;
+    for (int i = 0; i < n; i++) {
+        if (feats[i].desc_dtype != MIS_U8 || feats[i].desc_cols != 32 || caps[i] < 1 || caps[i] > HM_MAX_TRAINS || !counts[i]) return MIS_OK;
+        maxcap = std::max(maxcap, caps[i]);
+    }
+    hipStream_t st = ctx->stream;
+    std::vector<uint8_t> sel;
+    if (mask) {
+        sel.assign((size_t)n * n, 0);
+        for (int i = 0; i < n; i++)
+            for (int j = i + 1; j < n; j++) sel[(size_t)i * n + j] = mask[(size_t)i * n + j] != 0;
+    }
+    const bool same_plan = A.tables_ready && (int)A.caps.size() == n && std::equal(caps, caps + n, A.caps.begin()) && A.has_mask == (mask != nullptr) &&
+                           A.mask == sel && A.range_width == range_width;
+    if (!same_plan) {
+        A.tables_ready = false;
+        plan_knn_capacity(n, caps, mask, range_width, rank, world, &A.plan);
+        const KnnCapPlan& P = A.plan;
+        const size_t np = P.pairs.size(), nj = P.jobs.size();
+        A.caps.assign(caps, caps + n);
+        A.has_mask = mask != nullptr;
+        A.mask = sel;
+        A.range_width = range_width;
+        if (np > 0) {
+            Carver c;
+            c.off = P.xp_bytes;
+            const size_t o_tab = c.off, o_pairs = c.take(sizeof(PairDesc) * np), o_fr = c.take(sizeof(HmFrame) * n), o_jobs = c.take(sizeof(HmJob) * nj),
+                         tab_bytes = c.off - o_tab, o_feats = c.take(sizeof(FeatDev) * n), o_idx = c.take(sizeof(int) * 2 * P.knn_total),
+                         o_dist = c.take(sizeof(float) * 2 * P.knn_total);
+            if (A.ev_tables.ev) MIS_HIP(ctx, hipEventSynchronize(A.ev_tables.ev));
+            MIS_HIP(ctx, A.ev_tables.ready());
+            MIS_HIP(ctx, A.dev.reserve(c.off));
+            MIS_HIP(ctx, A.pinned.reserve(tab_bytes));
+            uint8_t *D = (uint8_t*)A.dev.p, *T = (uint8_t*)A.pinned.p;
+            memcpy(T + (o_pairs - o_tab), P.pairs.data(), sizeof(PairDesc) * np);
+            memcpy(T + (o_fr - o_tab), P.frames.data(), sizeof(HmFrame) * n);
+            memcpy(T + (o_jobs - o_tab), P.jobs.data(), sizeof(HmJob) * nj);
+            MIS_HIP(ctx, hipMemcpyAsync(D + o_tab, T, tab_bytes, hipMemcpyHostToDevice, st));
+            MIS_HIP(ctx, hipEventRecord(A.ev_tables.ev, st));
+            A.d_pairs = (PairDesc*)(D + o_pairs); A.d_frames = (HmFrame*)(D + o_fr); A.d_jobs = (HmJob*)(D + o_jobs); A.d_feats = (FeatDev*)(D + o_feats);
+            A.idx = (int*)(D + o_idx); A.dist = (float*)(D + o_dist);
+        }
+        A.tables_ready = true;
+    }
+    if (A.plan.pairs.empty()) return MIS_OK;
+    AheadFrames fr;
+    for (int i = 0; i < n; i++) {
+        fr.desc[i] = (const uint8_t*)feats[i].descriptors; fr.kps[i] = feats[i].keypoints; fr.count[i] = counts[i];
+        fr.cap[i] = caps[i]; fr.w[i] = feats[i].img_w; fr.h[i] = feats[i].img_h;
+    }
+    hipLaunchKernelGGL(feat_counts_kernel, dim3(1), dim3(AHEAD_MAX_FRAMES), 0, st, A.d_feats, fr, n);
+    const int maxpad = (int)knn_rows_padded(maxcap);
+    hipLaunchKernelGGL(hamming_expand4_kernel, dim3(maxpad * 8 / 256, n), dim3(256), 0, st, (const FeatDev*)A.d_feats, (const HmFrame*)A.d_frames, (int8_t*)A.dev.p);
+    hipLaunchKernelGGL(knn2_hamming_fp4_kernel, dim3((unsigned)A.plan.jobs.size()), dim3(256), 0, st, (const FeatDev*)A.d_feats, (const PairDesc*)A.d_pairs,
+                       (const HmFrame*)A.d_frames, (const int8_t*)A.dev.p, A.idx, A.dist, (const HmJob*)A.d_jobs);
+    MIS_HIP(ctx, hipGetLastError());
+    A.desc.resize(n); A.owner.resize(n);
+    for (int i = 0; i < n; i++) { A.desc[i] = feats[i].descriptors; A.owner[i] = feats[i].owner_; }
+    A.enqueued = true;
+    return MIS_OK;
+}
+
+void mis_knn_ahead_confirm(MisContext* ctx, const MisFeatures* feats, int n) {
+    if (!ctx->match_ws) return;
+    MatchWorkspace::Ahead& A = static_cast<MatchWorkspace*>(ctx->match_ws)->ahead;
+    if (!A.enqueued || n != (int)A.desc.size()) { A.valid = A.enqueued = false; return; }
+    A.counts.resize(n);
+    for (int i = 0; i < n; i++) A.counts[i] = feats[i].n;
+    A.valid = true;
+}
+
+void mis_knn_ahead_drop(MisContext* ctx, const void* owner) {
+    if (!ctx->match_ws) return;
+    MatchWorkspace::Ahead& A = static_cast<MatchWorkspace*>(ctx->match_ws)->ahead;
+    if (owner && std::find(A.owner.begin(), A.owner.end(), owner) == A.owner.end()) return;
+    A.valid = A.enqueued = false;
+}
+
+extern "C" long long mis_debug_knn_ahead_adopted(MisContext* ctx) {
+    if (!ctx) return -1;
+    return ctx->match_ws ? static_cast<MatchWorkspace*>(ctx->match_ws)->ahead_adopted : 0;
 }
 
 extern "C" int mis_match_on_enqueued(MisContext* ctx, void (*fn)(void*), void* user) {
diff --git a/image_stitching_amd/csrc/orb.hip b/image_stitching_amd/csrc/orb.hip
--- a/image_stitching_amd/csrc/orb.hip
+++ b/image_stitching_amd/csrc/orb.hip
@@ -831,6 +831,11 @@
     MisContext* ctx = nullptr;
     void (*enqueued_cb)(void*) = nullptr;
     void* enqueued_user = nullptr;
+    bool knn_armed = false;
+    int knn_n = 0, knn_range_width = -1, knn_rank = 0, knn_world = 1;
+    bool knn_has_mask = false;
+    std::vector<uint8_t> knn_mask;
+    OwnedEvent ev_counts;
     MisOrbParams p;
     int max_w = 0, max_h = 0;
     int cur_w = 0, cur_h = 0;
@@ -1071,6 +1076,29 @@
     return MIS_OK;
 }
 
+bool gather_fits_one(const MisOrb* o, int n) { return n + o->ws_frames <= ORB_GATHER_MAX; }
+int gather_enqueue(MisOrb* o, MisFeatures* out, int n) {
+    MisContext* ctx = o->ctx;
+    const int total = n + o->ws_frames;
+    if (!o->host_counts) MIS_HIP(ctx, hipHostMalloc((void**)&o->host_counts, sizeof(int) * ORB_GATHER_MAX, hipHostMallocMapped));
+    int* dev_view = nullptr;
+    MIS_HIP(ctx, hipHostGetDevicePointer((void**)&dev_view, o->host_counts, 0));
+    MIS_HIP(ctx, o->ev_counts.ready());
+    GatherPtrs gp;
+    for (int k = 0; k < total; k++)
+        gp.p[k] = k < n ? mis_feat_count(&out[k], o->out_cap) : (const int*)((const char*)o->w.flags + (size_t)(k - n) * o->ws_stride);
+    hipLaunchKernelGGL(gather_ints_kernel, dim3(1), dim3(ORB_GATHER_MAX), 0, ctx->stream, gp, total, dev_view);
+    MIS_HIP(ctx, hipEventRecord(o->ev_counts.ev, ctx->stream));
+    return MIS_OK;
+}
+int gather_finish(MisOrb* o, MisFeatures* out, int n, int* flags) {
+    MIS_HIP(o->ctx, hipEventSynchronize(o->ev_counts.ev));
+    for (int i = 0; i < n; i++) out[i].n = o->host_counts[i];
+    *flags = 0;
+    for (int k = n; k < n + o->ws_frames; k++) *flags |= o->host_counts[k];
+    return MIS_OK;
+}
+
 }
 
 extern "C" void mis_orb_default_params(MisOrbParams* p) {
@@ -1143,6 +1171,9 @@
 extern "C" int mis_orb_detect_batch(MisOrb* o, const MisImage* imgs, int n, MisFeatures* out) {
     if (!o) return MIS_E_INVALID;
     MisContext* ctx = o->ctx;
+    const bool armed = o->knn_armed;
+    o->knn_armed = false;
+    mis_knn_ahead_drop(ctx, nullptr);
     MIS_CHECK(ctx, imgs && out && n >= 1, MIS_E_INVALID, "null argument");
     MIS_HIP(ctx, hipSetDevice(ctx->device));
     int rc;
@@ -1155,6 +1186,7 @@
     std::vector<DevView> dimg(n);
     for (int i = 0; i < n; i++) memset(&out[i], 0, sizeof(MisFeatures));
     auto fail = [&](int code) {
+        mis_knn_ahead_drop(ctx, nullptr);
         hipStreamSynchronize(ctx->stream);
         for (int i = 0; i < n; i++)
             if (out[i].keypoints || out[i].descriptors) mis_features_free(ctx, &out[i]);
@@ -1172,6 +1204,17 @@
         if ((rc = enqueue_detect_group(o, &dimg[g0], imgs[0].width, imgs[0].height, &out[g0], ng)) != MIS_OK) return fail(rc);
     }
     if (trace) fprintf(stderr, "orb batch: %d frames enqueued in %.0f us\n", n, (double)std::chrono::duration_cast<std::chrono::microseconds>(std::chrono::steady_clock::now() - t_enq0).count());
+    bool ahead = false;
+    if (armed && n == o->knn_n && gather_fits_one(o, n)) {
+        if ((rc = gather_enqueue(o, out, n)) != MIS_OK) return fail(rc);
+        std::vector<int> caps(n, o->out_cap);
+        std::vector<int*> counts(n);
+        for (int i = 0; i < n; i++) counts[i] = mis_feat_count(&out[i], o->out_cap);
+        if ((rc = mis_knn_ahead_enqueue(ctx, out, n, caps.data(), counts.data(), o->knn_has_mask ? o->knn_mask.data() : nullptr, o->knn_range_width,
+                                        o->knn_rank, o->knn_world)) != MIS_OK) return fail(rc);
+        ahead = true;
+        if (trace) fprintf(stderr, "orb batch: 2-NN pass enqueued ahead at %.0f us\n", (double)std::chrono::duration_cast<std::chrono::microseconds>(std::chrono::steady_clock::now() - t_enq0).count());
+    }
     if (o->enqueued_cb) {
         void (*cb)(void*) = o->enqueued_cb;
         void* user = o->enqueued_user;
@@ -1180,11 +1223,13 @@
         MIS_HIP(ctx, hipSetDevice(ctx->device));
     }
     int flags = 0;
-    if ((rc = gather_counts_and_flags(o, out, n, &flags)) != MIS_OK) return rc;
+    if ((rc = ahead ? gather_finish(o, out, n, &flags) : gather_counts_and_flags(o, out, n, &flags)) != MIS_OK) { mis_knn_ahead_drop(ctx, nullptr); return rc; }
     if (flags) {
+        mis_knn_ahead_drop(ctx, nullptr);
         hipMemset2DAsync(o->w.flags, o->ws_stride, 0, sizeof(int), (size_t)o->ws_frames, ctx->stream);
         return mis_set_error(ctx, MIS_E_OVERFLOW, "ORB candidate buffers overflowed (flags %d): too many tied scores", flags);
     }
+    if (ahead) mis_knn_ahead_confirm(ctx, out, n);
     return MIS_OK;
 }
 
@@ -1193,6 +1238,18 @@
 extern "C" int mis_orb_on_enqueued(MisOrb* o, void (*fn)(void*), void* user) {
     if (!o) return MIS_E_INVALID;
     o->enqueued_cb = fn; o->enqueued_user = user;
+    return MIS_OK;
+}
+
+extern "C" int mis_orb_arm_knn_ahead(MisOrb* o, int n, const uint8_t* mask, int range_width, int rank, int world) {
+    if (!o) return MIS_E_INVALID;
+    o->knn_armed = false;
+    if (n <= 0) return MIS_OK;
+    MIS_CHECK(o->ctx, (range_width == -1 || range_width >= 1) && world >= 1 && rank >= 0 && rank < world, MIS_E_INVALID, "bad selection (range_width -1 or >= 1, 0 <= rank < world)");
+    o->knn_n = n; o->knn_range_width = range_width; o->knn_rank = rank; o->knn_world = world;
+    o->knn_has_mask = mask != nullptr;
+    if (mask) o->knn_mask.assign(mask, mask + (size_t)n * n); else o->knn_mask.clear();
+    o->knn_armed = true;
     return MIS_OK;
 }
 
diff --git a/image_stitching_amd/distributed.py b/image_stitching_amd/distributed.py
--- a/image_stitching_amd/distributed.py
+++ b/image_stitching_amd/distributed.py
@@ -406,7 +406,11 @@
             raise ValueError("the frame count must divide evenly over the ranks")
 
     def stage_features(self, frames):
-        return self.engine.detect([frames[i] for i in self.my_frames])
+        mine = [frames[i] for i in self.my_frames]
+        finder = getattr(self.engine, "finder", None)
+        if self.world == 1 and not self.force_collectives and hasattr(finder, "arm_knn_ahead"):
+            finder.arm_knn_ahead(len(mine), None, self.cfg.range_width)
+        return self.engine.detect(mine)
 
     def stage_gather(self, local_feats):
         if self.world == 1 and not self.force_collectives:
diff --git a/image_stitching_amd/stitching.py b/image_stitching_amd/stitching.py
--- a/image_stitching_amd/stitching.py
+++ b/image_stitching_amd/stitching.py
@@ -663,6 +663,14 @@
         if getattr(self, "_enqueued_cb", None) is None:
             self._enqueued_cb = C.CFUNCTYPE(None, C.c_void_p)(self._run_enqueued)
         self.ctx.check(self.ctx.lib.mis_orb_on_enqueued(self.h, C.cast(self._enqueued_cb, C.c_void_p), None))
+
+    def arm_knn_ahead(self, n, mask=None, range_width=-1, rank=0, world_size=1):
+        if mask is not None:
+            mask = np.ascontiguousarray(np.asarray(mask) != 0, np.uint8)
+            if mask.shape != (n, n):
+                raise ValueError("mask must be %d x %d, got shape %r" % (n, n, mask.shape))
+        self.ctx.check(self.ctx.lib.mis_orb_arm_knn_ahead(self.h, int(n), None if mask is None else mask.ctypes.data_as(C.c_void_p),
+                                                          int(range_width), int(rank), int(world_size)))
 
     def _run_enqueued(self, _user):
         fn, self._enqueued_fn = getattr(self, "_enqueued_fn", None), None
diff --git a/include/mistitch.h b/include/mistitch.h
--- a/include/mistitch.h
+++ b/include/mistitch.h
@@ -79,6 +79,7 @@
 int mis_orb_detect(MisOrb* orb, const MisImage* bgr, MisFeatures* out);
 int mis_orb_detect_batch(MisOrb* orb, const MisImage* bgr, int n_images, MisFeatures* out);
 int mis_orb_on_enqueued(MisOrb* orb, void (*fn)(void*), void* user);
+int mis_orb_arm_knn_ahead(MisOrb* orb, int n, const uint8_t* mask, int range_width, int rank, int world);
 int mis_features_download(MisContext* ctx, const MisFeatures* f, MisKeyPoint* kps_host, void* desc_host);
 int mis_features_upload(MisContext* ctx, int img_w, int img_h, int n, const MisKeyPoint* kps_host,
                         const void* desc_host, int desc_cols, int desc_dtype, MisFeatures* out);
@@ -122,6 +123,7 @@
 long long mis_match_sequence(MisContext* ctx);
 int mis_match_knn_fence(MisContext* ctx, void* stream, long long target_seq, int timeout_ms);
 int mis_match_on_enqueued(MisContext* ctx, void (*fn)(void*), void* user);
+long long mis_debug_knn_ahead_adopted(MisContext* ctx);
 int mis_knn2(MisContext* ctx, const MisFeatures* query, const MisFeatures* train, int* idx2_host, float* dist2_host);
 int mis_find_homography(MisContext* ctx, const float* src_xy, const float* dst_xy, int n, double thresh, int max_iters,
                         double confidence, double H[9], uint8_t* mask, int* ok);
```

After: 3527, median of 6. 1.02x the previous value.
